# akshathmangudi/KAN-ViT

Hardware: AMD Instinct MI355X
Metric: images/sec (train step) KAN-ViT 224x224 (higher is better)
Workload: dtype f32

## Files before the change

include/kanvit.h:

```cpp
#ifndef KANVIT_H
#define KANVIT_H

#include <stddef.h>
#include <stdint.h>

#ifdef __cplusplus
extern "C" {
#endif

#if defined(__GNUC__) || defined(__clang__)
#pragma GCC visibility push(default)
#endif

#define KANVIT_ABI_VERSION 7

#define KANVIT_OK 0
#define KANVIT_EINVAL (-22)
#define KANVIT_ENOMEM (-12)
#define KANVIT_EDEVICE (-5)

#define KANVIT_FLAG_BF16_MFMA 1

#define KANVIT_FLAG_UNIFORM_KNOTS 2
#define KANVIT_FLAG_FUSED_LN 8
#define KANVIT_FLAG_SHARED_BPARAMS 4

#define KANVIT_FLAG_SINE_DFREQ 16

#define KANVIT_LINEAR 0
#define KANVIT_CHEBY 1
#define KANVIT_BSPLINE 2
#define KANVIT_RBF 3
#define KANVIT_SINE 4
#define KANVIT_FOURIER 5

typedef struct kanvit_layer_desc {
    int32_t family;
    int32_t groups;
    int32_t x_group_mod;
    int32_t I;
    int32_t O;
    int32_t G;
    int32_t spline_order;
    int32_t has_base;
    float rbf_inv_h;
    int32_t flags;
    int64_t M;
    int64_t ldx;
    int64_t ldu;
    int64_t ldy;
    int64_t bparam_stride;
    float ln_eps;
    int32_t base_act;
} kanvit_layer_desc;


#define KANVIT_BASE_SILU 0
#define KANVIT_BASE_GELU 1
#define KANVIT_BASE_GELU_TANH 2
#define KANVIT_BASE_RELU 3
#define KANVIT_BASE_TANH 4
#define KANVIT_BASE_IDENTITY 5

int kanvit_layer_ln_fusable(const kanvit_layer_desc* d);

size_t kanvit_layer_ln_bwd_workspace(const kanvit_layer_desc* d);
int kanvit_layer_ln_bwd(const kanvit_layer_desc* d, const float* x, const float* stats, const float* bparams, const float* du,
                        float* dx, float* dgamma, float* dbeta, void* workspace, size_t workspace_bytes, void* stream);

size_t kanvit_layer_fwd_workspace(const kanvit_layer_desc* d);
int kanvit_layer_fwd(const kanvit_layer_desc* d, const float* x, const float* u, const float* w,
                     const float* bparams, const float* bias, float* y, void* workspace, size_t workspace_bytes,
                     void* stream);

size_t kanvit_layer_bwd_input_workspace(const kanvit_layer_desc* d);
int kanvit_layer_bwd_input(const kanvit_layer_desc* d, const float* x, const float* u, const float* w,
                           const float* bparams, const float* dy, float* dx, float* du, float* dparam,
                           void* workspace, size_t workspace_bytes, void* stream);
int64_t kanvit_layer_dparam_tiles(const kanvit_layer_desc* d);
int kanvit_layer_sine_dfreq_ok(const kanvit_layer_desc* d);

size_t kanvit_layer_bwd_weight_workspace(const kanvit_layer_desc* d);
int kanvit_layer_bwd_weight(const kanvit_layer_desc* d, const float* x, const float* u, const float* bparams,
                            const float* dy, float* dw, void* workspace, size_t workspace_bytes, void* stream);

int kanvit_edge_l1_supported(const kanvit_layer_desc* d);
int64_t kanvit_edge_l1_row_bands(const kanvit_layer_desc* d);
size_t kanvit_edge_l1_fwd_workspace(const kanvit_layer_desc* d);
int kanvit_edge_l1_fwd(const kanvit_layer_desc* d, const float* x, const float* w, const float* bparams, float* A, void* workspace,
                       size_t workspace_bytes, void* stream);
size_t kanvit_edge_l1_bwd_workspace(const kanvit_layer_desc* d);
int kanvit_edge_l1_bwd(const kanvit_layer_desc* d, const float* x, const float* w, const float* bparams, const float* gA, float* dw,
                       float* dx, void* workspace, size_t workspace_bytes, void* stream);

#define KANVIT_BSPLINE_REFIT_TAU 1e-5
int kanvit_bspline_refit_supported(const kanvit_layer_desc* d);
size_t kanvit_bspline_refit_workspace(const kanvit_layer_desc* d);
int kanvit_bspline_refit_gram(const kanvit_layer_desc* d, const float* x, const float* old_knots, const float* new_knots, double* N,
                              double* C, void* workspace, size_t workspace_bytes, void* stream);
int kanvit_bspline_refit_solve(const kanvit_layer_desc* d, const double* N, const double* C, const float* w_old, float* w_new,
                               unsigned char* ok, void* stream);

int kanvit_bspline_regrid_supported(const kanvit_layer_desc* d, int old_G);
size_t kanvit_bspline_regrid_workspace(const kanvit_layer_desc* d, int old_G);
int kanvit_bspline_regrid_gram(const kanvit_layer_desc* d, int old_G, const float* x, const float* old_knots, const float* new_knots,
                               double* N, double* C, void* workspace, size_t workspace_bytes, void* stream);
int kanvit_bspline_regrid_solve(const kanvit_layer_desc* d, int old_G, const double* N, const double* C, const float* w_old,
                                float* w_new, unsigned char* ok, void* stream);

typedef struct kanvit_patch_desc {
    int32_t C, H, W;
    int32_t n_patches;
    int32_t prepend_rows;
    int32_t reserved;
} kanvit_patch_desc;
int kanvit_patch_embed_fwd(const kanvit_layer_desc* d, const kanvit_patch_desc* p, const float* images, const float* w,
                           const float* bparams, const float* bias, const float* cls, const float* pos, float* y,
                           void* stream);
int kanvit_patch_embed_fwd_ws(const kanvit_layer_desc* d, const kanvit_patch_desc* p, const float* images, const float* w,
                              const float* bparams, const float* bias, const float* cls, const float* pos, float* y,
                              void* workspace, size_t workspace_bytes, void* stream);
int kanvit_patch_embed_bwd_weight_ok(const kanvit_layer_desc* d, const kanvit_patch_desc* p);
size_t kanvit_patch_embed_bwd_weight_workspace(const kanvit_layer_desc* d, const kanvit_patch_desc* p);
int kanvit_patch_embed_bwd_weight(const kanvit_layer_desc* d, const kanvit_patch_desc* p, const float* images,
                                  const float* bparams, const float* dy, float* dw, void* workspace, size_t workspace_bytes,
                                  void* stream);

#define KANVIT_ATTN_MAX_N 256
#define KANVIT_ATTN_MAX_D 64
typedef struct kanvit_attn_desc {
    int32_t B, H, N, D;
    int32_t causal;
    float scale;
    int32_t flags;
    int32_t reserved;
    int64_t q_stride_b, q_stride_h, q_stride_n;
    int64_t k_stride_b, k_stride_h, k_stride_n;
    int64_t v_stride_b, v_stride_h, v_stride_n;
    int64_t o_stride_b, o_stride_h, o_stride_n;
} kanvit_attn_desc;

int kanvit_attn_fwd(const kanvit_attn_desc* d, const float* q, const float* k, const float* v,
                    float* o, float* lse, void* stream);
size_t kanvit_attn_bwd_workspace(const kanvit_attn_desc* d);
int kanvit_attn_bwd(const kanvit_attn_desc* d, const float* q, const float* k, const float* v,
                    const float* o, const float* lse, const float* d_o,
                    float* dq, float* dk, float* dv, void* workspace, size_t workspace_bytes, void* stream);

#define KANVIT_ATTN_X_MAX_D 128
typedef struct kanvit_attn_ext {
    int32_t Nk;
    int32_t reserved;
    const void* mask;
    int64_t mask_stride_b, mask_stride_h, mask_stride_q, mask_stride_k;
} kanvit_attn_ext;
int kanvit_attn_x_fwd(const kanvit_attn_desc* d, const kanvit_attn_ext* e, const float* q, const float* k, const float* v,
                      float* o, float* lse, void* stream);
size_t kanvit_attn_x_bwd_workspace(const kanvit_attn_desc* d, const kanvit_attn_ext* e);
int kanvit_attn_x_bwd(const kanvit_attn_desc* d, const kanvit_attn_ext* e, const float* q, const float* k, const float* v,
                      const float* o, const float* lse, const float* d_o, float* dq, float* dk, float* dv, void* workspace,
                      size_t workspace_bytes, void* stream);

int kanvit_attn_probs(const kanvit_attn_desc* d, const kanvit_attn_ext* e, const float* q, const float* k, float* p,
                      int64_t p_stride_b, int64_t p_stride_h, int64_t p_stride_q, int32_t rows, void* stream);

int kanvit_ff_small_supported(int D, int F);
int64_t kanvit_ff_small_max_rows(void);
int kanvit_ff_small_fwd(int64_t M, int D, int F, const float* x, const float* w1, const float* b1, const float* w2, const float* b2,
                        float* y, void* stream);
size_t kanvit_ff_small_bwd_workspace(int64_t M, int D, int F);
int kanvit_ff_small_bwd(int64_t M, int D, int F, const float* x, const float* w1, const float* b1, const float* w2, const float* dy,
                        float* dx, float* dw1, float* db1, float* dw2, float* db2, void* workspace, size_t workspace_bytes, void* stream);
int kanvit_lnff_small_fwd(int64_t M, int D, int F, float eps, const float* x, const float* delta, const float* gamma, const float* beta,
                          const float* w1, const float* b1, const float* w2, const float* b2, float* s, float* mean, float* rstd, float* y,
                          void* stream);
int kanvit_lnff_small_bwd(int64_t M, int D, int F, const float* s, const float* mean, const float* rstd, const float* gamma, const float* beta,
                          const float* w1, const float* b1, const float* w2, const float* dy, const float* ds_in, float* ds, float* dgamma,
                          float* dbeta, float* dw1, float* db1, float* dw2, float* db2, void* workspace, size_t workspace_bytes, void* stream);

int kanvit_addln_fwd(int64_t M, int D, float eps, const float* x, const float* delta, const float* gamma, const float* beta,
                     float* xsum, float* y, float* mean, float* rstd, void* stream);
size_t kanvit_addln_bwd_workspace(int64_t M, int D);
int kanvit_addln_bwd(int64_t M, int D, const float* xsum, const float* gamma, const float* mean, const float* rstd,
                     const float* dy, const float* dres, float* dx, float* dgamma, float* dbeta, void* workspace,
                     size_t workspace_bytes, void* stream);
int kanvit_addln_fwd_ex(int64_t M, int D, float eps, const float* x, const void* delta, int delta_bf16, const float* gamma, const float* beta,
                        float* xsum, void* y, int y_bf16, float* mean, float* rstd, void* stream);
int kanvit_addln_bwd_ex(int64_t M, int D, const float* xsum, const float* gamma, const float* mean, const float* rstd,
                        const void* dy, int dy_bf16, const float* dres, float* dx, void* dx_bf16, float* dgamma, float* dbeta, void* workspace,
                        size_t workspace_bytes, void* stream);

size_t kanvit_relu_bwd_bias_workspace(int64_t M, int N);
int kanvit_relu_bwd_bias(int64_t M, int N, const float* dy, const float* y, float* dh, float* dbias, void* workspace,
                         size_t workspace_bytes, void* stream);
int kanvit_relu_bwd_bias_bf16(int64_t M, int N, const void* dy_bf16, const void* y_bf16, void* dh_bf16, float* dbias, void* workspace,
                              size_t workspace_bytes, void* stream);

int kanvit_split3_bf16(int64_t M, int K, const float* x, const float* bias, int relu, const void* mask_hi, int64_t mask_ld,
                       void* out, int pattern, void* stream);

#define KANVIT_DECLARE_FAMILY(name)                                                                           \
    int kanvit_##name##_fwd(const kanvit_layer_desc*, const float*, const float*, const float*, const float*, \
                            const float*, float*, void*, size_t, void*);                                      \
    int kanvit_##name##_bwd_input(const kanvit_layer_desc*, const float*, const float*, const float*,         \
                                  const float*, const float*, float*, float*, float*, void*, size_t, void*);  \
    int kanvit_##name##_bwd_weight(const kanvit_layer_desc*, const float*, const float*, const float*,        \
                                   const float*, float*, void*, size_t, void*);                               \
    int kanvit_##name##_qkv_fwd(const kanvit_layer_desc*, const float*, const float*, const float*,           \
                                const float*, const float*, float*, void*, size_t, void*);                    \
    int kanvit_##name##_qkv_bwd_input(const kanvit_layer_desc*, const float*, const float*, const float*,     \
                                      const float*, const float*, float*, float*, float*, void*, size_t,      \
                                      void*);                                                                 \
    int kanvit_##name##_qkv_bwd_weight(const kanvit_layer_desc*, const float*, const float*, const float*,    \
                                       const float*, float*, void*, size_t, void*);
KANVIT_DECLARE_FAMILY(linear)
KANVIT_DECLARE_FAMILY(cheby)
KANVIT_DECLARE_FAMILY(bspline)
KANVIT_DECLARE_FAMILY(rbf)
KANVIT_DECLARE_FAMILY(sine)
KANVIT_DECLARE_FAMILY(fourier)

int kanvit_abi_version(void);
const char* kanvit_last_error(void);
const char* kanvit_config(void);
int kanvit_config_reload(void);
int kanvit_device_count(void);

#if defined(__GNUC__) || defined(__clang__)
#pragma GCC visibility pop
#endif

#ifdef __cplusplus
}
#endif
#endif
```

kan-vit_amd/attention.py:

```python
import torch
from torch import nn

from kanvit import grouped, ops
from models.cheby import ChebyKANLayer
from models.effkan import KANLinear
from models.fastkan import FastKANLayer
from models.sinekan import SineKANLayer
from utils import FlashAttentionFunction, default


class FlashAttention(nn.Module):

    def __init__(self, *, dim, heads=8, dim_head=64, causal=False, q_bucket_size=512, k_bucket_size=1024,
                 parallel=False, mixed_precision=False):
        super().__init__()
        if parallel or mixed_precision:
            raise NotImplementedError("parallel / mixed_precision are not part of the accelerated path; "
                                      "data parallelism is done per process (see train.py --dp)")
        self.heads = heads
        self.causal = causal
        self.parallel = parallel
        self.mixed_precision = mixed_precision
        inner = heads * dim_head
        self.to_q = nn.Linear(dim, inner, bias=False)
        self.to_kv = nn.Linear(dim, inner * 2, bias=False)
        self.to_out = nn.Linear(inner, dim, bias=False)
        self.q_bucket_size = q_bucket_size
        self.k_bucket_size = k_bucket_size

    def forward(self, x, context=None, mask=None, q_bucket_size=None, k_bucket_size=None):
        qb = default(q_bucket_size, self.q_bucket_size)
        kb = default(k_bucket_size, self.k_bucket_size)
        h = self.heads
        context = default(context, x)
        q = self.to_q(x)
        k, v = self.to_kv(context).chunk(2, dim=-1)
        b, n, _ = q.shape
        q, k, v = (t.view(b, t.shape[1], h, -1).permute(0, 2, 1, 3) for t in (q, k, v))
        out = FlashAttentionFunction.apply(q, k, v, mask, self.causal, qb, kb)
        return self.to_out(out.permute(0, 2, 1, 3).reshape(b, n, -1))

    @torch.no_grad()
    def attention_map(self, x, context=None, mask=None, rows=None):
        h = self.heads
        context = default(context, x)
        q = self.to_q(x)
        k = self.to_kv(context).chunk(2, dim=-1)[0]
        b = q.shape[0]
        q, k = (t.view(b, t.shape[1], h, -1).permute(0, 2, 1, 3) for t in (q, k))
        return ops.attention_probs(q, k, mask=mask, causal=self.causal, rows=rows)


class MSA(torch.nn.Module):

    def __init__(self, d, n_heads=4, type: str = "vanilla"):
        super().__init__()
        self.d = d
        self.n_heads = n_heads
        self.type = type
        assert d % n_heads == 0
        dh = d // n_heads
        makers = {
            "vanilla": lambda: nn.Linear(dh, dh),
            "flash-attn": lambda: nn.Linear(dh, dh),
            "fourier": lambda: nn.Linear(dh, dh),
            "efficientkan": lambda: KANLinear(dh, dh),
            "fast": lambda: FastKANLayer(dh, dh),
            "sine": lambda: SineKANLayer(dh, dh, grid_size=4),
            "cheby": lambda: ChebyKANLayer(dh, dh, 4),
        }
        if type not in makers:
            raise ValueError(f"{type} invalid. Please use a different argument.")
        make = makers[type]
        self.q_mappings = nn.ModuleList([make() for _ in range(n_heads)])
        self.k_mappings = nn.ModuleList([make() for _ in range(n_heads)])
        self.v_mappings = nn.ModuleList([make() for _ in range(n_heads)])
        self.d_head = dh
        self.softmax = nn.Softmax(dim=-1)

    REGULARIZED_TYPES = ("efficientkan", "cheby", "fast")

    def edge_activation_l1(self, x, include_base=False):
        from dataclasses import replace
        layers = list(self.q_mappings) + list(self.k_mappings) + list(self.v_mappings)
        l0 = layers[0]
        if not isinstance(l0, (KANLinear, ChebyKANLayer, FastKANLayer)):
            raise NotImplementedError(f"edge_activation_l1: per-head layers of type {type(l0).__name__} have no edge-activation "
                                      f"statistic; supported MSA types: {', '.join(self.REGULARIZED_TYPES)}")
        H, dh = self.n_heads, self.d_head
        x2d = x.reshape(-1, self.d)
        cfg = l0.kan_cfg() if isinstance(l0, ChebyKANLayer) else l0.kan_cfg(layers)
        w, bp, _ = type(l0).kan_pack_grouped(layers)
        base = bool(include_base) and cfg.has_base
        if base and len({ops.base_activation_code(m.base_activation) for m in layers}) > 1:
            raise NotImplementedError("edge_activation_l1(include_base=True): one grouped launch has one base activation")
        if cfg.has_base and not base:
            w = w.reshape(3 * H, dh, cfg.GP, dh)[:, :, :cfg.G].reshape(3 * H, dh * cfg.G, dh)
            cfg = replace(cfg, has_base=0, base_act=0)
        if isinstance(l0, FastKANLayer):
            xin = FastKANLayer.kan_u_grouped(layers, x2d, H)
            if base:
                xin = torch.cat([xin, x2d.to(xin.dtype).repeat(1, 3)], dim=1)
            cfg = replace(cfg, groups=3 * H, x_group_mod=3 * H)
        else:
            xin = x2d
            cfg = replace(cfg, groups=3 * H, x_group_mod=H)
        A = ops.edge_l1(xin, w, cfg, bp)
        return A.view(3, H, dh, dh).transpose(-1, -2)

    def regularization_loss(self, x, regularize_activation=1.0, regularize_entropy=1.0, include_base=False):
        return ops.l1_entropy_loss(self.edge_activation_l1(x, include_base), regularize_activation, regularize_entropy)

    @torch.no_grad()
    def update_grid(self, x, margin=0.01):
        from dataclasses import replace
        layers = list(self.q_mappings) + list(self.k_mappings) + list(self.v_mappings)
        l0 = layers[0]
        if not isinstance(l0, KANLinear):
            raise NotImplementedError(f"update_grid: MSA type '{self.type}' has no B-spline grid to update (only 'efficientkan' has)")
        for m in layers[1:]:
            assert (m.grid_size, m.spline_order, m.grid_eps, m.enable_standalone_scale_spline) == \
                (l0.grid_size, l0.spline_order, l0.grid_eps, l0.enable_standalone_scale_spline), \
                "update_grid: the per-head layers of one MSA must agree in grid_size, spline_order and grid_eps"
        H, dh = self.n_heads, self.d_head
        nb = l0.grid_size + l0.spline_order
        x2d = x.reshape(-1, self.d).float()
        new_grid = KANLinear.adapted_grid(x2d, l0.grid_size, l0.spline_order, l0.grid_eps, margin).view(H, dh, -1)
        cfg = replace(l0.kan_cfg(layers), has_base=0, base_act=0, groups=3 * H, x_group_mod=H)
        sw = torch.stack([m.scaled_spline_weight for m in layers])
        w_old = sw.permute(0, 2, 3, 1).reshape(3 * H, dh * nb, dh)
        old = torch.stack([m.grid.reshape(-1) for m in layers])
        w_new, ok = ops.bspline_refit(x2d, w_old, cfg, old, new_grid)
        for g, m in enumerate(layers):
            m.apply_refit(new_grid[g % H], w_new[g], ok[g % H])
        return (~ok).sum()

    @torch.no_grad()
    def extend_grid(self, x, grid_size, margin=0.01):
        from dataclasses import replace
        layers = list(self.q_mappings) + list(self.k_mappings) + list(self.v_mappings)
        l0 = layers[0]
        if not isinstance(l0, KANLinear):
            raise NotImplementedError(f"extend_grid: MSA type '{self.type}' has no B-spline grid to extend (only 'efficientkan' has)")
        for m in layers[1:]:
            assert (m.grid_size, m.spline_order, m.grid_eps, m.enable_standalone_scale_spline) == \
                (l0.grid_size, l0.spline_order, l0.grid_eps, l0.enable_standalone_scale_spline), \
                "extend_grid: the per-head layers of one MSA must agree in grid_size, spline_order and grid_eps"
        KANLinear.check_extension(grid_size, l0.spline_order)
        H, dh, order = self.n_heads, self.d_head, l0.spline_order
        nb_old = l0.grid_size + order
        x2d = x.reshape(-1, self.d).float()
        cfg = replace(l0.kan_cfg(layers), has_base=0, base_act=0, groups=3 * H, x_group_mod=H, G=grid_size + order)
        sw = torch.stack([m.scaled_spline_weight for m in layers])
        w_old = sw.permute(0, 2, 3, 1).reshape(3 * H, dh * nb_old, dh)
        grids = torch.stack([m.grid for m in layers])
        old = grids.reshape(3 * H, -1)
        new_grid = KANLinear.adapted_grid(x2d, grid_size, order, l0.grid_eps, margin).view(H, dh, -1)
        w_new, ok = ops.bspline_regrid(x2d, w_old, cfg, nb_old, old, new_grid)
        lo = grids[:, :, order].view(3, H * dh).min(dim=0).values
        hi = grids[:, :, -order - 1].view(3, H * dh).max(dim=0).values
        xf = KANLinear.span_samples(lo, hi, KANLinear.FALLBACK_SAMPLES)
        fb_grid = KANLinear.adapted_grid(xf, grid_size, order, l0.grid_eps, margin).view(H, dh, -1)
        w_fb, _ = ops.bspline_regrid(xf, w_old, cfg, nb_old, old, fb_grid)
        for g, m in enumerate(layers):
            m.apply_regrid(grid_size, new_grid[g % H], w_new[g], fb_grid[g % H], w_fb[g], ok[g % H])
        return (~ok).sum()

    @torch.no_grad()
    def attention_map(self, x, rows=None):
        b, n, d = x.shape
        qkv = grouped.run_qkv(self.q_mappings, self.k_mappings, self.v_mappings, x.reshape(b * n, d))
        return ops.attention_probs_packed(qkv.view(b, n, 3, self.n_heads, self.d_head), causal=False,
                                          scale=1.0 / (self.d_head ** 0.5), rows=rows)

    def forward(self, sequences):
        b, n, d = sequences.shape
        qkv = grouped.run_qkv(self.q_mappings, self.k_mappings, self.v_mappings, sequences.reshape(b * n, d))
        return ops.attention_packed(qkv.view(b, n, 3, self.n_heads, self.d_head), causal=False,
                                    scale=1.0 / (self.d_head ** 0.5))
```

kan-vit_amd/csrc/attention_x.hip:

```cpp
#include "kanvit_common.h"

#include <float.h>
#include <initializer_list>

namespace {

template <int DT>
struct XShape {
    static constexpr int THR = DT <= 2 ? 512 : 256;
    static constexpr int W = THR / 64;
    static constexpr bool ALIAS = DT > 2;
};
constexpr float LOG2E_X = 1.4426950408889634f;

struct AttnXArgs {
    const float* q;
    const float* k;
    const float* v;
    const float* o;
    const float* lse_in;
    const float* d_o;
    const float* delta_in;
    const unsigned char* mask;
    float* out;
    float* lse;
    float* dq;
    float* dk;
    float* dv;
    float* delta;
    long long msb, msh, msq, msk;
    long long qsb, qsh, qsn, ksb, ksh, ksn, vsb, vsh, vsn, osb, osh, osn;
    int B, H, Nq, Nk, D, causal, nqt, nkt;
    int vec;
    float scale;
};

__device__ __forceinline__ bool x_dead(const AttnXArgs& a, const unsigned char* mrow_base, int qrow, int key) {
    if (key >= a.Nk || (a.causal && key > qrow)) return true;
    if (mrow_base) {
        const int qi = qrow < a.Nq ? qrow : a.Nq - 1;
        return mrow_base[(long long)qi * a.msq + (long long)key * a.msk] == 0;
    }
    return false;
}

template <bool KEY_IN_REG>
__device__ __forceinline__ unsigned x_dead_bits(const AttnXArgs& a, const unsigned char* mrow_base, int lane_index, int tile0, int hf) {
    unsigned bits = 0;
#pragma unroll
    for (int r = 0; r < 16; ++r) {
        const int reg_index = tile0 + kv_acc_row(r, hf);
        const bool d = KEY_IN_REG ? x_dead(a, mrow_base, lane_index, reg_index) : x_dead(a, mrow_base, reg_index, lane_index);
        bits |= (d ? 1u : 0u) << r;
    }
    return bits;
}

template <int DT>
__device__ __forceinline__ void x_load_tile(float* __restrict__ dst, const float* __restrict__ src, long long stride_n, int row0,
                                            int rows, int n_valid, int D, int tid, int nthr, bool vec) {
    constexpr int W = 32 * DT, KS = W + 1;
    if (vec) {
        constexpr int W4 = W / 4;
        for (int idx = tid; idx < rows * W4; idx += nthr) {
            const int r = idx / W4, c = (idx - r * W4) * 4;
            const int n = row0 + r;
            f32x4 t = {0.0f, 0.0f, 0.0f, 0.0f};
            if (n < n_valid && c < D) t = *reinterpret_cast<const f32x4*>(src + (long long)n * stride_n + c);
#pragma unroll
            for (int e = 0; e < 4; ++e) dst[r * KS + c + e] = t[e];
        }
        return;
    }
    for (int idx = tid; idx < rows * W; idx += nthr) {
        const int r = idx / W, c = idx - r * W;
        const int n = row0 + r;
        dst[r * KS + c] = (n < n_valid && c < D) ? src[(long long)n * stride_n + c] : 0.0f;
    }
}

template <int DT>
__device__ __forceinline__ void x_store_tile(float* __restrict__ dstg, long long stride_n, int row0, int n_valid, int D,
                                             const float* __restrict__ T, int lane) {
    constexpr int KS = 32 * DT + 1;
    for (int idx = lane; idx < 32 * D; idx += 64) {
        const int r = idx / D, c = idx - r * D;
        const int n = row0 + r;
        if (n < n_valid) dstg[(long long)n * stride_n + c] = T[r * KS + c];
    }
}

constexpr int XCH = 4;

template <int DT>
__global__ __launch_bounds__(XShape<DT>::THR) void attn_x_fwd_kernel(const AttnXArgs a) {
    extern __shared__ __attribute__((aligned(16))) float smem[];
    constexpr int KS = 32 * DT + 1, CH = XCH * 32, XTHR = XShape<DT>::THR, XW = XShape<DT>::W;
    const int tid = threadIdx.x, lane = tid & 63, wave = tid >> 6, l31 = lane & 31, hf = lane >> 5;
    const int bh = blockIdx.x, bi = bh / a.H, hi = bh - bi * a.H;
    const int D = a.D, nkt = a.nkt;
    float* K_s = smem;
    float* V_s = K_s + CH * KS;
    float* Q_w = (XShape<DT>::ALIAS ? smem : V_s + CH * KS) + wave * 32 * KS;

    const float* qb = a.q + bi * a.qsb + hi * a.qsh;
    const float* kb = a.k + bi * a.ksb + hi * a.ksh;
    const float* vb = a.v + bi * a.vsb + hi * a.vsh;
    float* ob = a.out + bi * a.osb + hi * a.osh;
    const unsigned char* mb = a.mask ? a.mask + bi * a.msb + hi * a.msh : nullptr;

    const float sc2 = a.scale * LOG2E_X;
    const int qt = blockIdx.y * XW + wave;
    const int qrow = qt * 32 + l31;
    x_load_tile<DT>(Q_w, qb, a.qsn, qt * 32, 32, (qt < a.nqt) ? a.Nq : 0, D, lane, 64, a.vec);
    __syncthreads();
    float qf[16 * DT];
#pragma unroll
    for (int s = 0; s < 16 * DT; ++s) qf[s] = Q_w[l31 * KS + 2 * s + hf];

    f32x16 oacc[DT];
#pragma unroll
    for (int dt = 0; dt < DT; ++dt)
#pragma unroll
        for (int r = 0; r < 16; ++r) oacc[dt][r] = 0.0f;
    float mrun = -INFINITY, lrun = 0.0f;

    for (int kc = 0; kc < nkt; kc += XCH) {
        __syncthreads();
        x_load_tile<DT>(K_s, kb, a.ksn, kc * 32, CH, a.Nk, D, tid, XTHR, a.vec);
        x_load_tile<DT>(V_s, vb, a.vsn, kc * 32, CH, a.Nk, D, tid, XTHR, a.vec);
        __syncthreads();
        f32x16 sacc[XCH];
        unsigned dbits[XCH];
#pragma unroll
        for (int j = 0; j < XCH; ++j) {
#pragma unroll
            for (int r = 0; r < 16; ++r) sacc[j][r] = 0.0f;
            dbits[j] = (kc + j < nkt) ? x_dead_bits<true>(a, mb, qrow, (kc + j) * 32, hf) : 0xffffu;
            if (kc + j < nkt) {
                const float* kp = K_s + (j * 32 + l31) * KS + hf;
#pragma unroll
                for (int s = 0; s < 16 * DT; ++s) sacc[j] = __builtin_amdgcn_mfma_f32_32x32x2f32(kp[2 * s], qf[s], sacc[j], 0, 0, 0);
            }
        }
        float mx = mrun;
#pragma unroll
        for (int j = 0; j < XCH; ++j)
#pragma unroll
            for (int r = 0; r < 16; ++r) {
                const float sv = ((dbits[j] >> r) & 1u) ? -INFINITY : sacc[j][r];
                sacc[j][r] = sv;
                mx = fmaxf(mx, sv);
            }
        mx = fmaxf(mx, __shfl_xor(mx, 32));
        const float mxs = (mx == -INFINITY) ? 0.0f : mx * sc2;
        const float corr = exp2f(mrun * sc2 - mxs);
        float sum = 0.0f;
#pragma unroll
        for (int j = 0; j < XCH; ++j)
#pragma unroll
            for (int r = 0; r < 16; ++r) {
                const float p = exp2f(sacc[j][r] * sc2 - mxs);
                sacc[j][r] = p;
                sum += p;
            }
        sum += __shfl_xor(sum, 32);
        lrun = lrun * corr + sum;
        mrun = mx;
#pragma unroll
        for (int dt = 0; dt < DT; ++dt)
#pragma unroll
            for (int r = 0; r < 16; ++r) oacc[dt][r] *= corr;
#pragma unroll
        for (int j = 0; j < XCH; ++j) {
            if (kc + j < nkt) {
#pragma unroll
                for (int r = 0; r < 16; ++r) {
                    const float* vp = V_s + (j * 32 + kv_acc_row(r, hf)) * KS + l31;
#pragma unroll
                    for (int dt = 0; dt < DT; ++dt) oacc[dt] = __builtin_amdgcn_mfma_f32_32x32x2f32(vp[dt * 32], sacc[j][r], oacc[dt], 0, 0, 0);
                }
            }
        }
    }
    const float inv = lrun > 0.0f ? 1.0f / lrun : 0.0f;
    __syncthreads();
#pragma unroll
    for (int dt = 0; dt < DT; ++dt)
#pragma unroll
        for (int r = 0; r < 16; ++r) Q_w[l31 * KS + dt * 32 + kv_acc_row(r, hf)] = oacc[dt][r] * inv;
    __syncthreads();
    if (qt < a.nqt) {
        x_store_tile<DT>(ob, a.osn, qt * 32, a.Nq, D, Q_w, lane);
        if (hf == 0 && qrow < a.Nq && a.lse) a.lse[(long long)bh * a.Nq + qrow] = lrun > 0.0f ? mrun * a.scale + logf(lrun) : -FLT_MAX;
    }
}

__global__ __launch_bounds__(256) void attn_x_delta_kernel(const AttnXArgs a) {
    const int sub = threadIdx.x & 15;
    const long long row = (long long)blockIdx.x * 16 + (threadIdx.x >> 4);
    const long long rows = (long long)a.B * a.H * a.Nq;
    float s = 0.0f;
    if (row < rows) {
        const int n = (int)(row % a.Nq);
        const long long bh = row / a.Nq;
        const int hi = (int)(bh % a.H);
        const long long bi = bh / a.H;
        const float* op = a.o + bi * a.osb + hi * a.osh + (long long)n * a.osn;
        const float* dp = a.d_o + bi * a.osb + hi * a.osh + (long long)n * a.osn;
        for (int c = sub; c < a.D; c += 16) s += op[c] * dp[c];
    }
    s += __shfl_xor(s, 8);
    s += __shfl_xor(s, 4);
    s += __shfl_xor(s, 2);
    s += __shfl_xor(s, 1);
    if (row < rows && sub == 0) a.delta[row] = s;
}

template <int DT>
__global__ __launch_bounds__(XShape<DT>::THR) void attn_x_bwd_kv_kernel(const AttnXArgs a) {
    extern __shared__ __attribute__((aligned(16))) float smem[];
    constexpr int KS = 32 * DT + 1, CH = XCH * 32, XTHR = XShape<DT>::THR, XW = XShape<DT>::W;
    const int tid = threadIdx.x, lane = tid & 63, wave = tid >> 6, l31 = lane & 31, hf = lane >> 5;
    const int bh = blockIdx.x, bi = bh / a.H, hi = bh - bi * a.H;
    const int D = a.D;
    float* Q_s = smem;
    float* dO_s = Q_s + CH * KS;
    float* lse_s = dO_s + CH * KS;
    float* dl_s = lse_s + CH;
    float* T_w = (XShape<DT>::ALIAS ? smem : dl_s + CH) + wave * 32 * KS;

    const float* qb = a.q + bi * a.qsb + hi * a.qsh;
    const float* kb = a.k + bi * a.ksb + hi * a.ksh;
    const float* vb = a.v + bi * a.vsb + hi * a.vsh;
    const float* dob = a.d_o + bi * a.osb + hi * a.osh;
    float* dkb = a.dk + bi * a.ksb + hi * a.ksh;
    float* dvb = a.dv + bi * a.vsb + hi * a.vsh;
    const unsigned char* mb = a.mask ? a.mask + bi * a.msb + hi * a.msh : nullptr;
    const float sc2 = a.scale * LOG2E_X;

    const int jt = blockIdx.y * XW + wave;
    const int key = jt * 32 + l31;
    float kf[16 * DT], vf[16 * DT];
    x_load_tile<DT>(T_w, kb, a.ksn, jt * 32, 32, (jt < a.nkt) ? a.Nk : 0, D, lane, 64, a.vec);
    __syncthreads();
#pragma unroll
    for (int s = 0; s < 16 * DT; ++s) kf[s] = T_w[l31 * KS + 2 * s + hf];
    __syncthreads();
    x_load_tile<DT>(T_w, vb, a.vsn, jt * 32, 32, (jt < a.nkt) ? a.Nk : 0, D, lane, 64, a.vec);
    __syncthreads();
#pragma unroll
    for (int s = 0; s < 16 * DT; ++s) vf[s] = T_w[l31 * KS + 2 * s + hf];

    f32x16 dkacc[DT], dvacc[DT];
#pragma unroll
    for (int dt = 0; dt < DT; ++dt)
#pragma unroll
        for (int r = 0; r < 16; ++r) {
            dkacc[dt][r] = 0.0f;
            dvacc[dt][r] = 0.0f;
        }
    for (int qc = 0; qc < a.nqt; qc += XCH) {
        __syncthreads();
        x_load_tile<DT>(Q_s, qb, a.qsn, qc * 32, CH, a.Nq, D, tid, XTHR, a.vec);
        x_load_tile<DT>(dO_s, dob, a.osn, qc * 32, CH, a.Nq, D, tid, XTHR, a.vec);
        for (int n = tid; n < CH; n += XTHR) {
            const int qn = qc * 32 + n;
            lse_s[n] = (qn < a.Nq) ? a.lse_in[(long long)bh * a.Nq + qn] * LOG2E_X : INFINITY;
            dl_s[n] = (qn < a.Nq) ? a.delta_in[(long long)bh * a.Nq + qn] : 0.0f;
        }
        __syncthreads();
        for (int qq = 0; qq < XCH && qc + qq < a.nqt; ++qq) {
            f32x16 sacc, pacc;
#pragma unroll
            for (int r = 0; r < 16; ++r) {
                sacc[r] = 0.0f;
                pacc[r] = 0.0f;
            }
            const float* qp = Q_s + (qq * 32 + l31) * KS + hf;
            const float* dp = dO_s + (qq * 32 + l31) * KS + hf;
#pragma unroll
            for (int s = 0; s < 16 * DT; ++s) {
                sacc = __builtin_amdgcn_mfma_f32_32x32x2f32(qp[2 * s], kf[s], sacc, 0, 0, 0);
                pacc = __builtin_amdgcn_mfma_f32_32x32x2f32(dp[2 * s], vf[s], pacc, 0, 0, 0);
            }
            const unsigned db = x_dead_bits<false>(a, mb, key, (qc + qq) * 32, hf);
#pragma unroll
            for (int r = 0; r < 16; ++r) {
                const int ql = qq * 32 + kv_acc_row(r, hf), qrow = qc * 32 + ql;
                float p = exp2f(sacc[r] * sc2 - lse_s[ql]);
                if (jt >= a.nkt || qrow >= a.Nq || ((db >> r) & 1u)) p = 0.0f;
                sacc[r] = p;
                pacc[r] = p == 0.0f ? 0.0f : p * a.scale * (pacc[r] - dl_s[ql]);
            }
#pragma unroll
            for (int r = 0; r < 16; ++r) {
                const int row = (qq * 32 + kv_acc_row(r, hf)) * KS + l31;
#pragma unroll
                for (int dt = 0; dt < DT; ++dt) {
                    dvacc[dt] = __builtin_amdgcn_mfma_f32_32x32x2f32(dO_s[row + dt * 32], sacc[r], dvacc[dt], 0, 0, 0);
                    dkacc[dt] = __builtin_amdgcn_mfma_f32_32x32x2f32(Q_s[row + dt * 32], pacc[r], dkacc[dt], 0, 0, 0);
                }
            }
        }
    }
    __syncthreads();
#pragma unroll
    for (int dt = 0; dt < DT; ++dt)
#pragma unroll
        for (int r = 0; r < 16; ++r) T_w[l31 * KS + dt * 32 + kv_acc_row(r, hf)] = dkacc[dt][r];
    __syncthreads();
    if (jt < a.nkt) x_store_tile<DT>(dkb, a.ksn, jt * 32, a.Nk, D, T_w, lane);
    __syncthreads();
#pragma unroll
    for (int dt = 0; dt < DT; ++dt)
#pragma unroll
        for (int r = 0; r < 16; ++r) T_w[l31 * KS + dt * 32 + kv_acc_row(r, hf)] = dvacc[dt][r];
    __syncthreads();
    if (jt < a.nkt) x_store_tile<DT>(dvb, a.vsn, jt * 32, a.Nk, D, T_w, lane);
}

template <int DT>
__global__ __launch_bounds__(XShape<DT>::THR) void attn_x_bwd_q_kernel(const AttnXArgs a) {
    extern __shared__ __attribute__((aligned(16))) float smem[];
    constexpr int KS = 32 * DT + 1, CH = XCH * 32, XTHR = XShape<DT>::THR, XW = XShape<DT>::W;
    const int tid = threadIdx.x, lane = tid & 63, wave = tid >> 6, l31 = lane & 31, hf = lane >> 5;
    const int bh = blockIdx.x, bi = bh / a.H, hi = bh - bi * a.H;
    const int D = a.D, nkt = a.nkt;
    float* K_s = smem;
    float* V_s = K_s + CH * KS;
    float* T_w = (XShape<DT>::ALIAS ? smem : V_s + CH * KS) + wave * 32 * KS;

    const float* qb = a.q + bi * a.qsb + hi * a.qsh;
    const float* kb = a.k + bi * a.ksb + hi * a.ksh;
    const float* vb = a.v + bi * a.vsb + hi * a.vsh;
    const float* dob = a.d_o + bi * a.osb + hi * a.osh;
    float* dqb = a.dq + bi * a.qsb + hi * a.qsh;
    const unsigned char* mb = a.mask ? a.mask + bi * a.msb + hi * a.msh : nullptr;
    const float sc2 = a.scale * LOG2E_X;

    const int qt = blockIdx.y * XW + wave;
    const int qrow = qt * 32 + l31;
    const bool q_ok = (qt < a.nqt) && (qrow < a.Nq);
    float qf[16 * DT], dof[16 * DT];
    x_load_tile<DT>(T_w, qb, a.qsn, qt * 32, 32, (qt < a.nqt) ? a.Nq : 0, D, lane, 64, a.vec);
    __syncthreads();
#pragma unroll
    for (int s = 0; s < 16 * DT; ++s) qf[s] = T_w[l31 * KS + 2 * s + hf];
    __syncthreads();
    x_load_tile<DT>(T_w, dob, a.osn, qt * 32, 32, (qt < a.nqt) ? a.Nq : 0, D, lane, 64, a.vec);
    __syncthreads();
#pragma unroll
    for (int s = 0; s < 16 * DT; ++s) dof[s] = T_w[l31 * KS + 2 * s + hf];
    const float lse2 = q_ok ? a.lse_in[(long long)bh * a.Nq + qrow] * LOG2E_X : INFINITY;
    const float dl = q_ok ? a.delta_in[(long long)bh * a.Nq + qrow] : 0.0f;

    f32x16 dqacc[DT];
#pragma unroll
    for (int dt = 0; dt < DT; ++dt)
#pragma unroll
        for (int r = 0; r < 16; ++r) dqacc[dt][r] = 0.0f;
    for (int kc = 0; kc < nkt; kc += XCH) {
        __syncthreads();
        x_load_tile<DT>(K_s, kb, a.ksn, kc * 32, CH, a.Nk, D, tid, XTHR, a.vec);
        x_load_tile<DT>(V_s, vb, a.vsn, kc * 32, CH, a.Nk, D, tid, XTHR, a.vec);
        __syncthreads();
        for (int j = 0; j < XCH && kc + j < nkt; ++j) {
            f32x16 sacc, pacc;
#pragma unroll
            for (int r = 0; r < 16; ++r) {
                sacc[r] = 0.0f;
                pacc[r] = 0.0f;
            }
            const float* kp = K_s + (j * 32 + l31) * KS + hf;
            const float* vp = V_s + (j * 32 + l31) * KS + hf;
#pragma unroll
            for (int s = 0; s < 16 * DT; ++s) {
                sacc = __builtin_amdgcn_mfma_f32_32x32x2f32(kp[2 * s], qf[s], sacc, 0, 0, 0);
                pacc = __builtin_amdgcn_mfma_f32_32x32x2f32(vp[2 * s], dof[s], pacc, 0, 0, 0);
            }
            const unsigned db = x_dead_bits<true>(a, mb, qrow, (kc + j) * 32, hf);
#pragma unroll
            for (int r = 0; r < 16; ++r) {
                const float p = exp2f(sacc[r] * sc2 - lse2);
                const bool dead = !q_ok || ((db >> r) & 1u);
                pacc[r] = dead ? 0.0f : p * a.scale * (pacc[r] - dl);
            }
#pragma unroll
            for (int r = 0; r < 16; ++r) {
                const float* kr = K_s + (j * 32 + kv_acc_row(r, hf)) * KS + l31;
#pragma unroll
                for (int dt = 0; dt < DT; ++dt) dqacc[dt] = __builtin_amdgcn_mfma_f32_32x32x2f32(kr[dt * 32], pacc[r], dqacc[dt], 0, 0, 0);
            }
        }
    }
    __syncthreads();
#pragma unroll
    for (int dt = 0; dt < DT; ++dt)
#pragma unroll
        for (int r = 0; r < 16; ++r) T_w[l31 * KS + dt * 32 + kv_acc_row(r, hf)] = dqacc[dt][r];
    __syncthreads();
    if (qt < a.nqt) x_store_tile<DT>(dqb, a.qsn, qt * 32, a.Nq, D, T_w, lane);
}

typedef __bf16 bf16x8_t __attribute__((ext_vector_type(8)));
typedef __bf16 bf16x2_t __attribute__((ext_vector_type(2)));
typedef unsigned u32x4 __attribute__((ext_vector_type(4)));

__device__ __forceinline__ unsigned kv_pk(float lo, float hi) {
    bf16x2_t v = {(__bf16)lo, (__bf16)hi};
    return __builtin_bit_cast(unsigned, v);
}
__device__ __forceinline__ bf16x8_t kv_pack8(const float (&f)[8]) {
    const u32x4 u = {kv_pk(f[0], f[1]), kv_pk(f[2], f[3]), kv_pk(f[4], f[5]), kv_pk(f[6], f[7])};
    return __builtin_bit_cast(bf16x8_t, u);
}
__device__ __forceinline__ bf16x8_t kv_acc8(const f32x16& a, int s) {
    const u32x4 u = {kv_pk(a[8 * s], a[8 * s + 1]), kv_pk(a[8 * s + 2], a[8 * s + 3]), kv_pk(a[8 * s + 4], a[8 * s + 5]),
                     kv_pk(a[8 * s + 6], a[8 * s + 7])};
    return __builtin_bit_cast(bf16x8_t, u);
}
__device__ __forceinline__ int kv_key_slot(int ko) {
    const int w = ko & 15;
    return (ko & 16) + 8 * ((w >> 2) & 1) + 4 * (w >> 3) + (w & 3);
}

template <int DT>
struct XbShape {
    static constexpr int RB = 32 * DT + 8;
    static constexpr int TB = XCH * 32 + 8;
    static constexpr int ROWS = XCH * 32 * RB;
    static constexpr int TRANS = 32 * DT * TB;
};

__device__ __forceinline__ bf16x8_t xb_grow8(const float* __restrict__ p, int c, int D, bool ok, bool vec) {
    float f[8];
    if (vec) {
        f32x4 u0 = {0.0f, 0.0f, 0.0f, 0.0f}, u1 = u0;
        if (ok && c < D) u0 = *reinterpret_cast<const f32x4*>(p + c);
        if (ok && c + 4 < D) u1 = *reinterpret_cast<const f32x4*>(p + c + 4);
#pragma unroll
        for (int e = 0; e < 4; ++e) {
            f[e] = u0[e];
            f[4 + e] = u1[e];
        }
    } else {
#pragma unroll
        for (int e = 0; e < 8; ++e) f[e] = (ok && c + e < D) ? p[c + e] : 0.0f;
    }
    return kv_pack8(f);
}

template <int DT, int NTHR, bool ROWS, bool TRANS>
__device__ __forceinline__ void xb_fill(unsigned short* __restrict__ rimg, unsigned short* __restrict__ timg, const float* __restrict__ src,
                                        long long stride_n, int row0, int n_valid, int D, int tid, bool vec) {
    constexpr int W4 = 8 * DT, ITEMS = XCH * 16 * W4, RB = XbShape<DT>::RB, TB = XbShape<DT>::TB;
    static_assert(ITEMS % NTHR == 0, "whole passes");
#pragma unroll
    for (int it = 0; it < ITEMS / NTHR; ++it) {
        const int idx = it * NTHR + tid;
        const int m = idx / W4, c = (idx - m * W4) * 4;
        const int n0 = row0 + 2 * m;
        f32x4 t0 = {0.0f, 0.0f, 0.0f, 0.0f}, t1 = t0;
        if (vec) {
            if (c < D && n0 < n_valid) t0 = *reinterpret_cast<const f32x4*>(src + (long long)n0 * stride_n + c);
            if (c < D && n0 + 1 < n_valid) t1 = *reinterpret_cast<const f32x4*>(src + (long long)(n0 + 1) * stride_n + c);
        } else {
#pragma unroll
            for (int e = 0; e < 4; ++e) {
                if (c + e < D && n0 < n_valid) t0[e] = src[(long long)n0 * stride_n + c + e];
                if (c + e < D && n0 + 1 < n_valid) t1[e] = src[(long long)(n0 + 1) * stride_n + c + e];
            }
        }
        if constexpr (ROWS) {
            unsigned* r0p = reinterpret_cast<unsigned*>(rimg + (2 * m) * RB + c);
            unsigned* r1p = reinterpret_cast<unsigned*>(rimg + (2 * m + 1) * RB + c);
            r0p[0] = kv_pk(t0[0], t0[1]);
            r0p[1] = kv_pk(t0[2], t0[3]);
            r1p[0] = kv_pk(t1[0], t1[1]);
            r1p[1] = kv_pk(t1[2], t1[3]);
        }
        if constexpr (TRANS) {
            const int pos = ((2 * m) & ~31) + kv_key_slot((2 * m) & 31);
#pragma unroll
            for (int e = 0; e < 4; ++e) *reinterpret_cast<unsigned*>(timg + (c + e) * TB + pos) = kv_pk(t0[e], t1[e]);
        }
    }
}

template <int DT>
__device__ __forceinline__ void xb_store_row(float* __restrict__ p, const f32x16 (&acc)[DT], float mul, int D, int hf, bool vec) {
#pragma unroll
    for (int dt = 0; dt < DT; ++dt)
#pragma unroll
        for (int q = 0; q < 4; ++q) {
            const int c = dt * 32 + 8 * q + 4 * hf;
            if (vec) {
                if (c < D) {
                    const f32x4 v = {acc[dt][4 * q] * mul, acc[dt][4 * q + 1] * mul, acc[dt][4 * q + 2] * mul, acc[dt][4 * q + 3] * mul};
                    *reinterpret_cast<f32x4*>(p + c) = v;
                }
            } else {
#pragma unroll
                for (int e = 0; e < 4; ++e)
                    if (c + e < D) p[c + e] = acc[dt][4 * q + e] * mul;
            }
        }
}

constexpr int XB_THR = 512;

template <int DT>
__device__ __forceinline__ void xb_fwd_scores(f32x16 (&sacc)[XCH], const unsigned short* __restrict__ Kr, const bf16x8_t (&qf)[2 * DT],
                                              const AttnXArgs& a, const unsigned char* mb, int qrow, int kc, int l31, int hf) {
    constexpr int RB = XbShape<DT>::RB;
#pragma unroll
    for (int j = 0; j < XCH; ++j) {
#pragma unroll
        for (int r = 0; r < 16; ++r) sacc[j][r] = 0.0f;
        const unsigned dbits = (kc + j < a.nkt) ? x_dead_bits<true>(a, mb, qrow, (kc + j) * 32, hf) : 0xffffu;
        if (kc + j < a.nkt) {
            const unsigned short* kp = Kr + (j * 32 + l31) * RB + 8 * hf;
#pragma unroll
            for (int ks = 0; ks < 2 * DT; ++ks)
                sacc[j] = __builtin_amdgcn_mfma_f32_32x32x16_bf16(*reinterpret_cast<const bf16x8_t*>(kp + 16 * ks), qf[ks], sacc[j], 0, 0, 0);
        }
#pragma unroll
        for (int r = 0; r < 16; ++r) sacc[j][r] = ((dbits >> r) & 1u) ? -INFINITY : sacc[j][r];
    }
}

template <int DT>
__global__ __launch_bounds__(XB_THR) void attn_x_fwd_bf16_kernel(const AttnXArgs a) {
    extern __shared__ __attribute__((aligned(16))) float smem[];
    constexpr int TB = XbShape<DT>::TB, XW = XB_THR / 64;
    const int tid = threadIdx.x, lane = tid & 63, wave = tid >> 6, l31 = lane & 31, hf = lane >> 5;
    const int bh = blockIdx.x, bi = bh / a.H, hi = bh - bi * a.H;
    const int D = a.D, nkt = a.nkt;
    unsigned short* Kr = reinterpret_cast<unsigned short*>(smem);
    unsigned short* Vt = Kr + XbShape<DT>::ROWS;

    const float* qb = a.q + bi * a.qsb + hi * a.qsh;
    const float* kb = a.k + bi * a.ksb + hi * a.ksh;
    const float* vb = a.v + bi * a.vsb + hi * a.vsh;
    float* ob = a.out + bi * a.osb + hi * a.osh;
    const unsigned char* mb = a.mask ? a.mask + bi * a.msb + hi * a.msh : nullptr;

    const float sc2 = a.scale * LOG2E_X;
    const int qt = blockIdx.y * XW + wave;
    const int qrow = qt * 32 + l31;
    const bool q_ok = qt < a.nqt && qrow < a.Nq;
    bf16x8_t qf[2 * DT];
#pragma unroll
    for (int ks = 0; ks < 2 * DT; ++ks) qf[ks] = xb_grow8(qb + (long long)(q_ok ? qrow : 0) * a.qsn, 16 * ks + 8 * hf, D, q_ok, a.vec);

    f32x16 sacc[XCH];
    float mx = -INFINITY;
    for (int kc = 0; kc < nkt; kc += XCH) {
        __syncthreads();
        xb_fill<DT, XB_THR, true, false>(Kr, nullptr, kb, a.ksn, kc * 32, a.Nk, D, tid, a.vec);
        __syncthreads();
        xb_fwd_scores<DT>(sacc, Kr, qf, a, mb, qrow, kc, l31, hf);
#pragma unroll
        for (int j = 0; j < XCH; ++j)
#pragma unroll
            for (int r = 0; r < 16; ++r) mx = fmaxf(mx, sacc[j][r]);
    }
    mx = fmaxf(mx, __shfl_xor(mx, 32));
    const float mxs = (mx == -INFINITY) ? 0.0f : mx * sc2;

    f32x16 oacc[DT];
#pragma unroll
    for (int dt = 0; dt < DT; ++dt)
#pragma unroll
        for (int r = 0; r < 16; ++r) oacc[dt][r] = 0.0f;
    float lsum = 0.0f;
    for (int kc = 0; kc < nkt; kc += XCH) {
        __syncthreads();
        if (nkt > XCH) xb_fill<DT, XB_THR, true, false>(Kr, nullptr, kb, a.ksn, kc * 32, a.Nk, D, tid, a.vec);
        xb_fill<DT, XB_THR, false, true>(nullptr, Vt, vb, a.vsn, kc * 32, a.Nk, D, tid, a.vec);
        __syncthreads();
        xb_fwd_scores<DT>(sacc, Kr, qf, a, mb, qrow, kc, l31, hf);
        float sum = 0.0f;
#pragma unroll
        for (int j = 0; j < XCH; ++j)
#pragma unroll
            for (int r = 0; r < 16; ++r) {
                const float p = exp2f(sacc[j][r] * sc2 - mxs);
                sacc[j][r] = p;
                sum += p;
            }
        lsum += sum + __shfl_xor(sum, 32);
#pragma unroll
        for (int j = 0; j < XCH; ++j) {
            if (kc + j < nkt) {
#pragma unroll
                for (int s2 = 0; s2 < 2; ++s2) {
                    const bf16x8_t pb = kv_acc8(sacc[j], s2);
                    const unsigned short* vp = Vt + l31 * TB + j * 32 + 16 * s2 + 8 * hf;
#pragma unroll
                    for (int dt = 0; dt < DT; ++dt)
                        oacc[dt] = __builtin_amdgcn_mfma_f32_32x32x16_bf16(*reinterpret_cast<const bf16x8_t*>(vp + dt * 32 * TB), pb, oacc[dt], 0, 0, 0);
                }
            }
        }
    }
    if (q_ok) {
        const float inv = lsum > 0.0f ? 1.0f / lsum : 0.0f;
        xb_store_row<DT>(ob + (long long)qrow * a.osn, oacc, inv, D, hf, a.vec && ((uintptr_t)ob % 16 == 0));
        if (hf == 0 && a.lse) a.lse[(long long)bh * a.Nq + qrow] = lsum > 0.0f ? mx * a.scale + logf(lsum) : -FLT_MAX;
    }
}

template <int DT>
__global__ __launch_bounds__(XB_THR) void attn_x_bwd_kv_bf16_kernel(const AttnXArgs a) {
    extern __shared__ __attribute__((aligned(16))) float smem[];
    constexpr int RB = XbShape<DT>::RB, TB = XbShape<DT>::TB, CH = XCH * 32, XW = XB_THR / 64;
    const int tid = threadIdx.x, lane = tid & 63, wave = tid >> 6, l31 = lane & 31, hf = lane >> 5;
    const int bh = blockIdx.x, bi = bh / a.H, hi = bh - bi * a.H;
    const int D = a.D;
    unsigned short* Qr = reinterpret_cast<unsigned short*>(smem);
    unsigned short* dOr = Qr + XbShape<DT>::ROWS;
    unsigned short* Qt = dOr + XbShape<DT>::ROWS;
    unsigned short* dOt = Qt + XbShape<DT>::TRANS;
    float* lse_s = reinterpret_cast<float*>(dOt + XbShape<DT>::TRANS);
    float* dl_s = lse_s + CH;

    const float* qb = a.q + bi * a.qsb + hi * a.qsh;
    const float* kb = a.k + bi * a.ksb + hi * a.ksh;
    const float* vb = a.v + bi * a.vsb + hi * a.vsh;
    const float* dob = a.d_o + bi * a.osb + hi * a.osh;
    float* dkb = a.dk + bi * a.ksb + hi * a.ksh;
    float* dvb = a.dv + bi * a.vsb + hi * a.vsh;
    const unsigned char* mb = a.mask ? a.mask + bi * a.msb + hi * a.msh : nullptr;
    const float sc2 = a.scale * LOG2E_X;

    const int jt = blockIdx.y * XW + wave;
    const int key = jt * 32 + l31;
    const bool k_ok = jt < a.nkt && key < a.Nk;
    bf16x8_t kf[2 * DT], vf[2 * DT];
#pragma unroll
    for (int ks = 0; ks < 2 * DT; ++ks) {
        kf[ks] = xb_grow8(kb + (long long)(k_ok ? key : 0) * a.ksn, 16 * ks + 8 * hf, D, k_ok, a.vec);
        vf[ks] = xb_grow8(vb + (long long)(k_ok ? key : 0) * a.vsn, 16 * ks + 8 * hf, D, k_ok, a.vec);
    }

    f32x16 dkacc[DT], dvacc[DT];
#pragma unroll
    for (int dt = 0; dt < DT; ++dt)
#pragma unroll
        for (int r = 0; r < 16; ++r) {
            dkacc[dt][r] = 0.0f;
            dvacc[dt][r] = 0.0f;
        }
    for (int qc = 0; qc < a.nqt; qc += XCH) {
        __syncthreads();
        xb_fill<DT, XB_THR, true, true>(Qr, Qt, qb, a.qsn, qc * 32, a.Nq, D, tid, a.vec);
        xb_fill<DT, XB_THR, true, true>(dOr, dOt, dob, a.osn, qc * 32, a.Nq, D, tid, a.vec);
        for (int n = tid; n < CH; n += XB_THR) {
            const int qn = qc * 32 + n;
            lse_s[n] = (qn < a.Nq) ? a.lse_in[(long long)bh * a.Nq + qn] * LOG2E_X : INFINITY;
            dl_s[n] = (qn < a.Nq) ? a.delta_in[(long long)bh * a.Nq + qn] : 0.0f;
        }
        __syncthreads();
        for (int qq = 0; qq < XCH && qc + qq < a.nqt; ++qq) {
            f32x16 sacc, pacc;
#pragma unroll
            for (int r = 0; r < 16; ++r) {
                sacc[r] = 0.0f;
                pacc[r] = 0.0f;
            }
            const unsigned short* qp = Qr + (qq * 32 + l31) * RB + 8 * hf;
            const unsigned short* dp = dOr + (qq * 32 + l31) * RB + 8 * hf;
#pragma unroll
            for (int ks = 0; ks < 2 * DT; ++ks) {
                sacc = __builtin_amdgcn_mfma_f32_32x32x16_bf16(*reinterpret_cast<const bf16x8_t*>(qp + 16 * ks), kf[ks], sacc, 0, 0, 0);
                pacc = __builtin_amdgcn_mfma_f32_32x32x16_bf16(*reinterpret_cast<const bf16x8_t*>(dp + 16 * ks), vf[ks], pacc, 0, 0, 0);
            }
            const unsigned db = x_dead_bits<false>(a, mb, key, (qc + qq) * 32, hf);
#pragma unroll
            for (int r = 0; r < 16; ++r) {
                const int ql = qq * 32 + kv_acc_row(r, hf), qrow = qc * 32 + ql;
                float p = exp2f(sacc[r] * sc2 - lse_s[ql]);
                if (jt >= a.nkt || qrow >= a.Nq || ((db >> r) & 1u)) p = 0.0f;
                sacc[r] = p;
                pacc[r] = p == 0.0f ? 0.0f : p * a.scale * (pacc[r] - dl_s[ql]);
            }
#pragma unroll
            for (int s2 = 0; s2 < 2; ++s2) {
                const bf16x8_t pb = kv_acc8(sacc, s2), sb = kv_acc8(pacc, s2);
                const int off = l31 * TB + qq * 32 + 16 * s2 + 8 * hf;
#pragma unroll
                for (int dt = 0; dt < DT; ++dt) {
                    dvacc[dt] = __builtin_amdgcn_mfma_f32_32x32x16_bf16(*reinterpret_cast<const bf16x8_t*>(dOt + off + dt * 32 * TB), pb, dvacc[dt], 0, 0, 0);
                    dkacc[dt] = __builtin_amdgcn_mfma_f32_32x32x16_bf16(*reinterpret_cast<const bf16x8_t*>(Qt + off + dt * 32 * TB), sb, dkacc[dt], 0, 0, 0);
                }
            }
        }
    }
    if (k_ok) {
        xb_store_row<DT>(dkb + (long long)key * a.ksn, dkacc, 1.0f, D, hf, a.vec && ((uintptr_t)dkb % 16 == 0));
        xb_store_row<DT>(dvb + (long long)key * a.vsn, dvacc, 1.0f, D, hf, a.vec && ((uintptr_t)dvb % 16 == 0));
    }
}

template <int DT>
__global__ __launch_bounds__(XB_THR) void attn_x_bwd_q_bf16_kernel(const AttnXArgs a) {
    extern __shared__ __attribute__((aligned(16))) float smem[];
    constexpr int RB = XbShape<DT>::RB, TB = XbShape<DT>::TB, XW = XB_THR / 64;
    const int tid = threadIdx.x, lane = tid & 63, wave = tid >> 6, l31 = lane & 31, hf = lane >> 5;
    const int bh = blockIdx.x, bi = bh / a.H, hi = bh - bi * a.H;
    const int D = a.D, nkt = a.nkt;
    unsigned short* Kr = reinterpret_cast<unsigned short*>(smem);
    unsigned short* Vr = Kr + XbShape<DT>::ROWS;
    unsigned short* Kt = Vr + XbShape<DT>::ROWS;

    const float* qb = a.q + bi * a.qsb + hi * a.qsh;
    const float* kb = a.k + bi * a.ksb + hi * a.ksh;
    const float* vb = a.v + bi * a.vsb + hi * a.vsh;
    const float* dob = a.d_o + bi * a.osb + hi * a.osh;
    float* dqb = a.dq + bi * a.qsb + hi * a.qsh;
    const unsigned char* mb = a.mask ? a.mask + bi * a.msb + hi * a.msh : nullptr;
    const float sc2 = a.scale * LOG2E_X;

    const int qt = blockIdx.y * XW + wave;
    const int qrow = qt * 32 + l31;
    const bool q_ok = (qt < a.nqt) && (qrow < a.Nq);
    bf16x8_t qf[2 * DT], dof[2 * DT];
#pragma unroll
    for (int ks = 0; ks < 2 * DT; ++ks) {
        qf[ks] = xb_grow8(qb + (long long)(q_ok ? qrow : 0) * a.qsn, 16 * ks + 8 * hf, D, q_ok, a.vec);
        dof[ks] = xb_grow8(dob + (long long)(q_ok ? qrow : 0) * a.osn, 16 * ks + 8 * hf, D, q_ok, a.vec);
    }
    const float lse2 = q_ok ? a.lse_in[(long long)bh * a.Nq + qrow] * LOG2E_X : INFINITY;
    const float dl = q_ok ? a.delta_in[(long long)bh * a.Nq + qrow] : 0.0f;

    f32x16 dqacc[DT];
#pragma unroll
    for (int dt = 0; dt < DT; ++dt)
#pragma unroll
        for (int r = 0; r < 16; ++r) dqacc[dt][r] = 0.0f;
    for (int kc = 0; kc < nkt; kc += XCH) {
        __syncthreads();
        xb_fill<DT, XB_THR, true, true>(Kr, Kt, kb, a.ksn, kc * 32, a.Nk, D, tid, a.vec);
        xb_fill<DT, XB_THR, true, false>(Vr, nullptr, vb, a.vsn, kc * 32, a.Nk, D, tid, a.vec);
        __syncthreads();
        for (int j = 0; j < XCH && kc + j < nkt; ++j) {
            f32x16 sacc, pacc;
#pragma unroll
            for (int r = 0; r < 16; ++r) {
                sacc[r] = 0.0f;
                pacc[r] = 0.0f;
            }
            const unsigned short* kp = Kr + (j * 32 + l31) * RB + 8 * hf;
            const unsigned short* vp = Vr + (j * 32 + l31) * RB + 8 * hf;
#pragma unroll
            for (int ks = 0; ks < 2 * DT; ++ks) {
                sacc = __builtin_amdgcn_mfma_f32_32x32x16_bf16(*reinterpret_cast<const bf16x8_t*>(kp + 16 * ks), qf[ks], sacc, 0, 0, 0);
                pacc = __builtin_amdgcn_mfma_f32_32x32x16_bf16(*reinterpret_cast<const bf16x8_t*>(vp + 16 * ks), dof[ks], pacc, 0, 0, 0);
            }
            const unsigned db = x_dead_bits<true>(a, mb, qrow, (kc + j) * 32, hf);
#pragma unroll
            for (int r = 0; r < 16; ++r) {
                const float p = exp2f(sacc[r] * sc2 - lse2);
                const bool dead = !q_ok || ((db >> r) & 1u);
                pacc[r] = dead ? 0.0f : p * a.scale * (pacc[r] - dl);
            }
#pragma unroll
            for (int s2 = 0; s2 < 2; ++s2) {
                const bf16x8_t sb = kv_acc8(pacc, s2);
                const unsigned short* kt = Kt + l31 * TB + j * 32 + 16 * s2 + 8 * hf;
#pragma unroll
                for (int dt = 0; dt < DT; ++dt)
                    dqacc[dt] = __builtin_amdgcn_mfma_f32_32x32x16_bf16(*reinterpret_cast<const bf16x8_t*>(kt + dt * 32 * TB), sb, dqacc[dt], 0, 0, 0);
            }
        }
    }
    if (q_ok) xb_store_row<DT>(dqb + (long long)qrow * a.qsn, dqacc, 1.0f, D, hf, a.vec && ((uintptr_t)dqb % 16 == 0));
}

int x_check(const kanvit_attn_desc* d, const kanvit_attn_ext* e, const char* who) {
    if (!d || !e) return kv_fail(KANVIT_EINVAL, "%s: null descriptor", who);
    if (d->B < 0 || d->H < 1 || d->N < 1 || e->Nk < 1 || d->D < 1) return kv_fail(KANVIT_EINVAL, "%s: bad sizes", who);
    if (d->D > KANVIT_ATTN_X_MAX_D || (d->D & 1)) return kv_fail(KANVIT_EINVAL, "%s: D=%d must be even and <= %d", who, d->D, KANVIT_ATTN_X_MAX_D);
    if ((long long)d->B * d->H > 0x7fffffffLL) return kv_fail(KANVIT_EINVAL, "%s: B*H too large", who);
    if (!(d->scale > 0.0f)) return kv_fail(KANVIT_EINVAL, "%s: scale=%g must be positive (the running maximum is taken over the raw scores)", who, (double)d->scale);
    if (d->causal && e->Nk > d->N)
        return kv_fail(KANVIT_EINVAL, "%s: causal with k_len=%d > q_len=%d is ill-defined in the reference (utils.py:169,183: the first k_len - q_len queries see no key)", who, e->Nk, d->N);
    if ((d->flags & KANVIT_FLAG_BF16_MFMA) && d->D > KANVIT_ATTN_MAX_D)
        return kv_fail(KANVIT_EINVAL, "%s: KANVIT_FLAG_BF16_MFMA covers D <= %d in the general attention kernels; D=%d runs exact fp32 only (pass no flag)",
                       who, KANVIT_ATTN_MAX_D, d->D);
    if ((long long)(d->N + 127) / 128 > 65535 || (long long)(e->Nk + 127) / 128 > 65535) return kv_fail(KANVIT_EINVAL, "%s: sequence too long for one launch", who);
    return 0;
}

AttnXArgs x_args(const kanvit_attn_desc* d, const kanvit_attn_ext* e) {
    AttnXArgs a{};
    a.B = d->B; a.H = d->H; a.Nq = d->N; a.Nk = e->Nk; a.D = d->D; a.causal = d->causal; a.scale = d->scale;
    a.nqt = (d->N + 31) / 32;
    a.nkt = (e->Nk + 31) / 32;
    a.qsb = d->q_stride_b; a.qsh = d->q_stride_h; a.qsn = d->q_stride_n;
    a.ksb = d->k_stride_b; a.ksh = d->k_stride_h; a.ksn = d->k_stride_n;
    a.vsb = d->v_stride_b; a.vsh = d->v_stride_h; a.vsn = d->v_stride_n;
    a.osb = d->o_stride_b; a.osh = d->o_stride_h; a.osn = d->o_stride_n;
    a.vec = (d->D % 4 == 0);
    for (long long sd : {a.qsb, a.qsh, a.qsn, a.ksb, a.ksh, a.ksn, a.vsb, a.vsh, a.vsn, a.osb, a.osh, a.osn}) a.vec = a.vec && (sd % 4 == 0);
    a.mask = (const unsigned char*)e->mask;
    a.msb = e->mask_stride_b; a.msh = e->mask_stride_h; a.msq = e->mask_stride_q; a.msk = e->mask_stride_k;
    return a;
}

template <int DT>
constexpr size_t x_stage_floats() {
    static_assert(!XShape<DT>::ALIAS || XShape<DT>::W * 32 <= 2 * XCH * 32, "aliased staging tiles must lie inside the chunk buffers");
    return XShape<DT>::ALIAS ? 0 : (size_t)XShape<DT>::W * 32 * (32 * DT + 1);
}

template <int DT>
int x_launch_fwd(const AttnXArgs& a, hipStream_t st) {
    constexpr int KS = 32 * DT + 1, CH = XCH * 32, XTHR = XShape<DT>::THR, XW = XShape<DT>::W;
    const size_t lds = sizeof(float) * ((size_t)2 * CH * KS + x_stage_floats<DT>());
    static_assert(sizeof(float) * ((size_t)2 * CH * KS + x_stage_floats<DT>()) <= 160 * 1024, "forward LDS over 160 KiB");
    KV_ALLOW_LDS(160 * 1024, (attn_x_fwd_kernel<DT>));
    hipLaunchKernelGGL((attn_x_fwd_kernel<DT>), dim3((unsigned)(a.B * a.H), (unsigned)((a.nqt + XW - 1) / XW)), dim3(XTHR), lds, st, a);
    KV_LAUNCH_CHECK("attn_x_fwd_kernel");
    return 0;
}

template <int DT>
int x_launch_bwd(const AttnXArgs& a, hipStream_t st) {
    constexpr int KS = 32 * DT + 1, CH = XCH * 32, XTHR = XShape<DT>::THR, XW = XShape<DT>::W;
    const size_t lds_kv = sizeof(float) * ((size_t)2 * CH * KS + 2 * (size_t)CH + x_stage_floats<DT>());
    const size_t lds_q = sizeof(float) * ((size_t)2 * CH * KS + x_stage_floats<DT>());
    static_assert(sizeof(float) * ((size_t)2 * CH * KS + 2 * (size_t)CH + x_stage_floats<DT>()) <= 160 * 1024, "dK/dV LDS over 160 KiB");
    KV_ALLOW_LDS(160 * 1024, (attn_x_bwd_kv_kernel<DT>));
    KV_ALLOW_LDS(160 * 1024, (attn_x_bwd_q_kernel<DT>));
    hipLaunchKernelGGL((attn_x_bwd_kv_kernel<DT>), dim3((unsigned)(a.B * a.H), (unsigned)((a.nkt + XW - 1) / XW)), dim3(XTHR), lds_kv, st, a);
    KV_LAUNCH_CHECK("attn_x_bwd_kv_kernel");
    hipLaunchKernelGGL((attn_x_bwd_q_kernel<DT>), dim3((unsigned)(a.B * a.H), (unsigned)((a.nqt + XW - 1) / XW)), dim3(XTHR), lds_q, st, a);
    KV_LAUNCH_CHECK("attn_x_bwd_q_kernel");
    return 0;
}

template <int DT>
int xb_launch_fwd(const AttnXArgs& a, hipStream_t st) {
    constexpr int XW = XB_THR / 64;
    constexpr size_t lds = 2 * ((size_t)XbShape<DT>::ROWS + XbShape<DT>::TRANS);
    KV_ALLOW_LDS(lds, (attn_x_fwd_bf16_kernel<DT>));
    hipLaunchKernelGGL((attn_x_fwd_bf16_kernel<DT>), dim3((unsigned)(a.B * a.H), (unsigned)((a.nqt + XW - 1) / XW)), dim3(XB_THR), lds, st, a);
    KV_LAUNCH_CHECK("attn_x_fwd_bf16_kernel");
    return 0;
}

template <int DT>
int xb_launch_bwd(const AttnXArgs& a, hipStream_t st) {
    constexpr int XW = XB_THR / 64;
    constexpr size_t lds_kv = 2 * (2 * (size_t)XbShape<DT>::ROWS + 2 * (size_t)XbShape<DT>::TRANS) + sizeof(float) * 2 * XCH * 32;
    constexpr size_t lds_q = 2 * (2 * (size_t)XbShape<DT>::ROWS + XbShape<DT>::TRANS);
    static_assert(lds_kv <= 160 * 1024 && (2 * (2 * (size_t)XbShape<DT>::ROWS + 2 * (size_t)XbShape<DT>::TRANS)) % 16 == 0, "dK/dV LDS");
    KV_ALLOW_LDS(lds_kv, (attn_x_bwd_kv_bf16_kernel<DT>));
    KV_ALLOW_LDS(lds_q, (attn_x_bwd_q_bf16_kernel<DT>));
    hipLaunchKernelGGL((attn_x_bwd_kv_bf16_kernel<DT>), dim3((unsigned)(a.B * a.H), (unsigned)((a.nkt + XW - 1) / XW)), dim3(XB_THR), lds_kv, st, a);
    KV_LAUNCH_CHECK("attn_x_bwd_kv_bf16_kernel");
    hipLaunchKernelGGL((attn_x_bwd_q_bf16_kernel<DT>), dim3((unsigned)(a.B * a.H), (unsigned)((a.nqt + XW - 1) / XW)), dim3(XB_THR), lds_q, st, a);
    KV_LAUNCH_CHECK("attn_x_bwd_q_bf16_kernel");
    return 0;
}

}

extern "C" {

int kanvit_attn_x_fwd(const kanvit_attn_desc* d, const kanvit_attn_ext* e, const float* q, const float* k, const float* v, float* o,
                      float* lse, void* stream) {
    if (int rc = x_check(d, e, "kanvit_attn_x_fwd")) return rc;
    if (!q || !k || !v || !o) return kv_fail(KANVIT_EINVAL, "kanvit_attn_x_fwd: null q/k/v/o");
    if (d->B == 0) return 0;
    AttnXArgs a = x_args(d, e);
    a.q = q; a.k = k; a.v = v; a.out = o; a.lse = lse;
    a.vec = a.vec && (((uintptr_t)q | (uintptr_t)k | (uintptr_t)v) % 16 == 0);
    hipStream_t st = (hipStream_t)stream;
    if (d->flags & KANVIT_FLAG_BF16_MFMA) return d->D <= 32 ? xb_launch_fwd<1>(a, st) : xb_launch_fwd<2>(a, st);
    return d->D <= 32 ? x_launch_fwd<1>(a, st) : d->D <= 64 ? x_launch_fwd<2>(a, st) : d->D <= 96 ? x_launch_fwd<3>(a, st) : x_launch_fwd<4>(a, st);
}

size_t kanvit_attn_x_bwd_workspace(const kanvit_attn_desc* d, const kanvit_attn_ext* e) {
    if (!d || !e || d->B < 0 || d->H < 1 || d->N < 1) return 0;
    return (sizeof(float) * (size_t)d->B * d->H * d->N + 15) / 16 * 16;
}

int kanvit_attn_x_bwd(const kanvit_attn_desc* d, const kanvit_attn_ext* e, const float* q, const float* k, const float* v, const float* o,
                      const float* lse, const float* d_o, float* dq, float* dk, float* dv, void* workspace, size_t workspace_bytes,
                      void* stream) {
    if (int rc = x_check(d, e, "kanvit_attn_x_bwd")) return rc;
    if (!q || !k || !v || !o || !lse || !d_o || !dq || !dk || !dv) return kv_fail(KANVIT_EINVAL, "kanvit_attn_x_bwd: null argument");
    if (d->B == 0) return 0;
    const size_t need = kanvit_attn_x_bwd_workspace(d, e);
    if (!workspace || workspace_bytes < need) return kv_fail(KANVIT_ENOMEM, "kanvit_attn_x_bwd: workspace %zu bytes < required %zu", workspace_bytes, need);
    AttnXArgs a = x_args(d, e);
    a.q = q; a.k = k; a.v = v; a.o = o; a.lse_in = lse; a.d_o = d_o;
    a.dq = dq; a.dk = dk; a.dv = dv; a.delta = (float*)workspace; a.delta_in = (const float*)workspace;
    a.vec = a.vec && (((uintptr_t)q | (uintptr_t)k | (uintptr_t)v | (uintptr_t)d_o) % 16 == 0);
    hipStream_t st = (hipStream_t)stream;
    const long long rows = (long long)d->B * d->H * d->N;
    hipLaunchKernelGGL(attn_x_delta_kernel, dim3((unsigned)((rows + 15) / 16)), dim3(256), 0, st, a);
    KV_LAUNCH_CHECK("attn_x_delta_kernel");
    if (d->flags & KANVIT_FLAG_BF16_MFMA) return d->D <= 32 ? xb_launch_bwd<1>(a, st) : xb_launch_bwd<2>(a, st);
    return d->D <= 32 ? x_launch_bwd<1>(a, st) : d->D <= 64 ? x_launch_bwd<2>(a, st) : d->D <= 96 ? x_launch_bwd<3>(a, st) : x_launch_bwd<4>(a, st);
}

}
```

kan-vit_amd/kanvit/_lib.py:

```python
import ctypes as C
import os

import torch

HERE = os.path.dirname(os.path.abspath(__file__))
LIB_PATH = os.environ.get("KANVIT_LIB") or os.path.join(HERE, "libkanvit.so")

LINEAR, CHEBY, BSPLINE, RBF, SINE, FOURIER = range(6)
FLAG_BF16_MFMA = 1
FLAG_UNIFORM_KNOTS = 2
FLAG_SHARED_BPARAMS = 4
FLAG_FUSED_LN = 8
FLAG_SINE_DFREQ = 16
FAMILY_NAMES = ["linear", "cheby", "bspline", "rbf", "sine", "fourier"]
BASE_SILU, BASE_GELU, BASE_GELU_TANH, BASE_RELU, BASE_TANH, BASE_IDENTITY = range(6)
BASE_NAMES = ["silu", "gelu", "gelu-tanh", "relu", "tanh", "identity"]


class KanvitError(RuntimeError):
    pass


class LayerDesc(C.Structure):
    _fields_ = [("family", C.c_int32), ("groups", C.c_int32), ("x_group_mod", C.c_int32), ("I", C.c_int32),
                ("O", C.c_int32), ("G", C.c_int32), ("spline_order", C.c_int32), ("has_base", C.c_int32),
                ("rbf_inv_h", C.c_float), ("flags", C.c_int32), ("M", C.c_int64), ("ldx", C.c_int64),
                ("ldu", C.c_int64), ("ldy", C.c_int64), ("bparam_stride", C.c_int64), ("ln_eps", C.c_float), ("base_act", C.c_int32)]


class AttnDesc(C.Structure):
    _fields_ = [("B", C.c_int32), ("H", C.c_int32), ("N", C.c_int32), ("D", C.c_int32), ("causal", C.c_int32),
                ("scale", C.c_float), ("flags", C.c_int32), ("reserved", C.c_int32),
                ("q_stride_b", C.c_int64), ("q_stride_h", C.c_int64), ("q_stride_n", C.c_int64),
                ("k_stride_b", C.c_int64), ("k_stride_h", C.c_int64), ("k_stride_n", C.c_int64),
                ("v_stride_b", C.c_int64), ("v_stride_h", C.c_int64), ("v_stride_n", C.c_int64),
                ("o_stride_b", C.c_int64), ("o_stride_h", C.c_int64), ("o_stride_n", C.c_int64)]


class AttnExt(C.Structure):
    _fields_ = [("Nk", C.c_int32), ("reserved", C.c_int32), ("mask", C.c_void_p),
                ("mask_stride_b", C.c_int64), ("mask_stride_h", C.c_int64), ("mask_stride_q", C.c_int64), ("mask_stride_k", C.c_int64)]


class PatchDesc(C.Structure):
    _fields_ = [("C", C.c_int32), ("H", C.c_int32), ("W", C.c_int32), ("n_patches", C.c_int32), ("prepend_rows", C.c_int32),
                ("reserved", C.c_int32)]


_P = C.c_void_p
_LAYER_FWD = [C.POINTER(LayerDesc), _P, _P, _P, _P, _P, _P, _P, C.c_size_t, _P]
_LAYER_BWD_IN = [C.POINTER(LayerDesc), _P, _P, _P, _P, _P, _P, _P, _P, _P, C.c_size_t, _P]
_LAYER_BWD_W = [C.POINTER(LayerDesc), _P, _P, _P, _P, _P, _P, C.c_size_t, _P]

SYMBOLS = {
    "kanvit_abi_version": (C.c_int, []),
    "kanvit_last_error": (C.c_char_p, []),
    "kanvit_device_count": (C.c_int, []),
    "kanvit_config": (C.c_char_p, []),
    "kanvit_config_reload": (C.c_int, []),
    "kanvit_ff_small_supported": (C.c_int, [C.c_int, C.c_int]),
    "kanvit_ff_small_max_rows": (C.c_int64, []),
    "kanvit_ff_small_fwd": (C.c_int, [C.c_int64, C.c_int, C.c_int] + [C.c_void_p] * 7),
    "kanvit_ff_small_bwd_workspace": (C.c_size_t, [C.c_int64, C.c_int, C.c_int]),
    "kanvit_ff_small_bwd": (C.c_int, [C.c_int64, C.c_int, C.c_int] + [C.c_void_p] * 11 + [C.c_size_t, C.c_void_p]),
    "kanvit_lnff_small_fwd": (C.c_int, [C.c_int64, C.c_int, C.c_int, C.c_float] + [C.c_void_p] * 13),
    "kanvit_lnff_small_bwd": (C.c_int, [C.c_int64, C.c_int, C.c_int] + [C.c_void_p] * 18 + [C.c_size_t, C.c_void_p]),
    "kanvit_layer_ln_fusable": (C.c_int, [C.POINTER(LayerDesc)]),
    "kanvit_layer_ln_bwd_workspace": (C.c_size_t, [C.POINTER(LayerDesc)]),
    "kanvit_layer_ln_bwd": (C.c_int, [C.POINTER(LayerDesc)] + [C.c_void_p] * 8 + [C.c_size_t, C.c_void_p]),
    "kanvit_layer_fwd_workspace": (C.c_size_t, [C.POINTER(LayerDesc)]),
    "kanvit_layer_bwd_input_workspace": (C.c_size_t, [C.POINTER(LayerDesc)]),
    "kanvit_layer_fwd": (C.c_int, _LAYER_FWD),
    "kanvit_layer_bwd_input": (C.c_int, _LAYER_BWD_IN),
    "kanvit_layer_dparam_tiles": (C.c_int64, [C.POINTER(LayerDesc)]),
    "kanvit_layer_sine_dfreq_ok": (C.c_int, [C.POINTER(LayerDesc)]),
    "kanvit_layer_bwd_weight_workspace": (C.c_size_t, [C.POINTER(LayerDesc)]),
    "kanvit_layer_bwd_weight": (C.c_int, _LAYER_BWD_W),
    "kanvit_edge_l1_supported": (C.c_int, [C.POINTER(LayerDesc)]),
    "kanvit_edge_l1_row_bands": (C.c_int64, [C.POINTER(LayerDesc)]),
    "kanvit_edge_l1_fwd_workspace": (C.c_size_t, [C.POINTER(LayerDesc)]),
    "kanvit_edge_l1_fwd": (C.c_int, [C.POINTER(LayerDesc), _P, _P, _P, _P, _P, C.c_size_t, _P]),
    "kanvit_edge_l1_bwd_workspace": (C.c_size_t, [C.POINTER(LayerDesc)]),
    "kanvit_edge_l1_bwd": (C.c_int, [C.POINTER(LayerDesc), _P, _P, _P, _P, _P, _P, _P, C.c_size_t, _P]),
    "kanvit_bspline_refit_supported": (C.c_int, [C.POINTER(LayerDesc)]),
    "kanvit_bspline_refit_workspace": (C.c_size_t, [C.POINTER(LayerDesc)]),
    "kanvit_bspline_refit_gram": (C.c_int, [C.POINTER(LayerDesc), _P, _P, _P, _P, _P, _P, C.c_size_t, _P]),
    "kanvit_bspline_refit_solve": (C.c_int, [C.POINTER(LayerDesc), _P, _P, _P, _P, _P, _P]),
    "kanvit_bspline_regrid_supported": (C.c_int, [C.POINTER(LayerDesc), C.c_int]),
    "kanvit_bspline_regrid_workspace": (C.c_size_t, [C.POINTER(LayerDesc), C.c_int]),
    "kanvit_bspline_regrid_gram": (C.c_int, [C.POINTER(LayerDesc), C.c_int, _P, _P, _P, _P, _P, _P, C.c_size_t, _P]),
    "kanvit_bspline_regrid_solve": (C.c_int, [C.POINTER(LayerDesc), C.c_int, _P, _P, _P, _P, _P, _P]),
    "kanvit_patch_embed_fwd": (C.c_int, [C.POINTER(LayerDesc), C.POINTER(PatchDesc), _P, _P, _P, _P, _P, _P, _P, _P]),
    "kanvit_patch_embed_fwd_ws": (C.c_int, [C.POINTER(LayerDesc), C.POINTER(PatchDesc), _P, _P, _P, _P, _P, _P, _P, _P, C.c_size_t, _P]),
    "kanvit_patch_embed_bwd_weight_ok": (C.c_int, [C.POINTER(LayerDesc), C.POINTER(PatchDesc)]),
    "kanvit_patch_embed_bwd_weight_workspace": (C.c_size_t, [C.POINTER(LayerDesc), C.POINTER(PatchDesc)]),
    "kanvit_patch_embed_bwd_weight": (C.c_int, [C.POINTER(LayerDesc), C.POINTER(PatchDesc), _P, _P, _P, _P, _P, C.c_size_t, _P]),
    "kanvit_attn_fwd": (C.c_int, [C.POINTER(AttnDesc), _P, _P, _P, _P, _P, _P]),
    "kanvit_attn_bwd_workspace": (C.c_size_t, [C.POINTER(AttnDesc)]),
    "kanvit_attn_bwd": (C.c_int, [C.POINTER(AttnDesc), _P, _P, _P, _P, _P, _P, _P, _P, _P, _P, C.c_size_t, _P]),
    "kanvit_attn_x_fwd": (C.c_int, [C.POINTER(AttnDesc), C.POINTER(AttnExt), _P, _P, _P, _P, _P, _P]),
    "kanvit_attn_x_bwd_workspace": (C.c_size_t, [C.POINTER(AttnDesc), C.POINTER(AttnExt)]),
    "kanvit_attn_x_bwd": (C.c_int, [C.POINTER(AttnDesc), C.POINTER(AttnExt), _P, _P, _P, _P, _P, _P, _P, _P, _P, _P, C.c_size_t, _P]),
    "kanvit_attn_probs": (C.c_int, [C.POINTER(AttnDesc), C.POINTER(AttnExt), _P, _P, _P, C.c_int64, C.c_int64, C.c_int64, C.c_int32, _P]),
    "kanvit_addln_fwd": (C.c_int, [C.c_int64, C.c_int, C.c_float, _P, _P, _P, _P, _P, _P, _P, _P, _P]),
    "kanvit_addln_fwd_ex": (C.c_int, [C.c_int64, C.c_int, C.c_float, _P, _P, C.c_int, _P, _P, _P, _P, C.c_int, _P, _P, _P]),
    "kanvit_addln_bwd_ex": (C.c_int, [C.c_int64, C.c_int, _P, _P, _P, _P, _P, C.c_int, _P, _P, _P, _P, _P, _P, C.c_size_t, _P]),
    "kanvit_addln_bwd_workspace": (C.c_size_t, [C.c_int64, C.c_int]),
    "kanvit_addln_bwd": (C.c_int, [C.c_int64, C.c_int, _P, _P, _P, _P, _P, _P, _P, _P, _P, _P, C.c_size_t, _P]),
    "kanvit_relu_bwd_bias_workspace": (C.c_size_t, [C.c_int64, C.c_int]),
    "kanvit_relu_bwd_bias": (C.c_int, [C.c_int64, C.c_int, _P, _P, _P, _P, _P, C.c_size_t, _P]),
    "kanvit_relu_bwd_bias_bf16": (C.c_int, [C.c_int64, C.c_int, _P, _P, _P, _P, _P, C.c_size_t, _P]),
    "kanvit_split3_bf16": (C.c_int, [C.c_int64, C.c_int, _P, _P, C.c_int, _P, C.c_int64, _P, C.c_int, _P]),
}
for _f in FAMILY_NAMES:
    SYMBOLS[f"kanvit_{_f}_fwd"] = (C.c_int, _LAYER_FWD)
    SYMBOLS[f"kanvit_{_f}_bwd_input"] = (C.c_int, _LAYER_BWD_IN)
    SYMBOLS[f"kanvit_{_f}_bwd_weight"] = (C.c_int, _LAYER_BWD_W)
    SYMBOLS[f"kanvit_{_f}_qkv_fwd"] = (C.c_int, _LAYER_FWD)
    SYMBOLS[f"kanvit_{_f}_qkv_bwd_input"] = (C.c_int, _LAYER_BWD_IN)
    SYMBOLS[f"kanvit_{_f}_qkv_bwd_weight"] = (C.c_int, _LAYER_BWD_W)

_lib = None


def lib():
    global _lib
    if _lib is None:
        if not os.path.exists(LIB_PATH):
            raise KanvitError(
                f"{LIB_PATH} not found: build it with `python kan-vit_amd/kanvit/build.py` "
                "(or __graft_entry__.build()). The kanvit ops have no CPU / eager fallback.")
        handle = C.CDLL(LIB_PATH)
        for name, (res, args) in SYMBOLS.items():
            fn = getattr(handle, name)
            fn.restype = res
            fn.argtypes = args
        if handle.kanvit_abi_version() != 7:
            raise KanvitError("libkanvit.so ABI version mismatch")
        _lib = handle
    return _lib


_py_switches = None


def py_switches() -> dict:
    global _py_switches
    if _py_switches is None:
        _py_switches = {"ff": os.environ.get("KANVIT_FF", ""), "no_ff_small": int(bool(os.environ.get("KANVIT_NO_FF_SMALL"))),
                        "no_lnff": int(bool(os.environ.get("KANVIT_NO_LNFF"))),
                        "no_ff_epi": int(bool(os.environ.get("KANVIT_NO_FF_EPILOGUE"))),
                        "no_dfreq_w": int(bool(os.environ.get("KANVIT_NO_DFREQ_W"))),
                        "no_patch_bw": int(bool(os.environ.get("KANVIT_NO_PATCH_BW")))}
    return _py_switches


def active_config() -> str:
    ps = py_switches()
    alt = f" lib={LIB_PATH}" if os.environ.get("KANVIT_LIB") else ""
    return lib().kanvit_config().decode() + f" py_ff={ps['ff'] or 'default'} py_no_ff_small={ps['no_ff_small']} py_no_lnff={ps['no_lnff']} py_no_ff_epi={ps['no_ff_epi']} py_no_dfreq_w={ps['no_dfreq_w']} py_no_patch_bw={ps['no_patch_bw']}" + alt


def reload_config() -> str:
    global _py_switches
    _py_switches = None
    lib().kanvit_config_reload()
    return active_config()


def check(rc, what):
    if rc != 0:
        msg = lib().kanvit_last_error()
        raise KanvitError(f"{what} failed (code {rc}): {msg.decode() if msg else '?'}")
```

kan-vit_amd/kanvit/grouped.py:

```python
from __future__ import annotations

from dataclasses import replace
from typing import Sequence

import torch
import torch.nn.functional as F

from . import ops


class _StackParams(torch.autograd.Function):

    @staticmethod
    def forward(ctx, *tensors):
        return torch.stack(tensors)

    @staticmethod
    def backward(ctx, grad):
        return grad.contiguous().unbind(0)


class _StackPermuted(torch.autograd.Function):

    @staticmethod
    def forward(ctx, perm, *tensors):
        ctx.inv = tuple(sorted(range(len(perm)), key=lambda a: perm[a]))
        return torch.stack([t.permute(*perm) for t in tensors])

    @staticmethod
    def backward(ctx, grad):
        inv = (0,) + tuple(1 + a for a in ctx.inv)
        return (None,) + grad.permute(*inv).contiguous().unbind(0)


def stack_params(tensors: Sequence[torch.Tensor], perm: Sequence[int] = None) -> torch.Tensor:
    tensors = list(tensors)
    if perm is not None:
        if any(t.requires_grad for t in tensors) and torch.is_grad_enabled():
            return _StackPermuted.apply(tuple(perm), *tensors)
        return torch.stack([t.permute(*perm) for t in tensors])
    if any(t.requires_grad for t in tensors) and torch.is_grad_enabled():
        return _StackParams.apply(*tensors)
    return torch.stack(tensors)


def linear_cfg(lin: torch.nn.Linear) -> ops.LayerCfg:
    return ops.LayerCfg(family=ops.LINEAR, I=lin.in_features, O=lin.out_features, G=1)


def linear_pack(lin: torch.nn.Linear):
    return lin.weight.t(), None, lin.bias


def _cfg_pack(m):
    if isinstance(m, torch.nn.Linear):
        return linear_cfg(m), linear_pack(m)
    return m.kan_cfg(), m.kan_pack()


def run_single(layer, x2d: torch.Tensor) -> torch.Tensor:
    cfg, (w, bp, bias) = _cfg_pack(layer)
    if hasattr(layer, "kan_ln") and layer.kan_ln() is not None and ops.ln_fusable(cfg, x2d.shape[0]):
        ln = layer.kan_ln()
        return ops.kan_layer_ln(x2d, w.unsqueeze(0), cfg, torch.cat([bp, ln.weight, ln.bias]).unsqueeze(0),
                                None if bias is None else bias.reshape(1, -1), ln.eps)
    u = layer.kan_u(x2d) if hasattr(layer, "kan_u") else None
    return ops.kan_layer(x2d, w.unsqueeze(0), cfg, u=u,
                         bparams=None if bp is None else bp.unsqueeze(0),
                         bias=None if bias is None else bias.reshape(1, -1))


def run_qkv(q_layers: Sequence, k_layers: Sequence, v_layers: Sequence, x2d: torch.Tensor) -> torch.Tensor:
    H = len(q_layers)
    layers = list(q_layers) + list(k_layers) + list(v_layers)
    acts = {ops.base_activation_code(m.base_activation) for m in layers
            if hasattr(m, "base_activation") and getattr(m, "use_base_update", True)}
    if len(acts) > 1:
        dh = x2d.shape[1] // H
        return torch.cat([run_single(m, x2d[:, (g % H) * dh:(g % H + 1) * dh]) for g, m in enumerate(layers)], dim=1)
    if isinstance(layers[0], torch.nn.Linear):
        cfg0 = linear_cfg(layers[0])
    elif hasattr(type(layers[0]), "kan_pack_grouped") and "layers" in layers[0].kan_cfg.__code__.co_varnames:
        cfg0 = layers[0].kan_cfg(layers)
    else:
        cfg0 = layers[0].kan_cfg()
    cfg = replace(cfg0, groups=3 * H, x_group_mod=H)
    if isinstance(layers[0], torch.nn.Linear):
        w = stack_params([m.weight for m in layers], perm=(1, 0))
        bp = None
        bias = None if layers[0].bias is None else stack_params([m.bias for m in layers])
    else:
        w, bp, bias = type(layers[0]).kan_pack_grouped(layers)
    if hasattr(layers[0], "kan_ln") and layers[0].kan_ln() is not None and ops.ln_fusable(cfg, x2d.shape[0]):
        gamma = stack_params([l.kan_ln().weight for l in layers])
        beta = stack_params([l.kan_ln().bias for l in layers])
        return ops.kan_layer_ln(x2d, w, cfg, torch.cat([bp, gamma, beta], dim=1), bias, layers[0].kan_ln().eps)
    u = None
    if hasattr(layers[0], "kan_u_grouped"):
        u = type(layers[0]).kan_u_grouped(layers, x2d, H)
    return ops.kan_layer(x2d, w, cfg, u=u, bparams=bp, bias=bias)
```

kan-vit_amd/kanvit/ops.py:

```python
from __future__ import annotations

import ctypes as C
from dataclasses import dataclass
from typing import Optional, Tuple

import torch

from . import _lib
from ._lib import BSPLINE, CHEBY, FOURIER, LINEAR, RBF, SINE, AttnDesc, KanvitError, LayerDesc, check


@dataclass(frozen=True)
class LayerCfg:
    family: int
    I: int
    O: int
    G: int
    groups: int = 1
    x_group_mod: int = 1
    spline_order: int = 0
    has_base: int = 0
    rbf_inv_h: float = 0.0
    flags: int = 0
    ln_eps: float = 0.0
    base_act: int = 0

    @property
    def GP(self) -> int:
        return {LINEAR: 1, CHEBY: self.G, BSPLINE: self.G + self.has_base, RBF: self.G + self.has_base,
                SINE: self.G, FOURIER: 2 * self.G}[self.family]

    @property
    def K(self) -> int:
        return self.I * self.GP


class KernelTimer:

    def __init__(self):
        self.records = {}

    def add(self, tag, start, end, flops, nbytes):
        self.records.setdefault(tag, []).append((start, end, flops, nbytes))

    def summary(self):
        torch.cuda.synchronize()
        out = {}
        for tag, recs in self.records.items():
            ms = [s.elapsed_time(e) for s, e, _, _ in recs]
            out[tag] = {"launches": len(recs), "total_ms": sum(ms), "avg_ms": sum(ms) / len(ms),
                        "flops": recs[0][2], "bytes": recs[0][3]}
        return out


timer: Optional[KernelTimer] = None


class _timed:
    def __init__(self, tag, flops=0, nbytes=0):
        self.tag, self.flops, self.nbytes = tag, flops, nbytes

    def __enter__(self):
        if timer is not None:
            self.s = torch.cuda.Event(enable_timing=True)
            self.e = torch.cuda.Event(enable_timing=True)
            self.s.record()
        return self

    def __exit__(self, *exc):
        if timer is not None:
            self.e.record()
            timer.add(self.tag, self.s, self.e, self.flops, self.nbytes)
        return False


def _layer_cost(cfg: "LayerCfg", M: int, kind: str):
    flops = 2 * M * cfg.K * cfg.O * cfg.groups
    xb, yb, wb = M * cfg.x_group_mod * cfg.I, M * cfg.groups * cfg.O, cfg.groups * cfg.K * cfg.O
    nbytes = 4 * {"fwd": xb + yb + wb, "bwd_input": 2 * xb + yb + wb, "bwd_weight": xb + yb + wb}[kind]
    return flops, nbytes


def _ptr(t: Optional[torch.Tensor]):
    return None if t is None else C.c_void_p(t.data_ptr())


def _stream():
    return C.c_void_p(torch.cuda.current_stream().cuda_stream)


def _require_gpu_f32(name: str, t: Optional[torch.Tensor]):
    if t is None:
        return
    if not t.is_cuda:
        raise KanvitError(f"{name} is on {t.device}: the kanvit ops run only on an AMD GPU (no CPU fallback)")
    if t.dtype != torch.float32:
        raise KanvitError(f"{name} has dtype {t.dtype}; the kanvit kernels compute in float32")


SUPPORTED_BASE_ACTIVATIONS = ("nn.SiLU(), F.silu; nn.GELU(), F.gelu; nn.GELU(approximate='tanh'), "
                              "functools.partial(F.gelu, approximate='tanh'); nn.ReLU(), F.relu, torch.relu; "
                              "nn.Tanh(), torch.tanh, F.tanh; nn.Identity()")


def base_activation_code(fn) -> Optional[int]:
    import functools
    import torch.nn.functional as F
    nn = torch.nn
    if isinstance(fn, functools.partial):
        if fn.args or not (fn.func is F.gelu or fn.func is torch._C._nn.gelu):
            return None
        if set(fn.keywords) - {"approximate"}:
            return None
        a = fn.keywords.get("approximate", "none")
        return {"none": _lib.BASE_GELU, "tanh": _lib.BASE_GELU_TANH}.get(a)
    if isinstance(fn, nn.Module):
        t = type(fn)
        if t is nn.SiLU:
            return None if fn.inplace else _lib.BASE_SILU
        if t is nn.GELU:
            return {"none": _lib.BASE_GELU, "tanh": _lib.BASE_GELU_TANH}.get(fn.approximate)
        if t is nn.ReLU:
            return None if fn.inplace else _lib.BASE_RELU
        if t is nn.Tanh:
            return _lib.BASE_TANH
        if t is nn.Identity:
            return _lib.BASE_IDENTITY
        return None
    if fn is F.silu:
        return _lib.BASE_SILU
    if fn is F.gelu or fn is torch._C._nn.gelu:
        return _lib.BASE_GELU
    if fn is F.relu or fn is torch.relu:
        return _lib.BASE_RELU
    if fn is torch.tanh or fn is F.tanh:
        return _lib.BASE_TANH
    return None


def base_act_of(fn) -> int:
    code = base_activation_code(fn)
    if code is None:
        raise NotImplementedError(f"base_activation {fn!r} is not implemented by the fused kernels; supported: "
                                  f"{SUPPORTED_BASE_ACTIVATIONS}")
    return code


def _desc(cfg: LayerCfg, M: int, ldx: int, ldu: int, ldy: int, bp_stride: int) -> LayerDesc:
    return LayerDesc(cfg.family, cfg.groups, cfg.x_group_mod, cfg.I, cfg.O, cfg.G, cfg.spline_order, cfg.has_base,
                     cfg.rbf_inv_h, cfg.flags, M, ldx, ldu, ldy, bp_stride, cfg.ln_eps, cfg.base_act)


def _workspace(nbytes: int, device):
    return torch.empty(max((nbytes + 3) // 4, 4), device=device, dtype=torch.float32)


_fwd_f32 = torch.amp.custom_fwd(device_type="cuda", cast_inputs=torch.float32)
_bwd = torch.amp.custom_bwd(device_type="cuda")


class _KanLayerFn(torch.autograd.Function):

    @staticmethod
    @_fwd_f32
    def forward(ctx, x, u, w, bparams, bias, cfg: LayerCfg):
        for n, t in (("x", x), ("u", u), ("w", w), ("bparams", bparams), ("bias", bias)):
            _require_gpu_f32(n, t)
        x = x.contiguous()
        w = w.contiguous()
        u = None if u is None else u.contiguous()
        bparams = None if bparams is None else bparams.contiguous()
        bias = None if bias is None else bias.contiguous()
        M, ldx = x.shape
        if ldx != cfg.x_group_mod * cfg.I:
            raise KanvitError(f"x has {ldx} columns, expected x_group_mod*I = {cfg.x_group_mod * cfg.I}")
        if tuple(w.shape) != (cfg.groups, cfg.K, cfg.O):
            raise KanvitError(f"packed weight shape {tuple(w.shape)} != {(cfg.groups, cfg.K, cfg.O)}")
        if u is not None and tuple(u.shape) != (M, cfg.groups * cfg.I):
            raise KanvitError(f"u shape {tuple(u.shape)} != {(M, cfg.groups * cfg.I)}")
        y = torch.empty(M, cfg.groups * cfg.O, device=x.device, dtype=torch.float32)
        d = _desc(cfg, M, ldx, cfg.groups * cfg.I, cfg.groups * cfg.O, 0 if bparams is None else bparams.shape[1])
        tag = ("qkv" if cfg.groups > 1 else "layer") + "_fwd" + ("_bf16" if cfg.flags & _lib.FLAG_BF16_MFMA else "")
        with torch.cuda.device(x.device):
            nbytes = int(_lib.lib().kanvit_layer_fwd_workspace(C.byref(d)))
            ws = _workspace(nbytes, x.device) if nbytes else None
            with _timed(tag, *_layer_cost(cfg, M, "fwd")):
                check(_lib.lib().kanvit_layer_fwd(C.byref(d), _ptr(x), _ptr(u), _ptr(w), _ptr(bparams), _ptr(bias),
                                                  _ptr(y), _ptr(ws), C.c_size_t(nbytes), _stream()), "kanvit_layer_fwd")
        ctx.cfg = cfg
        ctx.has_u = u is not None
        ctx.has_bp = bparams is not None
        ctx.has_bias = bias is not None
        ctx.save_for_backward(x, u, w, bparams)
        return y

    @staticmethod
    @_bwd
    def backward(ctx, dy):
        x, u, w, bparams = ctx.saved_tensors
        return _kan_backward(ctx.cfg, x, u if ctx.has_u else None, w, bparams, dy.float().contiguous(), ctx.needs_input_grad[:5],
                             ctx.has_u, ctx.has_bias) + (None,)


def _kan_backward(cfg: "LayerCfg", x, u, w, bparams, dy, needs, has_u, has_bias, patch=None):
    if patch is not None:
        pd, M = patch
        ldx = cfg.I
        assert not (needs[0] or needs[1]), "the patch form has no input gradient"
    else:
        pd = None
        M, ldx = x.shape
    need_x, need_u, need_w, need_bp, need_b = needs
    d = _desc(cfg, M, ldx, cfg.groups * cfg.I, cfg.groups * cfg.O, 0 if bparams is None else bparams.shape[1])
    L = _lib.lib()

    def weight_pass(desc, out, tag):
        if pd is not None:
            nbytes = int(L.kanvit_patch_embed_bwd_weight_workspace(C.byref(desc), C.byref(pd)))
            ws = torch.empty(max(nbytes // 4, 1), device=x.device, dtype=torch.float32)
            with _timed(tag, *_layer_cost(cfg, M, "bwd_weight")):
                check(L.kanvit_patch_embed_bwd_weight(C.byref(desc), C.byref(pd), _ptr(x), _ptr(bparams), _ptr(dy), _ptr(out),
                                                      _ptr(ws), C.c_size_t(nbytes), _stream()), "kanvit_patch_embed_bwd_weight")
            return
        nbytes = int(L.kanvit_layer_bwd_weight_workspace(C.byref(desc)))
        ws = torch.empty(max(nbytes // 4, 1), device=x.device, dtype=torch.float32)
        with _timed(tag, *_layer_cost(cfg, M, "bwd_weight")):
            check(L.kanvit_layer_bwd_weight(C.byref(desc), _ptr(x), _ptr(u), _ptr(bparams), _ptr(dy), _ptr(out),
                                            _ptr(ws), C.c_size_t(nbytes), _stream()), "kanvit_layer_bwd_weight")

    dx = du = dw = dbp = db = None
    sine_freq = cfg.family == SINE and need_bp
    freq_via_w = False
    if sine_freq and not need_x and (pd is not None or not _lib.py_switches()["no_dfreq_w"]):
        with torch.cuda.device(x.device):
            freq_via_w = bool(L.kanvit_layer_sine_dfreq_ok(C.byref(d)))
    if pd is not None and sine_freq and not freq_via_w:
        raise KanvitError("patch form: SineKAN's frequency gradient needs the register weight-gradient kernel")
    with torch.cuda.device(x.device):
        if need_x or (need_u and has_u) or (sine_freq and not freq_via_w):
            dx = torch.empty_like(x)
            du_buf = torch.empty(M, cfg.groups * cfg.I, device=x.device, dtype=torch.float32) if cfg.family == RBF else None
            dpart = None
            if cfg.family == SINE:
                tiles = int(L.kanvit_layer_dparam_tiles(C.byref(d)))
                dpart = torch.empty(tiles, cfg.groups, cfg.G, device=x.device, dtype=torch.float32)
            nb_in = int(L.kanvit_layer_bwd_input_workspace(C.byref(d)))
            ws_in = _workspace(nb_in, x.device) if nb_in else None
            with _timed(("qkv" if cfg.groups > 1 else "layer") + "_bwd_input" + ("_bf16" if nb_in else ""),
                        *_layer_cost(cfg, M, "bwd_input")):
                check(L.kanvit_layer_bwd_input(C.byref(d), _ptr(x), _ptr(u), _ptr(w), _ptr(bparams), _ptr(dy),
                                               _ptr(dx), _ptr(du_buf), _ptr(dpart), _ptr(ws_in), C.c_size_t(nb_in),
                                               _stream()), "kanvit_layer_bwd_input")
            if cfg.family == RBF:
                if has_u:
                    du = du_buf
                else:
                    nshare = cfg.groups // cfg.x_group_mod
                    dx = dx + du_buf.view(M, nshare, cfg.x_group_mod * cfg.I).sum(1)
            if sine_freq:
                dbp = torch.zeros_like(bparams)
                dbp[:, :cfg.G] = dpart.sum(0)
        if need_w:
            dw = torch.empty_like(w)
            weight_pass(d, dw, ("qkv" if cfg.groups > 1 else "layer") + "_bwd_weight" + ("_bf16" if cfg.flags & 1 else ""))
        if freq_via_w:
            dq = LayerDesc(*[getattr(d, f) for f, _ in LayerDesc._fields_])
            dq.flags = cfg.flags | _lib.FLAG_SINE_DFREQ
            q = torch.empty_like(w)
            weight_pass(dq, q, ("qkv" if cfg.groups > 1 else "layer") + "_bwd_freq" + ("_bf16" if cfg.flags & 1 else ""))
            dbp = torch.zeros_like(bparams)
            dbp[:, :cfg.G] = q.mul_(w).view(cfg.groups, cfg.I, cfg.G, cfg.O).sum((1, 3))
        if need_b and has_bias:
            if pd is not None:
                db = dy[:, pd.prepend_rows:, :].sum((0, 1)).view(1, cfg.O)
            else:
                db = dy.view(M, cfg.groups, cfg.O).sum(0)
    return (dx if need_x else None), (du if need_u else None), dw, dbp, db


def ln_fusable(cfg: "LayerCfg", M: int) -> bool:
    if cfg.family != RBF:
        return False
    f = cfg.flags | (_lib.FLAG_BF16_MFMA if _autocast_flags() else 0)
    d = _desc(LayerCfg(**{**cfg.__dict__, "flags": f}), M, cfg.x_group_mod * cfg.I, cfg.groups * cfg.I, cfg.groups * cfg.O,
              cfg.G + 2 * cfg.I)
    return bool(_lib.lib().kanvit_layer_ln_fusable(C.byref(d)))


class _KanLayerLnFn(torch.autograd.Function):

    @staticmethod
    @_fwd_f32
    def forward(ctx, x, w, bparams, bias, cfg: LayerCfg):
        for n, t in (("x", x), ("w", w), ("bparams", bparams), ("bias", bias)):
            _require_gpu_f32(n, t)
        x, w, bparams = x.contiguous(), w.contiguous(), bparams.contiguous()
        bias = None if bias is None else bias.contiguous()
        M, ldx = x.shape
        if ldx != cfg.x_group_mod * cfg.I:
            raise KanvitError(f"x has {ldx} columns, expected x_group_mod*I = {cfg.x_group_mod * cfg.I}")
        if tuple(w.shape) != (cfg.groups, cfg.K, cfg.O):
            raise KanvitError(f"packed weight shape {tuple(w.shape)} != {(cfg.groups, cfg.K, cfg.O)}")
        if tuple(bparams.shape) != (cfg.groups, cfg.G + 2 * cfg.I):
            raise KanvitError(f"bparams shape {tuple(bparams.shape)} != {(cfg.groups, cfg.G + 2 * cfg.I)} (centres | gamma | beta)")
        y = torch.empty(M, cfg.groups * cfg.O, device=x.device, dtype=torch.float32)
        stats = torch.empty(M, cfg.x_group_mod, 2, device=x.device, dtype=torch.float32)
        d = _desc(cfg, M, ldx, cfg.groups * cfg.I, cfg.groups * cfg.O, bparams.shape[1])
        tag = ("qkv" if cfg.groups > 1 else "layer") + "_fwd" + ("_bf16" if cfg.flags & _lib.FLAG_BF16_MFMA else "")
        with torch.cuda.device(x.device):
            nbytes = int(_lib.lib().kanvit_layer_fwd_workspace(C.byref(d)))
            ws = _workspace(nbytes, x.device) if nbytes else None
            with _timed(tag, *_layer_cost(cfg, M, "fwd")):
                check(_lib.lib().kanvit_layer_fwd(C.byref(d), _ptr(x), _ptr(stats), _ptr(w), _ptr(bparams), _ptr(bias),
                                                  _ptr(y), _ptr(ws), C.c_size_t(nbytes), _stream()), "kanvit_layer_fwd")
        ctx.cfg = cfg
        ctx.has_bias = bias is not None
        ctx.save_for_backward(x, stats, w, bparams)
        return y

    @staticmethod
    @_bwd
    def backward(ctx, dy):
        x, stats, w, bparams = ctx.saved_tensors
        cfg = ctx.cfg
        need_x, need_w, need_bp, need_b = ctx.needs_input_grad[:4]
        need_ln = need_x or need_bp
        dx, du, dw, _, db = _kan_backward(cfg, x, stats, w, bparams, dy.float().contiguous(),
                                          (need_ln, need_ln, need_w, False, need_b), True, ctx.has_bias)
        dbp = None
        if need_ln:
            M, I, G = x.shape[0], cfg.I, cfg.G
            d = _desc(cfg, M, x.shape[1], cfg.groups * I, cfg.groups * cfg.O, bparams.shape[1])
            L = _lib.lib()
            dgb = torch.empty(2, cfg.groups, I, device=x.device, dtype=torch.float32)
            with torch.cuda.device(x.device):
                nbytes = int(L.kanvit_layer_ln_bwd_workspace(C.byref(d)))
                ws = _workspace(nbytes, x.device)
                with _timed("ln_bwd", 0, 4 * M * (cfg.groups * I + (3 if need_x else 1) * cfg.x_group_mod * I)):
                    check(L.kanvit_layer_ln_bwd(C.byref(d), _ptr(x), _ptr(stats), _ptr(bparams), _ptr(du), _ptr(dx if need_x else None),
                                                _ptr(dgb[0]), _ptr(dgb[1]), _ptr(ws), C.c_size_t(nbytes), _stream()), "kanvit_layer_ln_bwd")
            if need_bp:
                dbp = torch.cat([torch.zeros(cfg.groups, G, device=x.device, dtype=torch.float32), dgb[0], dgb[1]], dim=1)
        return (dx if need_x else None), dw, dbp, db, None


def kan_layer_ln(x: torch.Tensor, w: torch.Tensor, cfg: LayerCfg, bparams: torch.Tensor, bias: Optional[torch.Tensor],
                 eps: float) -> torch.Tensor:
    from dataclasses import replace
    f = cfg.flags | _lib.FLAG_FUSED_LN | (_lib.FLAG_BF16_MFMA if _autocast_flags() else 0)
    return _KanLayerLnFn.apply(x, w, bparams, bias, replace(cfg, flags=f, ln_eps=float(eps)))


def patchify(images: torch.Tensor, n_patches: int) -> torch.Tensor:
    b, c, h, w = images.shape
    ph, pw = h // n_patches, w // n_patches
    return images.reshape(b, c, n_patches, ph, n_patches, pw).permute(0, 2, 4, 1, 3, 5).reshape(b, n_patches * n_patches, c * ph * pw)


class _PatchEmbedFn(torch.autograd.Function):

    @staticmethod
    @_fwd_f32
    def forward(ctx, images, w, bparams, bias, cls, pos, cfg: LayerCfg, n_patches: int):
        for n, t in (("images", images), ("w", w), ("bparams", bparams), ("bias", bias), ("cls", cls), ("pos", pos)):
            _require_gpu_f32(n, t)
        images = images.contiguous()
        w = w.contiguous()
        B, Cc, H, W = images.shape
        P = n_patches * n_patches
        y = torch.empty(B, P + 1, cfg.O, device=images.device, dtype=torch.float32)
        d = _desc(cfg, B * P, cfg.I, cfg.I, cfg.O, 0 if bparams is None else bparams.shape[1])
        pd = _lib.PatchDesc(Cc, H, W, n_patches, 1, 0)
        bp = None if bparams is None else bparams.contiguous()
        bs = None if bias is None else bias.contiguous()
        cl, po = cls.contiguous(), pos.contiguous()
        bf = bool(cfg.flags & _lib.FLAG_BF16_MFMA)
        with torch.cuda.device(images.device):
            nbytes = int(_lib.lib().kanvit_layer_fwd_workspace(C.byref(d))) if bf else 0
            ws = _workspace(nbytes, images.device) if nbytes else None
            with _timed("layer_fwd" + ("_bf16" if bf else ""), *_layer_cost(cfg, B * P, "fwd")):
                check(_lib.lib().kanvit_patch_embed_fwd_ws(C.byref(d), C.byref(pd), _ptr(images), _ptr(w), _ptr(bp), _ptr(bs), _ptr(cl),
                                                            _ptr(po), _ptr(y), _ptr(ws), C.c_size_t(nbytes), _stream()),
                      "kanvit_patch_embed_fwd")
        ctx.cfg, ctx.n_patches = cfg, n_patches
        ctx.has_bp, ctx.has_bias = bparams is not None, bias is not None
        ctx.save_for_backward(images, w, bp)
        return y

    @staticmethod
    @_bwd
    def backward(ctx, dy):
        images, w, bparams = ctx.saved_tensors
        cfg, P = ctx.cfg, ctx.n_patches ** 2
        dy = dy.float().contiguous()
        B, Cc, H, W = images.shape
        dcls = dy[:, 0, :].sum(0) if ctx.needs_input_grad[4] else None
        needs = (False, False, ctx.needs_input_grad[1], ctx.needs_input_grad[2] and ctx.has_bp, ctx.needs_input_grad[3] and ctx.has_bias)
        pd = _lib.PatchDesc(Cc, H, W, ctx.n_patches, 1, 0)
        d = _desc(cfg, B * P, cfg.I, cfg.I, cfg.O, 0 if bparams is None else bparams.shape[1])
        with torch.cuda.device(images.device):
            gather = bool(_lib.lib().kanvit_patch_embed_bwd_weight_ok(C.byref(d), C.byref(pd))) and not _lib.py_switches()["no_patch_bw"]
        if cfg.family == SINE and _lib.py_switches()["no_dfreq_w"]:
            gather = False
        if gather:
            _, _, dw, dbp, db = _kan_backward(cfg, images, None, w, bparams, dy, needs, False, ctx.has_bias, patch=(pd, B * P))
        else:
            x = patchify(images, ctx.n_patches).reshape(-1, cfg.I)
            dyt = dy[:, 1:, :].reshape(-1, cfg.O)
            _, _, dw, dbp, db = _kan_backward(cfg, x, None, w, bparams, dyt, needs, False, ctx.has_bias)
        return None, dw, dbp, db, dcls, None, None, None


def patch_embed(images, w, cfg: LayerCfg, bparams, bias, cls, pos, n_patches: int) -> torch.Tensor:
    if _autocast_flags() and not (cfg.flags & _lib.FLAG_BF16_MFMA):
        from dataclasses import replace
        cfg = replace(cfg, flags=cfg.flags | _lib.FLAG_BF16_MFMA)
    return _PatchEmbedFn.apply(images, w, bparams, bias, cls, pos, cfg, n_patches)


def kan_layer(x: torch.Tensor, w: torch.Tensor, cfg: LayerCfg, u: Optional[torch.Tensor] = None,
              bparams: Optional[torch.Tensor] = None, bias: Optional[torch.Tensor] = None) -> torch.Tensor:
    if torch.is_autocast_enabled("cuda") and torch.get_autocast_dtype("cuda") == torch.bfloat16 and not (cfg.flags & 1):
        from dataclasses import replace
        cfg = replace(cfg, flags=cfg.flags | _lib.FLAG_BF16_MFMA)
    return _KanLayerFn.apply(x, u, w, bparams, bias, cfg)


EDGE_L1_FAMILIES = (BSPLINE, CHEBY, RBF)


def _edge_l1_desc(cfg: LayerCfg, x: torch.Tensor, bparams) -> LayerDesc:
    M, cols = x.shape
    two = cfg.family == RBF and cfg.has_base
    want = cfg.x_group_mod * cfg.I * (2 if two else 1)
    if cols != want:
        raise KanvitError(f"edge_l1: x has {cols} columns, expected {want}" + (" ([u | x] for RBF with the base column)" if two else ""))
    ldx = max(x.stride(0), cols) if M > 1 else cols
    return _desc(cfg, M, ldx, cfg.x_group_mod * cfg.I if two else 0, cfg.groups * cfg.O, 0 if bparams is None else bparams.shape[1])


class _EdgeL1Fn(torch.autograd.Function):

    @staticmethod
    @_fwd_f32
    def forward(ctx, x, w, bparams, cfg: LayerCfg):
        for n, t in (("x", x), ("w", w), ("bparams", bparams)):
            _require_gpu_f32(n, t)
        if x.dim() != 2:
            raise KanvitError(f"edge_l1: x must be 2-D, got {tuple(x.shape)}")
        if x.stride(1) != 1 or (x.shape[0] > 1 and x.stride(0) < x.shape[1]):
            x = x.contiguous()
        w = w.contiguous()
        bparams = None if bparams is None else bparams.contiguous()
        if tuple(w.shape) != (cfg.groups, cfg.K, cfg.O):
            raise KanvitError(f"packed weight shape {tuple(w.shape)} != {(cfg.groups, cfg.K, cfg.O)}")
        d = _edge_l1_desc(cfg, x, bparams)
        L = _lib.lib()
        A = torch.empty(cfg.groups, cfg.I, cfg.O, device=x.device, dtype=torch.float32)
        with torch.cuda.device(x.device):
            nbytes = int(L.kanvit_edge_l1_fwd_workspace(C.byref(d)))
            ws = _workspace(nbytes, x.device)
            with _timed("edge_l1_fwd", 2 * x.shape[0] * cfg.K * cfg.O * cfg.groups, 4 * (x.numel() + w.numel() + A.numel())):
                check(L.kanvit_edge_l1_fwd(C.byref(d), _ptr(x), _ptr(w), _ptr(bparams), _ptr(A), _ptr(ws), C.c_size_t(nbytes), _stream()),
                      "kanvit_edge_l1_fwd")
        ctx.cfg = cfg
        ctx.save_for_backward(x, w, bparams)
        return A

    @staticmethod
    @_bwd
    def backward(ctx, gA):
        x, w, bparams = ctx.saved_tensors
        cfg = ctx.cfg
        gA = gA.float().contiguous()
        d = _edge_l1_desc(cfg, x, bparams)
        L = _lib.lib()
        dw = torch.empty_like(w)
        dx = torch.empty_strided(x.shape, (d.ldx, 1), device=x.device, dtype=torch.float32) if ctx.needs_input_grad[0] else None
        with torch.cuda.device(x.device):
            nbytes = int(L.kanvit_edge_l1_bwd_workspace(C.byref(d)))
            ws = _workspace(nbytes, x.device)
            with _timed("edge_l1_bwd", (6 if dx is not None else 4) * x.shape[0] * cfg.K * cfg.O * cfg.groups,
                        4 * ((1 if dx is None else 2) * x.numel() + 2 * w.numel() + gA.numel())):
                check(L.kanvit_edge_l1_bwd(C.byref(d), _ptr(x), _ptr(w), _ptr(bparams), _ptr(gA), _ptr(dw), _ptr(dx), _ptr(ws),
                                           C.c_size_t(nbytes), _stream()), "kanvit_edge_l1_bwd")
        return dx, dw, None, None


def edge_l1(x2d: torch.Tensor, w_packed: torch.Tensor, cfg: LayerCfg, bparams: Optional[torch.Tensor] = None) -> torch.Tensor:
    if cfg.family not in EDGE_L1_FAMILIES:
        raise NotImplementedError(f"edge_l1: family {_lib.FAMILY_NAMES[cfg.family]} is not supported (supported: bspline, cheby, rbf)")
    keep = _lib.FLAG_UNIFORM_KNOTS | _lib.FLAG_SHARED_BPARAMS
    if cfg.flags & ~keep:
        from dataclasses import replace
        cfg = replace(cfg, flags=cfg.flags & keep)
    return _EdgeL1Fn.apply(x2d, w_packed, bparams, cfg)


def l1_entropy_loss(l1: torch.Tensor, regularize_activation: float = 1.0, regularize_entropy: float = 1.0) -> torch.Tensor:
    total = l1.sum((-2, -1), keepdim=True)
    p = l1 / total
    per_layer = regularize_activation * total.squeeze(-1).squeeze(-1) - regularize_entropy * torch.special.xlogy(p, p).sum((-2, -1))
    return per_layer.sum()


@torch.no_grad()
def bspline_refit(x2d: torch.Tensor, w_old_packed: torch.Tensor, cfg: LayerCfg, old_knots: torch.Tensor,
                  new_knots: torch.Tensor) -> Tuple[torch.Tensor, torch.Tensor]:
    if cfg.family != BSPLINE:
        raise NotImplementedError(f"bspline_refit: family {_lib.FAMILY_NAMES[cfg.family]} has no knot table to refit (bspline only)")
    from dataclasses import replace
    cfg = replace(cfg, flags=cfg.flags & (_lib.FLAG_UNIFORM_KNOTS | _lib.FLAG_SHARED_BPARAMS))
    for n, t in (("x", x2d), ("w_old", w_old_packed), ("old_knots", old_knots), ("new_knots", new_knots)):
        _require_gpu_f32(n, t)
    x = x2d
    if x.dim() != 2:
        raise KanvitError(f"bspline_refit: x must be 2-D, got {tuple(x.shape)}")
    if x.shape[1] != cfg.x_group_mod * cfg.I:
        raise KanvitError(f"bspline_refit: x has {x.shape[1]} columns, expected {cfg.x_group_mod * cfg.I}")
    if x.stride(1) != 1 or (x.shape[0] > 1 and x.stride(0) < x.shape[1]):
        x = x.contiguous()
    M = x.shape[0]
    ldx = max(x.stride(0), x.shape[1]) if M > 1 else x.shape[1]
    nb, nk = cfg.G, cfg.G + cfg.spline_order + 1
    w_old = w_old_packed.contiguous()
    if tuple(w_old.shape) != (cfg.groups, cfg.I * nb, cfg.O):
        raise KanvitError(f"bspline_refit: packed weight shape {tuple(w_old.shape)} != {(cfg.groups, cfg.I * nb, cfg.O)}")
    old_knots = old_knots.reshape(cfg.groups, -1).contiguous()
    new_knots = new_knots.contiguous()
    if old_knots.shape[1] < cfg.I * nk or tuple(new_knots.shape) != (cfg.x_group_mod, cfg.I, nk):
        raise KanvitError(f"bspline_refit: knot tables {tuple(old_knots.shape)} / {tuple(new_knots.shape)} do not hold "
                          f"[{cfg.groups}][{cfg.I}*{nk}] / [{cfg.x_group_mod}][{cfg.I}][{nk}]")
    d = _desc(cfg, M, ldx, 0, cfg.groups * cfg.O, old_knots.shape[1])
    L = _lib.lib()
    dev = x.device
    gram_n = torch.empty(cfg.x_group_mod, cfg.I, nb, nb, device=dev, dtype=torch.float64)
    gram_c = torch.empty(cfg.groups, cfg.I, nb, nb, device=dev, dtype=torch.float64)
    w_new = w_old.clone()
    ok = torch.empty(cfg.x_group_mod, cfg.I, device=dev, dtype=torch.uint8)
    with torch.cuda.device(dev):
        nbytes = int(L.kanvit_bspline_refit_workspace(C.byref(d)))
        ws = _workspace(nbytes, dev)
        with _timed("bspline_refit", 2 * M * (cfg.groups + cfg.x_group_mod) * cfg.I * nb * nb, 4 * (x.numel() + 2 * w_old.numel())):
            check(L.kanvit_bspline_refit_gram(C.byref(d), _ptr(x), _ptr(old_knots), _ptr(new_knots), _ptr(gram_n), _ptr(gram_c), _ptr(ws),
                                              C.c_size_t(nbytes), _stream()), "kanvit_bspline_refit_gram")
            check(L.kanvit_bspline_refit_solve(C.byref(d), _ptr(gram_n), _ptr(gram_c), _ptr(w_old), _ptr(w_new), _ptr(ok), _stream()),
                  "kanvit_bspline_refit_solve")
    return w_new, ok.bool()


@torch.no_grad()
def bspline_regrid(x2d: torch.Tensor, w_old_packed: torch.Tensor, cfg_new: LayerCfg, old_G: int, old_knots: torch.Tensor,
                   new_knots: torch.Tensor) -> Tuple[torch.Tensor, torch.Tensor]:
    if cfg_new.family != BSPLINE:
        raise NotImplementedError(f"bspline_regrid: family {_lib.FAMILY_NAMES[cfg_new.family]} has no knot table to refit (bspline only)")
    from dataclasses import replace
    cfg = replace(cfg_new, flags=cfg_new.flags & (_lib.FLAG_UNIFORM_KNOTS | _lib.FLAG_SHARED_BPARAMS))
    old_G = int(old_G)
    for n, t in (("x", x2d), ("w_old", w_old_packed), ("old_knots", old_knots), ("new_knots", new_knots)):
        _require_gpu_f32(n, t)
    x = x2d
    if x.dim() != 2:
        raise KanvitError(f"bspline_regrid: x must be 2-D, got {tuple(x.shape)}")
    if x.shape[1] != cfg.x_group_mod * cfg.I:
        raise KanvitError(f"bspline_regrid: x has {x.shape[1]} columns, expected {cfg.x_group_mod * cfg.I}")
    if x.stride(1) != 1 or (x.shape[0] > 1 and x.stride(0) < x.shape[1]):
        x = x.contiguous()
    M = x.shape[0]
    ldx = max(x.stride(0), x.shape[1]) if M > 1 else x.shape[1]
    nb, nk = cfg.G, cfg.G + cfg.spline_order + 1
    nbo, nko = old_G, old_G + cfg.spline_order + 1
    w_old = w_old_packed.contiguous()
    if tuple(w_old.shape) != (cfg.groups, cfg.I * nbo, cfg.O):
        raise KanvitError(f"bspline_regrid: old packed weight shape {tuple(w_old.shape)} != {(cfg.groups, cfg.I * nbo, cfg.O)} "
                          f"(old nb={nbo})")
    if old_knots.dim() < 1 or old_knots.shape[0] != cfg.groups:
        raise KanvitError(f"bspline_regrid: old knot table {tuple(old_knots.shape)} does not hold [{cfg.groups}][{cfg.I}*{nko}]")
    old_knots = old_knots.reshape(cfg.groups, -1).contiguous()
    new_knots = new_knots.contiguous()
    if old_knots.shape[1] < cfg.I * nko:
        raise KanvitError(f"bspline_regrid: old knot table {tuple(old_knots.shape)} does not hold [{cfg.groups}][{cfg.I}*{nko}]")
    if tuple(new_knots.shape) != (cfg.x_group_mod, cfg.I, nk):
        raise KanvitError(f"bspline_regrid: new knot table {tuple(new_knots.shape)} != [{cfg.x_group_mod}][{cfg.I}][{nk}]")
    d = _desc(cfg, M, ldx, 0, cfg.groups * cfg.O, old_knots.shape[1])
    L = _lib.lib()
    dev = x.device
    og = C.c_int(old_G)
    gram_n = torch.empty(cfg.x_group_mod, cfg.I, nb, nb, device=dev, dtype=torch.float64)
    gram_c = torch.empty(cfg.groups, cfg.I, nb, nbo, device=dev, dtype=torch.float64)
    w_new = torch.zeros(cfg.groups, cfg.I * nb, cfg.O, device=dev, dtype=torch.float32)
    ok = torch.empty(cfg.x_group_mod, cfg.I, device=dev, dtype=torch.uint8)
    with torch.cuda.device(dev):
        nbytes = int(L.kanvit_bspline_regrid_workspace(C.byref(d), og))
        ws = _workspace(nbytes, dev)
        with _timed("bspline_regrid", 2 * M * cfg.I * nb * (cfg.groups * nbo + cfg.x_group_mod * nb), 4 * (x.numel() + w_old.numel() + w_new.numel())):
            check(L.kanvit_bspline_regrid_gram(C.byref(d), og, _ptr(x), _ptr(old_knots), _ptr(new_knots), _ptr(gram_n), _ptr(gram_c), _ptr(ws),
                                               C.c_size_t(nbytes), _stream()), "kanvit_bspline_regrid_gram")
            check(L.kanvit_bspline_regrid_solve(C.byref(d), og, _ptr(gram_n), _ptr(gram_c), _ptr(w_old), _ptr(w_new), _ptr(ok), _stream()),
                  "kanvit_bspline_regrid_solve")
    return w_new, ok.bool()


_attn_flags = 0


def _attn_build_desc(q, k, v, o, causal: bool, scale: float, flags: int, self_attention: bool) -> AttnDesc:
    B, H, Nq, D = q.shape
    Nk = Nq if self_attention else k.shape[2]
    for n, t, L in (("q", q, Nq), ("k", k, Nk), ("v", v, Nk), ("o", o, Nq)):
        if t.dim() != 4 or tuple(t.shape) != (B, H, L, D):
            if not self_attention:
                raise KanvitError(f"attention: q {tuple(q.shape)}, k {tuple(k.shape)}, v {tuple(v.shape)}, o {tuple(o.shape)} do not agree")
            raise KanvitError(f"attention: {n} has shape {tuple(t.shape)}, expected {(B, H, L, D)} "
                              "(self-attention only: q, k, v and o must agree in batch, heads, length and head size)")
        if t.stride(3) != 1:
            raise KanvitError(f"{n}: innermost dimension must be contiguous")
    return AttnDesc(B, H, Nq, D, int(bool(causal)), float(scale), int(flags), 0,
                    q.stride(0), q.stride(1), q.stride(2), k.stride(0), k.stride(1), k.stride(2),
                    v.stride(0), v.stride(1), v.stride(2), o.stride(0), o.stride(1), o.stride(2))


def _attn_desc(q, k, v, o, causal: bool, scale: float, flags: int = 0) -> AttnDesc:
    return _attn_build_desc(q, k, v, o, causal, scale, flags, True)


def _attn_fits_one_workgroup(N: int, D: int) -> bool:
    if D > 64:
        return False
    ks, npad = (32 if D <= 32 else 64) + 1, (N + 31) // 32 * 32
    return N <= 256 and 4 * (2 * npad * ks + 2 * npad + 4 * 32 * ks) <= 160 * 1024


def _attn_x_flags(flags: int, D: int) -> int:
    return flags & _lib.FLAG_BF16_MFMA if D <= 64 else 0


def _attn_takes_general_kernels(q, k) -> bool:
    return q.dim() == 4 and tuple(k.shape) == tuple(q.shape) and not _attn_fits_one_workgroup(q.shape[2], q.shape[3])


def _attn_fwd(q, k, v, o, causal, scale, flags=0):
    if _attn_takes_general_kernels(q, k):
        return _attn_x_fwd(q, k, v, o, None, causal, scale, flags=_attn_x_flags(flags, q.shape[3]))
    B, H, N, _ = q.shape
    lse = torch.empty(B, H, N, device=q.device, dtype=torch.float32)
    d = _attn_desc(q, k, v, o, causal, scale, flags)
    flops, nbytes = 4 * B * H * N * N * q.shape[3], 4 * 4 * B * H * N * q.shape[3]
    with torch.cuda.device(q.device), _timed("attn_fwd" + ("_bf16" if flags & 1 else ""), flops, nbytes):
        check(_lib.lib().kanvit_attn_fwd(C.byref(d), _ptr(q), _ptr(k), _ptr(v), _ptr(o), _ptr(lse), _stream()),
              "kanvit_attn_fwd")
    return lse


def _attn_bwd(q, k, v, o, lse, do, dq, dk, dv, causal, scale, flags=0):
    if _attn_takes_general_kernels(q, k):
        return _attn_x_bwd(q, k, v, o, lse, do, dq, dk, dv, None, causal, scale, flags=_attn_x_flags(flags, q.shape[3]))
    d = _attn_desc(q, k, v, o, causal, scale, flags)
    if (do.stride() != o.stride()) or dq.stride() != q.stride() or dk.stride() != k.stride() or dv.stride() != v.stride():
        raise KanvitError("attention backward: gradient layouts must match their forward tensors")
    L = _lib.lib()
    nbytes = int(L.kanvit_attn_bwd_workspace(C.byref(d)))
    ws = torch.empty(max(nbytes // 4, 1), device=q.device, dtype=torch.float32)
    B, H, N, D = q.shape
    with torch.cuda.device(q.device), _timed("attn_bwd" + ("_bf16" if flags & 1 else ""), 10 * B * H * N * N * D, 4 * 9 * B * H * N * D):
        check(L.kanvit_attn_bwd(C.byref(d), _ptr(q), _ptr(k), _ptr(v), _ptr(o), _ptr(lse), _ptr(do), _ptr(dq), _ptr(dk),
                                _ptr(dv), _ptr(ws), C.c_size_t(nbytes), _stream()), "kanvit_attn_bwd")


def _attn_x_desc(q, k, v, o, mask, causal: bool, scale: float, flags: int = 0):
    for n, t in (("q", q), ("k", k), ("v", v), ("o", o)):
        _require_gpu_f32(n, t)
    d = _attn_build_desc(q, k, v, o, causal, scale, flags, False)
    B, H, Nq, Nk = d.B, d.H, d.N, k.shape[2]
    if mask is None:
        e = _lib.AttnExt(Nk, 0, None, 0, 0, 0, 0)
    else:
        if mask.dtype != torch.bool or not mask.is_cuda or tuple(mask.shape) != (B, H, Nq, Nk):
            raise KanvitError(f"attention mask: need a torch.bool GPU tensor expanded to {(B, H, Nq, Nk)}, got {mask.dtype} {tuple(mask.shape)}")
        e = _lib.AttnExt(Nk, 0, mask.data_ptr(), mask.stride(0), mask.stride(1), mask.stride(2), mask.stride(3))
    return d, e


def _attn_x_fwd(q, k, v, o, mask, causal, scale, flags=0):
    B, H, Nq, D = q.shape
    lse = torch.empty(B, H, Nq, device=q.device, dtype=torch.float32)
    d, e = _attn_x_desc(q, k, v, o, mask, causal, scale, flags)
    Nk = k.shape[2]
    tag = "attn_x_fwd" + ("_bf16" if flags & _lib.FLAG_BF16_MFMA else "")
    with torch.cuda.device(q.device), _timed(tag, 4 * B * H * Nq * Nk * D, 4 * 2 * B * H * (Nq + Nk) * D):
        check(_lib.lib().kanvit_attn_x_fwd(C.byref(d), C.byref(e), _ptr(q), _ptr(k), _ptr(v), _ptr(o), _ptr(lse), _stream()), "kanvit_attn_x_fwd")
    return lse


def _attn_x_bwd(q, k, v, o, lse, do, dq, dk, dv, mask, causal, scale, flags=0):
    d, e = _attn_x_desc(q, k, v, o, mask, causal, scale, flags)
    if (do.stride() != o.stride()) or dq.stride() != q.stride() or dk.stride() != k.stride() or dv.stride() != v.stride():
        raise KanvitError("attention backward: gradient layouts must match their forward tensors")
    L = _lib.lib()
    nbytes = int(L.kanvit_attn_x_bwd_workspace(C.byref(d), C.byref(e)))
    ws = torch.empty(max(nbytes // 4, 1), device=q.device, dtype=torch.float32)
    B, H, Nq, D = q.shape
    Nk = k.shape[2]
    tag = "attn_x_bwd" + ("_bf16" if flags & _lib.FLAG_BF16_MFMA else "")
    with torch.cuda.device(q.device), _timed(tag, 14 * B * H * Nq * Nk * D, 4 * 4 * B * H * (Nq + Nk) * D):
        check(L.kanvit_attn_x_bwd(C.byref(d), C.byref(e), _ptr(q), _ptr(k), _ptr(v), _ptr(o), _ptr(lse), _ptr(do), _ptr(dq), _ptr(dk),
                                  _ptr(dv), _ptr(ws), C.c_size_t(nbytes), _stream()), "kanvit_attn_x_bwd")


class _AttnPackedFn(torch.autograd.Function):

    @staticmethod
    @_fwd_f32
    def forward(ctx, qkv, causal: bool, scale: float, flags: int = 0):
        _require_gpu_f32("qkv", qkv)
        qkv = qkv.contiguous()
        B, N, three, H, D = qkv.shape
        q, k, v = (qkv[:, :, i].permute(0, 2, 1, 3) for i in range(3))
        o = torch.empty(B, N, H, D, device=qkv.device, dtype=torch.float32)
        lse = _attn_fwd(q, k, v, o.permute(0, 2, 1, 3), causal, scale, flags)
        ctx.save_for_backward(qkv, o, lse)
        ctx.causal, ctx.scale, ctx.flags = causal, scale, flags
        return o.view(B, N, H * D)

    @staticmethod
    @_bwd
    def backward(ctx, do):
        do = do.float()
        qkv, o, lse = ctx.saved_tensors
        B, N, _, H, D = qkv.shape
        do = do.contiguous().view(B, N, H, D)
        dqkv = torch.empty_like(qkv)
        q, k, v = (qkv[:, :, i].permute(0, 2, 1, 3) for i in range(3))
        dq, dk, dv = (dqkv[:, :, i].permute(0, 2, 1, 3) for i in range(3))
        _attn_bwd(q, k, v, o.permute(0, 2, 1, 3), lse, do.permute(0, 2, 1, 3), dq, dk, dv, ctx.causal, ctx.scale, ctx.flags)
        return dqkv, None, None, None


class _AttnFn(torch.autograd.Function):

    @staticmethod
    @_fwd_f32
    def forward(ctx, q, k, v, causal: bool, scale: float, flags: int = 0):
        for n, t in (("q", q), ("k", k), ("v", v)):
            _require_gpu_f32(n, t)
        q, k, v = (t if t.stride(3) == 1 else t.contiguous() for t in (q, k, v))
        o = torch.empty(q.shape, device=q.device, dtype=torch.float32)
        lse = _attn_fwd(q, k, v, o, causal, scale, flags)
        ctx.save_for_backward(q, k, v, o, lse)
        ctx.causal, ctx.scale, ctx.flags = causal, scale, flags
        return o

    @staticmethod
    @_bwd
    def backward(ctx, do):
        q, k, v, o, lse = ctx.saved_tensors
        do = do.float().contiguous()
        dq, dk, dv = (torch.empty_strided(t.shape, t.stride(), device=t.device, dtype=t.dtype) for t in (q, k, v))
        _attn_bwd(q, k, v, o, lse, do, dq, dk, dv, ctx.causal, ctx.scale, ctx.flags)
        return dq, dk, dv, None, None, None


def _autocast_flags() -> int:
    on = torch.is_autocast_enabled("cuda") and torch.get_autocast_dtype("cuda") == torch.bfloat16
    return _lib.FLAG_BF16_MFMA if on else 0


def attention_packed(qkv: torch.Tensor, causal: bool = False, scale: Optional[float] = None) -> torch.Tensor:
    return _AttnPackedFn.apply(qkv, causal, qkv.shape[-1] ** -0.5 if scale is None else scale, _autocast_flags())


def attention(q: torch.Tensor, k: torch.Tensor, v: torch.Tensor, causal: bool = False,
              scale: Optional[float] = None) -> torch.Tensor:
    return _AttnFn.apply(q, k, v, causal, q.shape[-1] ** -0.5 if scale is None else scale, _autocast_flags())


def expand_attention_mask(mask: Optional[torch.Tensor], q: torch.Tensor, k: torch.Tensor) -> Optional[torch.Tensor]:
    if mask is None:
        return None
    if mask.dim() == 2:
        mask = mask[:, None, None, :]
    return mask.to(device=q.device, dtype=torch.bool).expand(q.shape[0], q.shape[1], q.shape[2], k.shape[2])


def _attn_probs(q, k, mask, causal, scale, rows):
    for n, t in (("q", q), ("k", k)):
        _require_gpu_f32(n, t)
        if t.dim() != 4:
            raise KanvitError(f"attention_probs: {n} has shape {tuple(t.shape)}, expected [B, H, length, D]")
    B, H, Nq, D = q.shape
    if tuple(k.shape[:2]) != (B, H) or k.shape[3] != D:
        raise KanvitError(f"attention_probs: q {tuple(q.shape)} and k {tuple(k.shape)} do not agree in batch, heads and head size")
    Nk = k.shape[2]
    q, k = (t if t.stride(3) == 1 else t.contiguous() for t in (q, k))
    mask = expand_attention_mask(mask, q, k)
    scale = D ** -0.5 if scale is None else scale
    rows = Nq if rows is None else int(rows)
    if not 1 <= rows <= Nq:
        raise KanvitError(f"attention_probs: rows={rows} must be in [1, {Nq}]")
    if B == 0:
        return torch.empty(B, H, rows, Nk, device=q.device, dtype=torch.float32)
    d = AttnDesc(B, H, Nq, D, int(bool(causal)), float(scale), 0, 0, q.stride(0), q.stride(1), q.stride(2),
                 k.stride(0), k.stride(1), k.stride(2), 0, 0, 0, 0, 0, 0)
    if mask is None:
        e = _lib.AttnExt(Nk, 0, None, 0, 0, 0, 0)
    else:
        e = _lib.AttnExt(Nk, 0, mask.data_ptr(), mask.stride(0), mask.stride(1), mask.stride(2), mask.stride(3))
    p = torch.empty(B, H, rows, Nk, device=q.device, dtype=torch.float32)
    with torch.cuda.device(q.device), _timed("attn_probs", 6 * B * H * rows * Nk * D, 4 * B * H * (rows * Nk + rows * D + Nk * D)):
        check(_lib.lib().kanvit_attn_probs(C.byref(d), C.byref(e), _ptr(q), _ptr(k), _ptr(p), p.stride(0), p.stride(1), p.stride(2),
                                           rows, _stream()), "kanvit_attn_probs")
    return p


@torch.no_grad()
def attention_probs(q: torch.Tensor, k: torch.Tensor, mask: Optional[torch.Tensor] = None, causal: bool = False,
                    scale: Optional[float] = None, rows: Optional[int] = None) -> torch.Tensor:
    with torch.autocast("cuda", enabled=False):
        q, k = (t.float() if t.is_cuda and t.is_floating_point() else t for t in (q, k))
        return _attn_probs(q, k, mask, causal, scale, rows)


@torch.no_grad()
def attention_probs_packed(qkv: torch.Tensor, causal: bool = False, scale: Optional[float] = None,
                           rows: Optional[int] = None) -> torch.Tensor:
    with torch.autocast("cuda", enabled=False):
        if qkv.is_cuda and qkv.is_floating_point():
            qkv = qkv.float()
        _require_gpu_f32("qkv", qkv)
        if qkv.dim() != 5 or qkv.shape[2] != 3:
            raise KanvitError(f"attention_probs_packed: qkv has shape {tuple(qkv.shape)}, expected [B, N, 3, H, D]")
        qkv = qkv.contiguous()
        q, k = (qkv[:, :, i].permute(0, 2, 1, 3) for i in range(2))
        return _attn_probs(q, k, None, causal, scale, rows)


class _AddLayerNormFn(torch.autograd.Function):

    @staticmethod
    @torch.amp.custom_fwd(device_type="cuda")
    def forward(ctx, x, delta, gamma, beta, eps, y_bf16):
        if not x.is_cuda:
            raise KanvitError(f"x is on {x.device}: the kanvit ops run only on an AMD GPU (no CPU fallback)")
        L = _lib.lib()
        D = x.shape[-1]
        x2 = x.float().contiguous().view(-1, D)
        d2 = None
        if delta is not None:
            d2 = (delta if delta.dtype in (torch.float32, torch.bfloat16) else delta.float()).contiguous().view(-1, D)
        M = x2.shape[0]
        y = torch.empty(M, D, device=x.device, dtype=torch.bfloat16 if y_bf16 else torch.float32)
        s = torch.empty_like(x2) if d2 is not None else x2
        mean = torch.empty(M, device=x.device, dtype=torch.float32)
        rstd = torch.empty(M, device=x.device, dtype=torch.float32)
        g, b = gamma.float().contiguous(), beta.float().contiguous()
        with torch.cuda.device(x.device):
            check(L.kanvit_addln_fwd_ex(M, D, float(eps), _ptr(x2), _ptr(d2), int(d2 is not None and d2.dtype == torch.bfloat16), _ptr(g), _ptr(b),
                                        _ptr(s) if d2 is not None else None, _ptr(y), int(bool(y_bf16)), _ptr(mean), _ptr(rstd), _stream()),
                  "kanvit_addln_fwd")
        ctx.save_for_backward(s, g, mean, rstd)
        ctx.delta_dtype = None if d2 is None else d2.dtype
        ctx.shape = x.shape
        return s.view(x.shape), y.view(x.shape)

    @staticmethod
    @torch.amp.custom_bwd(device_type="cuda")
    def backward(ctx, gs, gy):
        s, g, mean, rstd = ctx.saved_tensors
        L = _lib.lib()
        M, D = s.shape
        if gy is None:
            gy2 = torch.zeros_like(s)
        else:
            gy2 = gy.contiguous().view(M, D)
            if gy2.dtype != torch.bfloat16:
                gy2 = gy2.float()
        gs2 = None if gs is None else gs.contiguous().view(M, D).float()
        dx = torch.empty_like(s)
        dxb = torch.empty(M, D, device=s.device, dtype=torch.bfloat16) if ctx.delta_dtype == torch.bfloat16 else None
        dg = torch.empty(D, device=s.device, dtype=torch.float32)
        db = torch.empty(D, device=s.device, dtype=torch.float32)
        nbytes = int(L.kanvit_addln_bwd_workspace(M, D))
        ws = _workspace(nbytes, s.device)
        with torch.cuda.device(s.device):
            check(L.kanvit_addln_bwd_ex(M, D, _ptr(s), _ptr(g), _ptr(mean), _ptr(rstd), _ptr(gy2), int(gy2.dtype == torch.bfloat16), _ptr(gs2),
                                        _ptr(dx), _ptr(dxb), _ptr(dg), _ptr(db), _ptr(ws), C.c_size_t(nbytes), _stream()), "kanvit_addln_bwd")
        dx = dx.view(ctx.shape)
        dd = None if ctx.delta_dtype is None else (dxb.view(ctx.shape) if dxb is not None else dx)
        return dx, dd, dg, db, None, None


def add_layernorm(x: torch.Tensor, delta: Optional[torch.Tensor], norm: torch.nn.LayerNorm, y_bf16: bool = False):
    D = x.shape[-1]
    if norm.weight is None or norm.bias is None or len(norm.normalized_shape) != 1 or D % 4 or D > 1024 or D < 4:
        s = x if delta is None else x + delta
        return s, norm(s)
    return _AddLayerNormFn.apply(x, delta, norm.weight, norm.bias, norm.eps, bool(y_bf16))
```

kan-vit_amd/model.py:

```python
import torch
import torch.nn as nn

from attention import MSA, FlashAttention
from kanvit import ops
from kanvit.dense import feed_forward, ff_mode, ff_small_supported, ln_feed_forward
from kanvit.ops import add_layernorm
from models.cheby import ChebyKANLayer
from models.effkan import KANLinear
from models.fastkan import FastKANLayer
from models.nfkan import NaiveFourierKANLayer
from models.sinekan import SineKANLayer


class TransformerBlock(nn.Module):

    def __init__(self, d_model, n_heads, feedforward_dim=128, attn_type="vanilla"):
        super().__init__()
        self.norm1 = nn.LayerNorm(d_model)
        self.attn = MSA(d_model, n_heads, type=attn_type)
        self.norm2 = nn.LayerNorm(d_model)
        self.ff = nn.Sequential(nn.Linear(d_model, feedforward_dim), nn.ReLU(inplace=True),
                                nn.Linear(feedforward_dim, d_model))

    def forward(self, x):
        x, f = self.run(x, None)
        return x + f

    @torch.no_grad()
    def attention_map(self, x, rows=None):
        return self.attn.attention_map(self.norm1(x), rows)

    def run(self, x, pending, reg=None):
        x, h1 = add_layernorm(x, pending, self.norm1)
        if reg is not None:
            return self._rest(x, h1) + (self.attn.regularization_loss(h1, **reg),)
        return self._rest(x, h1)

    def _rest(self, x, h1):
        if x.dim() == 3 and ff_small_supported(self.ff[0].in_features, self.ff[0].out_features):
            return ln_feed_forward(x, self.attn(h1), self.norm2, self.ff[0], self.ff[2])
        ybf = (x.is_cuda and torch.is_autocast_enabled("cuda") and torch.get_autocast_dtype("cuda") == torch.bfloat16 and ff_mode() != "bf16x3")
        x, h2 = add_layernorm(x, self.attn(h1), self.norm2, y_bf16=ybf)
        b, n, d = x.shape
        return x, feed_forward(h2.reshape(b * n, d), self.ff[0], self.ff[2]).view(b, n, d)


class _ClsToken(torch.autograd.Function):

    @staticmethod
    def forward(ctx, out, pending):
        ctx.shape = out.shape
        ctx.pdtype = pending.dtype
        return out[:, 0] + pending[:, 0]

    @staticmethod
    def backward(ctx, g):
        full = torch.nn.functional.pad(g.unsqueeze(1), (0, 0, 0, ctx.shape[1] - 1))
        return full, (full if ctx.pdtype == full.dtype else full.to(ctx.pdtype))


def _patch_embedding(kind, in_dim, d):
    if kind in ("vanilla", "flash-attn"):
        return nn.Linear(in_dim, d)
    if kind == "efficientkan":
        return KANLinear(in_dim, d)
    if kind == "sine":
        return SineKANLayer(in_dim, d, grid_size=28)
    if kind == "fourier":
        return NaiveFourierKANLayer(in_dim, d, grid_size=28)
    if kind == "cheby":
        return ChebyKANLayer(in_dim, d, 4)
    if kind == "fast":
        return FastKANLayer(in_dim, d)
    raise ValueError(f"Unknown transformer type: {kind}")


def split_types(kind: str):
    kinds = [k.strip() for k in kind.replace("+", ",").split(",") if k.strip()]
    if not kinds:
        raise ValueError(f"Unknown transformer type: {kind}")
    if len(kinds) > 1 and any(k in ("flash-attn",) for k in kinds):
        raise ValueError("'flash-attn' stacks bare FlashAttention modules (model.py:113-117) and cannot be mixed per block")
    return kinds


def patch_embedding_type(model) -> str:
    lm = model.linear_mapper
    return {KANLinear: "efficientkan", ChebyKANLayer: "cheby", FastKANLayer: "fast", SineKANLayer: "sine",
            NaiveFourierKANLayer: "fourier"}.get(type(lm), "vanilla")


class VisionTransformer(nn.Module):
    def __init__(self, chw, n_patches=7, n_blocks=4, d_hidden=64, n_heads=2, out_d=10, type: str = "vanilla"):
        super().__init__()
        kinds = split_types(type)
        self.block_types = [kinds[l % len(kinds)] for l in range(n_blocks)]
        type = kinds[0]
        self.chw = chw
        self.n_patches = n_patches
        self.n_blocks = n_blocks
        self.n_heads = n_heads
        self.d_hidden = d_hidden
        assert chw[1] % n_patches == 0
        assert chw[2] % n_patches == 0
        self.patch_size = (chw[1] // n_patches, chw[2] // n_patches)
        self.input_d = int(chw[0] * self.patch_size[0] * self.patch_size[1])

        self.linear_mapper = _patch_embedding(type, self.input_d, d_hidden)
        self.v_class = nn.Parameter(torch.randn(1, d_hidden))
        self.register_buffer('pos_embeddings', self.positional_embeddings(n_patches ** 2 + 1, d_hidden),
                             persistent=False)
        if type == "flash-attn":
            self.blocks = nn.ModuleList([FlashAttention(dim=d_hidden, heads=n_heads) for _ in range(n_blocks)])
        else:
            self.blocks = nn.ModuleList([TransformerBlock(d_hidden, n_heads, feedforward_dim=4 * d_hidden,
                                                          attn_type=self.block_types[l]) for l in range(n_blocks)])
        self.mlp_head = nn.Sequential(nn.LayerNorm(d_hidden), nn.Linear(d_hidden, out_d))
        self._fused_embed = None

    def patchify(self, images, n_patches):
        b, c, h, w = images.shape
        ph, pw = h // n_patches, w // n_patches
        t = images.reshape(b, c, n_patches, ph, n_patches, pw).permute(0, 2, 4, 1, 3, 5)
        return t.reshape(b, n_patches * n_patches, c * ph * pw)

    def positional_embeddings(self, seq_length, d):
        i = torch.arange(seq_length, dtype=torch.float64).unsqueeze(1)
        j = torch.arange(d, dtype=torch.float64).unsqueeze(0)
        ang = i / torch.pow(torch.tensor(10000.0, dtype=torch.float64), j / d)
        even = (torch.arange(d) % 2 == 0).unsqueeze(0)
        return torch.where(even, torch.sin(ang), torch.cos(ang)).to(torch.float32)

    def _embed_fused(self, images):
        lm = self.linear_mapper
        if isinstance(lm, nn.Linear) or not hasattr(lm, "kan_pack") or hasattr(lm, "kan_u"):
            return None
        mode = bool(torch.is_autocast_enabled("cuda") and torch.get_autocast_dtype("cuda") == torch.bfloat16)
        if self._fused_embed is None:
            self._fused_embed = {}
        if self._fused_embed.get(mode) is False:
            return None
        if (not images.is_cuda or images.dim() != 4 or images.dtype != torch.float32 or images.requires_grad
                or (images.is_contiguous() and images.data_ptr() % 16)):
            return None
        cfg = lm.kan_cfg()
        w, bp, bias = lm.kan_pack()
        try:
            out = ops.patch_embed(images, w.unsqueeze(0), cfg, None if bp is None else bp.unsqueeze(0),
                                  None if bias is None else bias.reshape(1, -1), self.v_class.reshape(-1),
                                  self.pos_embeddings[: self.n_patches ** 2 + 1], self.n_patches)
        except ops.KanvitError:
            if mode not in self._fused_embed:
                self._fused_embed[mode] = False
                return None
            raise
        self._fused_embed[mode] = True
        return out

    def _embed(self, images, patches=None):
        out = self._embed_fused(images)
        if out is None:
            if patches is None:
                patches = self.patchify(images, self.n_patches)
            b, p, _ = patches.shape
            if isinstance(self.linear_mapper, nn.Linear):
                tokens = self.linear_mapper(patches)
            else:
                tokens = self.linear_mapper(patches).reshape(b, p, self.d_hidden)
            cls = self.v_class.unsqueeze(0).expand(b, -1, -1)
            out = torch.cat((cls, tokens), dim=1) + self.pos_embeddings[: p + 1]
        return out

    @torch.no_grad()
    def update_grid(self, images, margin=0.01):
        kan_blocks = [isinstance(blk, TransformerBlock) and isinstance(blk.attn.q_mappings[0], KANLinear) for blk in self.blocks]
        if not isinstance(self.linear_mapper, KANLinear) and not any(kan_blocks):
            raise NotImplementedError(f"update_grid: model type(s) {sorted(self.layer_types())} have no KANLinear, the only layer "
                                      "with a B-spline grid to update ('efficientkan')")
        kept = torch.zeros((), dtype=torch.int64, device=images.device)
        if isinstance(self.linear_mapper, KANLinear):
            kept = kept + self.linear_mapper.update_grid(self.patchify(images, self.n_patches).reshape(-1, self.input_d), margin)
        self._fused_embed = None
        out = self._embed(images)
        for blk, is_kan in zip(self.blocks, kan_blocks):
            if is_kan:
                kept = kept + blk.attn.update_grid(blk.norm1(out), margin)
            if blk is not self.blocks[-1]:
                out = blk(out)
        self._fused_embed = None
        return kept

    @torch.no_grad()
    def extend_grid(self, images, grid_size, margin=0.01):
        kan_blocks = [isinstance(blk, TransformerBlock) and isinstance(blk.attn.q_mappings[0], KANLinear) for blk in self.blocks]
        if not isinstance(self.linear_mapper, KANLinear) and not any(kan_blocks):
            raise NotImplementedError(f"extend_grid: model type(s) {sorted(self.layer_types())} have no KANLinear, the only layer "
                                      "with a B-spline grid to extend ('efficientkan')")
        for m in self.modules():
            if isinstance(m, KANLinear):
                KANLinear.check_extension(grid_size, m.spline_order)
        fell_back = torch.zeros((), dtype=torch.int64, device=images.device)
        if isinstance(self.linear_mapper, KANLinear):
            fell_back = fell_back + self.linear_mapper.extend_grid(self.patchify(images, self.n_patches).reshape(-1, self.input_d),
                                                                   grid_size, margin)
        self._fused_embed = None
        out = self._embed(images)
        for blk, is_kan in zip(self.blocks, kan_blocks):
            if is_kan:
                fell_back = fell_back + blk.attn.extend_grid(blk.norm1(out), grid_size, margin)
            if blk is not self.blocks[-1]:
                out = blk(out)
        self._fused_embed = None
        return fell_back

    def _walk_attention_maps(self, images, rows):
        out = self._embed(images)
        for blk in self.blocks:
            yield blk.attention_map(out, rows=rows)
            if blk is not self.blocks[-1]:
                out = blk(out)

    @torch.no_grad()
    def attention_maps(self, images, rows=None):
        return torch.stack(list(self._walk_attention_maps(images, rows)))

    @staticmethod
    def _rollout_factor(block_map, head_fusion):
        if block_map.dim() != 4 or block_map.shape[-1] != block_map.shape[-2]:
            raise ValueError(f"rollout needs full attention maps [.., B, H, N, N] (rows=None), got a block of shape {tuple(block_map.shape)}")
        a = block_map.float()
        if head_fusion == "mean":
            a = a.mean(dim=1)
        elif head_fusion == "max":
            a = a.amax(dim=1)
        elif head_fusion == "min":
            a = a.amin(dim=1)
        else:
            raise ValueError(f"head_fusion must be 'mean', 'max' or 'min', got {head_fusion!r}")
        a = a + torch.eye(a.shape[-1], dtype=a.dtype, device=a.device)
        return a / a.sum(dim=-1, keepdim=True)

    @staticmethod
    def rollout(maps, head_fusion="mean"):
        if maps.dim() != 5:
            raise ValueError(f"rollout needs maps [n_blocks, B, H, N, N], got shape {tuple(maps.shape)}")
        with torch.autocast(maps.device.type, enabled=False):
            out = None
            for block_map in maps:
                f = VisionTransformer._rollout_factor(block_map, head_fusion)
                out = f if out is None else f @ out
        return out

    @torch.no_grad()
    def attention_rollout(self, images, head_fusion="mean"):
        out = None
        for block_map in self._walk_attention_maps(images, None):
            with torch.autocast(block_map.device.type, enabled=False):
                f = self._rollout_factor(block_map, head_fusion)
                out = f if out is None else f @ out
        return out

    def cls_saliency(self, rollout):
        return rollout[:, 0, 1:].reshape(-1, self.n_patches, self.n_patches)

    REGULARIZED_TYPES = MSA.REGULARIZED_TYPES

    def layer_types(self):
        return set(self.block_types) | {patch_embedding_type(self)}

    def forward(self, images, return_regularization=False, regularize_activation=1.0, regularize_entropy=1.0):
        reg, reg_kw, patches = None, None, None
        if return_regularization:
            kinds = self.layer_types()
            if not kinds <= set(self.REGULARIZED_TYPES):
                raise NotImplementedError(f"return_regularization: model type(s) {sorted(kinds - set(self.REGULARIZED_TYPES))} have no "
                                          f"edge-activation regulariser; supported: {', '.join(self.REGULARIZED_TYPES)}")
            reg_kw = dict(regularize_activation=regularize_activation, regularize_entropy=regularize_entropy)
            patches = self.patchify(images, self.n_patches)
            rows = patches.reshape(-1, self.input_d)
            if isinstance(self.linear_mapper, KANLinear):
                reg = self.linear_mapper.regularization_loss(x=rows, **reg_kw)
            else:
                reg = self.linear_mapper.regularization_loss(rows, **reg_kw)
        out = self._embed(images, patches)
        pending = None
        for blk in self.blocks:
            if isinstance(blk, TransformerBlock) and reg_kw is not None:
                out, pending, r = blk.run(out, pending, reg_kw)
                reg = reg + r
            elif isinstance(blk, TransformerBlock):
                out, pending = blk.run(out, pending)
            else:
                out = blk(out)
        if pending is not None:
            out = _ClsToken.apply(out, pending)
        else:
            out = out[:, 0]
        if return_regularization:
            return self.mlp_head(out), reg
        return self.mlp_head(out)
```

kan-vit_amd/models/fastkan.py:

```python
import torch
import torch.nn as nn
import torch.nn.functional as F

from kanvit import grouped, ops


_RBF_FACTS = {}


def _rbf_grid_is_default(layers) -> bool:
    key = tuple((id(m), m.rbf.grid._version, m.rbf.grid.data_ptr(), float(m.rbf.denominator)) for m in layers)
    hit = _RBF_FACTS.get(key)
    if hit is None:
        l0 = layers[0]
        g = l0.rbf.grid.detach().double()
        h = float(l0.rbf.denominator)
        ok = g.numel() == 8 and h > 0
        if ok:
            ideal = g[0] + h * torch.arange(8, device=g.device, dtype=torch.float64)
            ok = float((g - ideal).abs().max()) <= 2e-6 * (float(g.abs().max()) + 1.0)
        ok = ok and all(float(m.rbf.denominator) == h and m.rbf.grid.shape == l0.rbf.grid.shape and bool((m.rbf.grid == l0.rbf.grid).all())
                        for m in layers[1:])
        if len(_RBF_FACTS) > 256:
            _RBF_FACTS.clear()
        hit = _RBF_FACTS[key] = bool(ok)
    return hit


class SplineLinear(nn.Linear):

    def __init__(self, in_features: int, out_features: int, init_scale: float = 0.1, **kw) -> None:
        self.init_scale = init_scale
        super().__init__(in_features, out_features, bias=False, **kw)

    def reset_parameters(self) -> None:
        nn.init.trunc_normal_(self.weight, mean=0, std=self.init_scale)


class RadialBasisFunction(nn.Module):

    def __init__(self, grid_min: float = -2., grid_max: float = 2., num_grids: int = 8, denominator: float = None):
        super().__init__()
        self.grid = torch.nn.Parameter(torch.linspace(grid_min, grid_max, num_grids), requires_grad=False)
        self.denominator = denominator or (grid_max - grid_min) / (num_grids - 1)

    def forward(self, x):
        eye = torch.eye(self.grid.numel(), device=x.device, dtype=x.dtype)
        n = self.grid.numel()
        cfg = ops.LayerCfg(family=ops.RBF, I=1, O=n, G=n, has_base=0, rbf_inv_h=1.0 / self.denominator)
        y = ops.kan_layer(x.reshape(-1, 1), eye.unsqueeze(0), cfg, bparams=self.grid.reshape(1, -1))
        return y.reshape(*x.shape, n)


class FastKANLayer(nn.Module):

    def __init__(self, input_dim: int, output_dim: int, grid_min: float = -2., grid_max: float = 2.,
                 num_grids: int = 8, use_base_update: bool = True, base_activation=F.silu,
                 spline_weight_init_scale: float = 0.1) -> None:
        super().__init__()
        self.input_dim, self.output_dim, self.num_grids = input_dim, output_dim, num_grids
        self.layernorm = nn.LayerNorm(input_dim)
        self.rbf = RadialBasisFunction(grid_min, grid_max, num_grids)
        self.spline_linear = SplineLinear(input_dim * num_grids, output_dim, spline_weight_init_scale)
        self.use_base_update = use_base_update
        if use_base_update:
            ops.base_act_of(base_activation)
            self.base_activation = base_activation
            self.base_linear = nn.Linear(input_dim, output_dim)

    def kan_cfg(self, layers=None):
        from kanvit import _lib
        uni = _rbf_grid_is_default(layers if layers is not None else [self])
        return ops.LayerCfg(family=ops.RBF, I=self.input_dim, O=self.output_dim, G=self.num_grids,
                            has_base=int(self.use_base_update), rbf_inv_h=1.0 / float(self.rbf.denominator),
                            flags=_lib.FLAG_UNIFORM_KNOTS if uni else 0,
                            base_act=ops.base_act_of(self.base_activation) if self.use_base_update else 0)

    def kan_pack(self):
        i, g, o = self.input_dim, self.num_grids, self.output_dim
        w = self.spline_linear.weight.view(o, i, g).permute(1, 2, 0)
        bias = None
        if self.use_base_update:
            w = torch.cat([w, self.base_linear.weight.t().unsqueeze(1)], dim=1)
            bias = self.base_linear.bias
        return w.reshape(-1, o), self.rbf.grid.detach(), bias

    @staticmethod
    def kan_pack_grouped(layers):
        l0 = layers[0]
        i, gr, o = l0.input_dim, l0.num_grids, l0.output_dim
        g = len(layers)
        w = grouped.stack_params([m.spline_linear.weight for m in layers]).view(g, o, i, gr).permute(0, 2, 3, 1)
        bias = None
        if l0.use_base_update:
            bw = grouped.stack_params([m.base_linear.weight for m in layers]).permute(0, 2, 1).unsqueeze(2)
            w = torch.cat([w, bw], dim=2)
            bias = grouped.stack_params([m.base_linear.bias for m in layers])
        return w.reshape(g, -1, o), torch.stack([m.rbf.grid.detach() for m in layers]), bias

    def kan_u(self, x2d):
        return self.layernorm(x2d) if getattr(self, "_use_ln", True) else None

    def kan_ln(self):
        return self.layernorm if getattr(self, "_use_ln", True) else None

    @staticmethod
    def kan_u_grouped(layers, x2d, n_heads):
        M = x2d.shape[0]
        dh = layers[0].input_dim
        xhat = F.layer_norm(x2d.view(M, n_heads, dh), (dh,), None, None, layers[0].layernorm.eps)
        gamma = grouped.stack_params([l.layernorm.weight for l in layers]).view(1, 3, n_heads, dh)
        beta = grouped.stack_params([l.layernorm.bias for l in layers]).view(1, 3, n_heads, dh)
        return torch.addcmul(beta, xhat.unsqueeze(1), gamma).reshape(M, 3 * n_heads * dh)

    def edge_activation_l1(self, x, include_base=False):
        from dataclasses import replace
        i, g, o = self.input_dim, self.num_grids, self.output_dim
        x2d = x if x.dim() == 2 else x.reshape(-1, i)
        u = self.layernorm(x2d)
        cfg = self.kan_cfg()
        if self.use_base_update and include_base:
            w, bp, _ = self.kan_pack()
            xin = torch.cat([u, x2d.to(u.dtype)], dim=1)
        else:
            cfg = replace(cfg, has_base=0, base_act=0)
            w, bp, xin = self.spline_linear.weight.view(o, i, g).permute(1, 2, 0).reshape(-1, o), self.rbf.grid.detach(), u
        return ops.edge_l1(xin, w.unsqueeze(0), cfg, bp.unsqueeze(0))[0].t()

    def regularization_loss(self, x, regularize_activation=1.0, regularize_entropy=1.0, include_base=False):
        return ops.l1_entropy_loss(self.edge_activation_l1(x, include_base), regularize_activation, regularize_entropy)

    def forward(self, x, time_benchmark=False):
        self._use_ln = not time_benchmark
        try:
            y = grouped.run_single(self, x.reshape(-1, self.input_dim))
        finally:
            self._use_ln = True
        return y.reshape(*x.shape[:-1], self.output_dim)
```

Measured before the change: 1514.

## Compute only the CLS row in the final transformer block

In the last transformer block only the CLS token reaches the classifier head, so Q projection, attention, the residual/LN and the feed-forward run for that single row. K and V are still projected for every token. New single-query attention forward and backward kernels are added, and the backward pass scatters gradients back by zero-padding. The path is skipped when regularization is on, when the small-FF path applies, or when KANVIT_NO_CLS_TAIL is set.

```diff
diff --git a/include/kanvit.h b/include/kanvit.h
--- a/include/kanvit.h
+++ b/include/kanvit.h
@@ -163,6 +163,11 @@
 
 int kanvit_attn_probs(const kanvit_attn_desc* d, const kanvit_attn_ext* e, const float* q, const float* k, float* p,
                       int64_t p_stride_b, int64_t p_stride_h, int64_t p_stride_q, int32_t rows, void* stream);
+
+int kanvit_attn_q1_fwd(const kanvit_attn_desc* d, const kanvit_attn_ext* e, const float* q, const float* k, const float* v,
+                       float* o, float* p, void* stream);
+int kanvit_attn_q1_bwd(const kanvit_attn_desc* d, const kanvit_attn_ext* e, const float* q, const float* k, const float* v,
+                       const float* o, const float* p, const float* d_o, float* dq, float* dk, float* dv, void* stream);
 
 int kanvit_ff_small_supported(int D, int F);
 int64_t kanvit_ff_small_max_rows(void);
diff --git a/kan-vit_amd/attention.py b/kan-vit_amd/attention.py
--- a/kan-vit_amd/attention.py
+++ b/kan-vit_amd/attention.py
@@ -178,3 +178,11 @@
         qkv = grouped.run_qkv(self.q_mappings, self.k_mappings, self.v_mappings, sequences.reshape(b * n, d))
         return ops.attention_packed(qkv.view(b, n, 3, self.n_heads, self.d_head), causal=False,
                                     scale=1.0 / (self.d_head ** 0.5))
+
+    def forward_cls(self, sequences):
+        b, n, d = sequences.shape
+        q0 = grouped.run_projections([self.q_mappings], sequences[:, 0], tag="qcls")
+        kv = grouped.run_projections([self.k_mappings, self.v_mappings], sequences.reshape(b * n, d), tag="kv")
+        o = ops.attention_q1(q0.view(b, self.n_heads, self.d_head), kv.view(b, n, 2, self.n_heads, self.d_head),
+                             scale=1.0 / (self.d_head ** 0.5))
+        return o.view(b, d)
diff --git a/kan-vit_amd/csrc/attention_x.hip b/kan-vit_amd/csrc/attention_x.hip
--- a/kan-vit_amd/csrc/attention_x.hip
+++ b/kan-vit_amd/csrc/attention_x.hip
@@ -867,9 +867,287 @@
     return 0;
 }
 
+struct AttnQ1Args {
+    const float* q;
+    const float* k;
+    const float* v;
+    const float* o_in;
+    const float* d_o;
+    float* o;
+    float* p;
+    float* dq;
+    float* dk;
+    float* dv;
+    long long qsb, qsh, ksb, ksh, ksn, vsb, vsh, vsn, osb, osh;
+    int H, Nk, D;
+    float scale;
+};
+
+constexpr int Q1_THR = 256, Q1_GROUPS = Q1_THR / 16;
+
+template <int V>
+struct Q1Frag {
+    static constexpr int T = KANVIT_ATTN_X_MAX_D / (16 * V);
+    float f[T][V];
+};
+
+template <int V>
+__device__ __forceinline__ void q1_zero(Q1Frag<V>& r) {
+#pragma unroll
+    for (int t = 0; t < Q1Frag<V>::T; ++t)
+#pragma unroll
+        for (int e = 0; e < V; ++e) r.f[t][e] = 0.0f;
+}
+
+template <int V>
+__device__ __forceinline__ void q1_load(Q1Frag<V>& r, const float* __restrict__ row, int sub, int D) {
+#pragma unroll
+    for (int t = 0; t < Q1Frag<V>::T; ++t) {
+        const int c = (t * 16 + sub) * V;
+        if (c < D) {
+            if constexpr (V == 4) {
+                const f32x4 u = *reinterpret_cast<const f32x4*>(row + c);
+#pragma unroll
+                for (int e = 0; e < 4; ++e) r.f[t][e] = u[e];
+            } else if constexpr (V == 2) {
+                const float2 u = *reinterpret_cast<const float2*>(row + c);
+                r.f[t][0] = u.x;
+                r.f[t][1] = u.y;
+            } else {
+                r.f[t][0] = row[c];
+            }
+        } else {
+#pragma unroll
+            for (int e = 0; e < V; ++e) r.f[t][e] = 0.0f;
+        }
+    }
+}
+
+template <int V>
+__device__ __forceinline__ void q1_store(float* __restrict__ row, const Q1Frag<V>& r, float mul, int sub, int D) {
+#pragma unroll
+    for (int t = 0; t < Q1Frag<V>::T; ++t) {
+        const int c = (t * 16 + sub) * V;
+        if (c < D) {
+            if constexpr (V == 4) {
+                const f32x4 u = {mul * r.f[t][0], mul * r.f[t][1], mul * r.f[t][2], mul * r.f[t][3]};
+                *reinterpret_cast<f32x4*>(row + c) = u;
+            } else if constexpr (V == 2) {
+                *reinterpret_cast<float2*>(row + c) = make_float2(mul * r.f[t][0], mul * r.f[t][1]);
+            } else {
+                row[c] = mul * r.f[t][0];
+            }
+        }
+    }
+}
+
+template <int V>
+__device__ __forceinline__ float q1_dot(const Q1Frag<V>& a, const Q1Frag<V>& b) {
+    float s = 0.0f;
+#pragma unroll
+    for (int t = 0; t < Q1Frag<V>::T; ++t)
+#pragma unroll
+        for (int e = 0; e < V; ++e) s = fmaf(a.f[t][e], b.f[t][e], s);
+    s += __shfl_xor(s, 8);
+    s += __shfl_xor(s, 4);
+    s += __shfl_xor(s, 2);
+    s += __shfl_xor(s, 1);
+    return s;
+}
+
+template <int V>
+__device__ __forceinline__ void q1_axpy(Q1Frag<V>& acc, float a, const Q1Frag<V>& x) {
+#pragma unroll
+    for (int t = 0; t < Q1Frag<V>::T; ++t)
+#pragma unroll
+        for (int e = 0; e < V; ++e) acc.f[t][e] = fmaf(a, x.f[t][e], acc.f[t][e]);
+}
+
+template <int V>
+__device__ __forceinline__ void q1_reduce_groups(float* __restrict__ red, const Q1Frag<V>& acc, float* __restrict__ out, float mul,
+                                                 int tid, int D) {
+    const int sub = tid & 15, grp = tid >> 4;
+#pragma unroll
+    for (int t = 0; t < Q1Frag<V>::T; ++t) {
+        const int c = (t * 16 + sub) * V;
+        if (c < D) {
+#pragma unroll
+            for (int e = 0; e < V; ++e) red[grp * KANVIT_ATTN_X_MAX_D + c + e] = acc.f[t][e];
+        }
+    }
+    __syncthreads();
+    if (tid < D) {
+        float s = 0.0f;
+#pragma unroll
+        for (int g = 0; g < Q1_GROUPS; ++g) s += red[g * KANVIT_ATTN_X_MAX_D + tid];
+        out[tid] = mul * s;
+    }
+}
+
+template <bool IS_MAX>
+__device__ __forceinline__ float q1_block_reduce(float x, float* __restrict__ wred, int tid) {
+#pragma unroll
+    for (int m = 32; m >= 1; m >>= 1) {
+        const float y = __shfl_xor(x, m);
+        x = IS_MAX ? fmaxf(x, y) : x + y;
+    }
+    __syncthreads();
+    if ((tid & 63) == 0) wred[tid >> 6] = x;
+    __syncthreads();
+    float r = wred[0];
+#pragma unroll
+    for (int w = 1; w < Q1_THR / 64; ++w) r = IS_MAX ? fmaxf(r, wred[w]) : r + wred[w];
+    return r;
+}
+
+template <int V>
+__global__ __launch_bounds__(Q1_THR) void attn_q1_fwd_kernel(const AttnQ1Args a) {
+    __shared__ float red[Q1_GROUPS * KANVIT_ATTN_X_MAX_D];
+    __shared__ float wred[Q1_THR / 64];
+    const int tid = threadIdx.x, sub = tid & 15, grp = tid >> 4;
+    const long long bh = blockIdx.x, bi = bh / a.H, hi = bh - bi * a.H;
+    const int D = a.D, Nk = a.Nk;
+    const float* kb = a.k + bi * a.ksb + hi * a.ksh;
+    const float* vb = a.v + bi * a.vsb + hi * a.vsh;
+    float* pb = a.p + bh * Nk;
+
+    Q1Frag<V> qf;
+    q1_load<V>(qf, a.q + bi * a.qsb + hi * a.qsh, sub, D);
+
+    float mx = -INFINITY;
+    for (int j = grp; j < Nk; j += Q1_GROUPS) {
+        Q1Frag<V> kf;
+        q1_load<V>(kf, kb + (long long)j * a.ksn, sub, D);
+        const float s = a.scale * q1_dot<V>(qf, kf);
+        if (sub == 0) pb[j] = s;
+        mx = fmaxf(mx, s);
+    }
+    mx = q1_block_reduce<true>(mx, wred, tid);
+
+    float sum = 0.0f;
+    for (int j = tid; j < Nk; j += Q1_THR) {
+        const float e = expf(pb[j] - mx);
+        pb[j] = e;
+        sum += e;
+    }
+    sum = q1_block_reduce<false>(sum, wred, tid);
+    const float inv = 1.0f / sum;
+
+    Q1Frag<V> oacc;
+    q1_zero<V>(oacc);
+    for (int j = grp; j < Nk; j += Q1_GROUPS) {
+        Q1Frag<V> vf;
+        q1_load<V>(vf, vb + (long long)j * a.vsn, sub, D);
+        q1_axpy<V>(oacc, pb[j] * inv, vf);
+    }
+    q1_reduce_groups<V>(red, oacc, a.o + bi * a.osb + hi * a.osh, 1.0f, tid, D);
+    for (int j = tid; j < Nk; j += Q1_THR) pb[j] *= inv;
+}
+
+template <int V>
+__global__ __launch_bounds__(Q1_THR) void attn_q1_bwd_kernel(const AttnQ1Args a) {
+    __shared__ float red[Q1_GROUPS * KANVIT_ATTN_X_MAX_D];
+    const int tid = threadIdx.x, sub = tid & 15, grp = tid >> 4;
+    const long long bh = blockIdx.x, bi = bh / a.H, hi = bh - bi * a.H;
+    const int D = a.D, Nk = a.Nk;
+    const float* kb = a.k + bi * a.ksb + hi * a.ksh;
+    const float* vb = a.v + bi * a.vsb + hi * a.vsh;
+    float* dkb = a.dk + bi * a.ksb + hi * a.ksh;
+    float* dvb = a.dv + bi * a.vsb + hi * a.vsh;
+    const float* pb = a.p + bh * Nk;
+
+    Q1Frag<V> qf, dof, of;
+    q1_load<V>(qf, a.q + bi * a.qsb + hi * a.qsh, sub, D);
+    q1_load<V>(dof, a.d_o + bi * a.osb + hi * a.osh, sub, D);
+    q1_load<V>(of, a.o_in + bi * a.osb + hi * a.osh, sub, D);
+    const float delta = q1_dot<V>(dof, of);
+
+    Q1Frag<V> dqacc;
+    q1_zero<V>(dqacc);
+    for (int j = grp; j < Nk; j += Q1_GROUPS) {
+        Q1Frag<V> kf, vf;
+        q1_load<V>(vf, vb + (long long)j * a.vsn, sub, D);
+        q1_load<V>(kf, kb + (long long)j * a.ksn, sub, D);
+        const float pj = pb[j];
+        const float ds = pj * (q1_dot<V>(dof, vf) - delta);
+        q1_store<V>(dvb + (long long)j * a.vsn, dof, pj, sub, D);
+        q1_store<V>(dkb + (long long)j * a.ksn, qf, a.scale * ds, sub, D);
+        q1_axpy<V>(dqacc, ds, kf);
+    }
+    q1_reduce_groups<V>(red, dqacc, a.dq + bi * a.qsb + hi * a.qsh, a.scale, tid, D);
+}
+
+int q1_check(const kanvit_attn_desc* d, const kanvit_attn_ext* e, const char* who) {
+    if (!d || !e) return kv_fail(KANVIT_EINVAL, "%s: null descriptor", who);
+    if (d->B < 0 || d->H < 1 || e->Nk < 1 || d->D < 1) return kv_fail(KANVIT_EINVAL, "%s: bad sizes", who);
+    if (d->N != 1) return kv_fail(KANVIT_EINVAL, "%s: q_len=%d, this entry takes ONE query per head (kanvit_attn_x_* take any)", who, d->N);
+    if (d->D > KANVIT_ATTN_X_MAX_D || (d->D & 1)) return kv_fail(KANVIT_EINVAL, "%s: D=%d must be even and <= %d", who, d->D, KANVIT_ATTN_X_MAX_D);
+    if ((long long)d->B * d->H > 0x7fffffffLL) return kv_fail(KANVIT_EINVAL, "%s: B*H too large", who);
+    if (!(d->scale == d->scale) || d->scale - d->scale != 0.0f) return kv_fail(KANVIT_EINVAL, "%s: scale must be finite", who);
+    if (d->causal || e->mask) return kv_fail(KANVIT_EINVAL, "%s: no causal / mask form (kanvit_attn_x_* have them)", who);
+    if (d->flags) return kv_fail(KANVIT_EINVAL, "%s: flags=%d: one mode, exact fp32 (KANVIT_FLAG_BF16_MFMA is not taken; pass no flag)", who, d->flags);
+    return 0;
+}
+
+AttnQ1Args q1_args(const kanvit_attn_desc* d, const kanvit_attn_ext* e) {
+    AttnQ1Args a{};
+    a.H = d->H; a.Nk = e->Nk; a.D = d->D; a.scale = d->scale;
+    a.qsb = d->q_stride_b; a.qsh = d->q_stride_h;
+    a.ksb = d->k_stride_b; a.ksh = d->k_stride_h; a.ksn = d->k_stride_n;
+    a.vsb = d->v_stride_b; a.vsh = d->v_stride_h; a.vsn = d->v_stride_n;
+    a.osb = d->o_stride_b; a.osh = d->o_stride_h;
+    return a;
+}
+
+int q1_width(const AttnQ1Args& a, std::initializer_list<const void*> ptrs) {
+    long long m = a.D;
+    for (long long sd : {a.qsb, a.qsh, a.ksb, a.ksh, a.ksn, a.vsb, a.vsh, a.vsn, a.osb, a.osh}) m |= sd;
+    uintptr_t pm = 0;
+    for (const void* p : ptrs) pm |= (uintptr_t)p;
+    if (m % 4 == 0 && pm % 16 == 0) return 4;
+    if (m % 2 == 0 && pm % 8 == 0) return 2;
+    return 1;
+}
+
 }
 
 extern "C" {
+
+int kanvit_attn_q1_fwd(const kanvit_attn_desc* d, const kanvit_attn_ext* e, const float* q, const float* k, const float* v, float* o,
+                       float* p, void* stream) {
+    if (int rc = q1_check(d, e, "kanvit_attn_q1_fwd")) return rc;
+    if (d->B == 0) return 0;
+    if (!q || !k || !v || !o || !p) return kv_fail(KANVIT_EINVAL, "kanvit_attn_q1_fwd: null q/k/v/o/p");
+    AttnQ1Args a = q1_args(d, e);
+    a.q = q; a.k = k; a.v = v; a.o = o; a.p = p;
+    hipStream_t st = (hipStream_t)stream;
+    const dim3 grid((unsigned)(d->B * d->H));
+    switch (q1_width(a, {q, k, v})) {
+        case 4: hipLaunchKernelGGL(attn_q1_fwd_kernel<4>, grid, dim3(Q1_THR), 0, st, a); break;
+        case 2: hipLaunchKernelGGL(attn_q1_fwd_kernel<2>, grid, dim3(Q1_THR), 0, st, a); break;
+        default: hipLaunchKernelGGL(attn_q1_fwd_kernel<1>, grid, dim3(Q1_THR), 0, st, a); break;
+    }
+    KV_LAUNCH_CHECK("attn_q1_fwd_kernel");
+    return 0;
+}
+
+int kanvit_attn_q1_bwd(const kanvit_attn_desc* d, const kanvit_attn_ext* e, const float* q, const float* k, const float* v, const float* o,
+                       const float* p, const float* d_o, float* dq, float* dk, float* dv, void* stream) {
+    if (int rc = q1_check(d, e, "kanvit_attn_q1_bwd")) return rc;
+    if (d->B == 0) return 0;
+    if (!q || !k || !v || !o || !p || !d_o || !dq || !dk || !dv) return kv_fail(KANVIT_EINVAL, "kanvit_attn_q1_bwd: null argument");
+    AttnQ1Args a = q1_args(d, e);
+    a.q = q; a.k = k; a.v = v; a.o_in = o; a.p = const_cast<float*>(p); a.d_o = d_o; a.dq = dq; a.dk = dk; a.dv = dv;
+    hipStream_t st = (hipStream_t)stream;
+    const dim3 grid((unsigned)(d->B * d->H));
+    switch (q1_width(a, {q, k, v, o, d_o, dq, dk, dv})) {
+        case 4: hipLaunchKernelGGL(attn_q1_bwd_kernel<4>, grid, dim3(Q1_THR), 0, st, a); break;
+        case 2: hipLaunchKernelGGL(attn_q1_bwd_kernel<2>, grid, dim3(Q1_THR), 0, st, a); break;
+        default: hipLaunchKernelGGL(attn_q1_bwd_kernel<1>, grid, dim3(Q1_THR), 0, st, a); break;
+    }
+    KV_LAUNCH_CHECK("attn_q1_bwd_kernel");
+    return 0;
+}
 
 int kanvit_attn_x_fwd(const kanvit_attn_desc* d, const kanvit_attn_ext* e, const float* q, const float* k, const float* v, float* o,
                       float* lse, void* stream) {
diff --git a/kan-vit_amd/kanvit/_lib.py b/kan-vit_amd/kanvit/_lib.py
--- a/kan-vit_amd/kanvit/_lib.py
+++ b/kan-vit_amd/kanvit/_lib.py
@@ -102,6 +102,8 @@
     "kanvit_attn_x_bwd_workspace": (C.c_size_t, [C.POINTER(AttnDesc), C.POINTER(AttnExt)]),
     "kanvit_attn_x_bwd": (C.c_int, [C.POINTER(AttnDesc), C.POINTER(AttnExt), _P, _P, _P, _P, _P, _P, _P, _P, _P, _P, C.c_size_t, _P]),
     "kanvit_attn_probs": (C.c_int, [C.POINTER(AttnDesc), C.POINTER(AttnExt), _P, _P, _P, C.c_int64, C.c_int64, C.c_int64, C.c_int32, _P]),
+    "kanvit_attn_q1_fwd": (C.c_int, [C.POINTER(AttnDesc), C.POINTER(AttnExt), _P, _P, _P, _P, _P, _P]),
+    "kanvit_attn_q1_bwd": (C.c_int, [C.POINTER(AttnDesc), C.POINTER(AttnExt), _P, _P, _P, _P, _P, _P, _P, _P, _P, _P]),
     "kanvit_addln_fwd": (C.c_int, [C.c_int64, C.c_int, C.c_float, _P, _P, _P, _P, _P, _P, _P, _P, _P]),
     "kanvit_addln_fwd_ex": (C.c_int, [C.c_int64, C.c_int, C.c_float, _P, _P, C.c_int, _P, _P, _P, _P, C.c_int, _P, _P, _P]),
     "kanvit_addln_bwd_ex": (C.c_int, [C.c_int64, C.c_int, _P, _P, _P, _P, _P, C.c_int, _P, _P, _P, _P, _P, _P, C.c_size_t, _P]),
@@ -151,14 +153,15 @@
                         "no_lnff": int(bool(os.environ.get("KANVIT_NO_LNFF"))),
                         "no_ff_epi": int(bool(os.environ.get("KANVIT_NO_FF_EPILOGUE"))),
                         "no_dfreq_w": int(bool(os.environ.get("KANVIT_NO_DFREQ_W"))),
-                        "no_patch_bw": int(bool(os.environ.get("KANVIT_NO_PATCH_BW")))}
+                        "no_patch_bw": int(bool(os.environ.get("KANVIT_NO_PATCH_BW"))),
+                        "no_cls_tail": int(bool(os.environ.get("KANVIT_NO_CLS_TAIL")))}
     return _py_switches
 
 
 def active_config() -> str:
     ps = py_switches()
     alt = f" lib={LIB_PATH}" if os.environ.get("KANVIT_LIB") else ""
-    return lib().kanvit_config().decode() + f" py_ff={ps['ff'] or 'default'} py_no_ff_small={ps['no_ff_small']} py_no_lnff={ps['no_lnff']} py_no_ff_epi={ps['no_ff_epi']} py_no_dfreq_w={ps['no_dfreq_w']} py_no_patch_bw={ps['no_patch_bw']}" + alt
+    return lib().kanvit_config().decode() + f" py_ff={ps['ff'] or 'default'} py_no_ff_small={ps['no_ff_small']} py_no_lnff={ps['no_lnff']} py_no_ff_epi={ps['no_ff_epi']} py_no_dfreq_w={ps['no_dfreq_w']} py_no_patch_bw={ps['no_patch_bw']}" + alt + f" py_no_cls_tail={ps['no_cls_tail']}"
 
 
 def reload_config() -> str:
diff --git a/kan-vit_amd/kanvit/grouped.py b/kan-vit_amd/kanvit/grouped.py
--- a/kan-vit_amd/kanvit/grouped.py
+++ b/kan-vit_amd/kanvit/grouped.py
@@ -71,31 +71,43 @@
 
 
 def run_qkv(q_layers: Sequence, k_layers: Sequence, v_layers: Sequence, x2d: torch.Tensor) -> torch.Tensor:
-    H = len(q_layers)
-    layers = list(q_layers) + list(k_layers) + list(v_layers)
-    acts = {ops.base_activation_code(m.base_activation) for m in layers
-            if hasattr(m, "base_activation") and getattr(m, "use_base_update", True)}
-    if len(acts) > 1:
-        dh = x2d.shape[1] // H
-        return torch.cat([run_single(m, x2d[:, (g % H) * dh:(g % H + 1) * dh]) for g, m in enumerate(layers)], dim=1)
+    return run_projections([q_layers, k_layers, v_layers], x2d)
+
+
+def pack_projections(projections: Sequence[Sequence]):
+    H = len(projections[0])
+    assert all(len(p) == H for p in projections), "every projection has one layer per head"
+    layers = [m for p in projections for m in p]
     if isinstance(layers[0], torch.nn.Linear):
         cfg0 = linear_cfg(layers[0])
     elif hasattr(type(layers[0]), "kan_pack_grouped") and "layers" in layers[0].kan_cfg.__code__.co_varnames:
         cfg0 = layers[0].kan_cfg(layers)
     else:
         cfg0 = layers[0].kan_cfg()
-    cfg = replace(cfg0, groups=3 * H, x_group_mod=H)
+    cfg = replace(cfg0, groups=len(layers), x_group_mod=H)
     if isinstance(layers[0], torch.nn.Linear):
         w = stack_params([m.weight for m in layers], perm=(1, 0))
         bp = None
         bias = None if layers[0].bias is None else stack_params([m.bias for m in layers])
     else:
         w, bp, bias = type(layers[0]).kan_pack_grouped(layers)
+    return cfg, w, bp, bias
+
+
+def run_projections(projections: Sequence[Sequence], x2d: torch.Tensor, tag: str = None) -> torch.Tensor:
+    H = len(projections[0])
+    layers = [m for p in projections for m in p]
+    acts = {ops.base_activation_code(m.base_activation) for m in layers
+            if hasattr(m, "base_activation") and getattr(m, "use_base_update", True)}
+    if len(acts) > 1:
+        dh = x2d.shape[1] // H
+        return torch.cat([run_single(m, x2d[:, (g % H) * dh:(g % H + 1) * dh]) for g, m in enumerate(layers)], dim=1)
+    cfg, w, bp, bias = pack_projections(projections)
     if hasattr(layers[0], "kan_ln") and layers[0].kan_ln() is not None and ops.ln_fusable(cfg, x2d.shape[0]):
         gamma = stack_params([l.kan_ln().weight for l in layers])
         beta = stack_params([l.kan_ln().bias for l in layers])
-        return ops.kan_layer_ln(x2d, w, cfg, torch.cat([bp, gamma, beta], dim=1), bias, layers[0].kan_ln().eps)
+        return ops.kan_layer_ln(x2d, w, cfg, torch.cat([bp, gamma, beta], dim=1), bias, layers[0].kan_ln().eps, tag=tag)
     u = None
     if hasattr(layers[0], "kan_u_grouped"):
         u = type(layers[0]).kan_u_grouped(layers, x2d, H)
-    return ops.kan_layer(x2d, w, cfg, u=u, bparams=bp, bias=bias)
+    return ops.kan_layer(x2d, w, cfg, u=u, bparams=bp, bias=bias, tag=tag)
diff --git a/kan-vit_amd/kanvit/ops.py b/kan-vit_amd/kanvit/ops.py
--- a/kan-vit_amd/kanvit/ops.py
+++ b/kan-vit_amd/kanvit/ops.py
@@ -163,7 +163,7 @@
 
     @staticmethod
     @_fwd_f32
-    def forward(ctx, x, u, w, bparams, bias, cfg: LayerCfg):
+    def forward(ctx, x, u, w, bparams, bias, cfg: LayerCfg, tag: Optional[str] = None):
         for n, t in (("x", x), ("u", u), ("w", w), ("bparams", bparams), ("bias", bias)):
             _require_gpu_f32(n, t)
         x = x.contiguous()
@@ -180,7 +180,8 @@
             raise KanvitError(f"u shape {tuple(u.shape)} != {(M, cfg.groups * cfg.I)}")
         y = torch.empty(M, cfg.groups * cfg.O, device=x.device, dtype=torch.float32)
         d = _desc(cfg, M, ldx, cfg.groups * cfg.I, cfg.groups * cfg.O, 0 if bparams is None else bparams.shape[1])
-        tag = ("qkv" if cfg.groups > 1 else "layer") + "_fwd" + ("_bf16" if cfg.flags & _lib.FLAG_BF16_MFMA else "")
+        ctx.tag = tag
+        tag = _tag_prefix(cfg, tag) + "_fwd" + ("_bf16" if cfg.flags & _lib.FLAG_BF16_MFMA else "")
         with torch.cuda.device(x.device):
             nbytes = int(_lib.lib().kanvit_layer_fwd_workspace(C.byref(d)))
             ws = _workspace(nbytes, x.device) if nbytes else None
@@ -199,10 +200,14 @@
     def backward(ctx, dy):
         x, u, w, bparams = ctx.saved_tensors
         return _kan_backward(ctx.cfg, x, u if ctx.has_u else None, w, bparams, dy.float().contiguous(), ctx.needs_input_grad[:5],
-                             ctx.has_u, ctx.has_bias) + (None,)
-
-
-def _kan_backward(cfg: "LayerCfg", x, u, w, bparams, dy, needs, has_u, has_bias, patch=None):
+                             ctx.has_u, ctx.has_bias, tag=ctx.tag) + (None, None)
+
+
+def _tag_prefix(cfg: "LayerCfg", tag: Optional[str]) -> str:
+    return tag or ("qkv" if cfg.groups > 1 else "layer")
+
+
+def _kan_backward(cfg: "LayerCfg", x, u, w, bparams, dy, needs, has_u, has_bias, patch=None, tag=None):
     if patch is not None:
         pd, M = patch
         ldx = cfg.I
@@ -211,6 +216,7 @@
         pd = None
         M, ldx = x.shape
     need_x, need_u, need_w, need_bp, need_b = needs
+    stem = _tag_prefix(cfg, tag)
     d = _desc(cfg, M, ldx, cfg.groups * cfg.I, cfg.groups * cfg.O, 0 if bparams is None else bparams.shape[1])
     L = _lib.lib()
 
@@ -246,7 +252,7 @@
                 dpart = torch.empty(tiles, cfg.groups, cfg.G, device=x.device, dtype=torch.float32)
             nb_in = int(L.kanvit_layer_bwd_input_workspace(C.byref(d)))
             ws_in = _workspace(nb_in, x.device) if nb_in else None
-            with _timed(("qkv" if cfg.groups > 1 else "layer") + "_bwd_input" + ("_bf16" if nb_in else ""),
+            with _timed(stem + "_bwd_input" + ("_bf16" if nb_in else ""),
                         *_layer_cost(cfg, M, "bwd_input")):
                 check(L.kanvit_layer_bwd_input(C.byref(d), _ptr(x), _ptr(u), _ptr(w), _ptr(bparams), _ptr(dy),
                                                _ptr(dx), _ptr(du_buf), _ptr(dpart), _ptr(ws_in), C.c_size_t(nb_in),
@@ -262,12 +268,12 @@
                 dbp[:, :cfg.G] = dpart.sum(0)
         if need_w:
             dw = torch.empty_like(w)
-            weight_pass(d, dw, ("qkv" if cfg.groups > 1 else "layer") + "_bwd_weight" + ("_bf16" if cfg.flags & 1 else ""))
+            weight_pass(d, dw, stem + "_bwd_weight" + ("_bf16" if cfg.flags & 1 else ""))
         if freq_via_w:
             dq = LayerDesc(*[getattr(d, f) for f, _ in LayerDesc._fields_])
             dq.flags = cfg.flags | _lib.FLAG_SINE_DFREQ
             q = torch.empty_like(w)
-            weight_pass(dq, q, ("qkv" if cfg.groups > 1 else "layer") + "_bwd_freq" + ("_bf16" if cfg.flags & 1 else ""))
+            weight_pass(dq, q, stem + "_bwd_freq" + ("_bf16" if cfg.flags & 1 else ""))
             dbp = torch.zeros_like(bparams)
             dbp[:, :cfg.G] = q.mul_(w).view(cfg.groups, cfg.I, cfg.G, cfg.O).sum((1, 3))
         if need_b and has_bias:
@@ -291,7 +297,7 @@
 
     @staticmethod
     @_fwd_f32
-    def forward(ctx, x, w, bparams, bias, cfg: LayerCfg):
+    def forward(ctx, x, w, bparams, bias, cfg: LayerCfg, tag: Optional[str] = None):
         for n, t in (("x", x), ("w", w), ("bparams", bparams), ("bias", bias)):
             _require_gpu_f32(n, t)
         x, w, bparams = x.contiguous(), w.contiguous(), bparams.contiguous()
@@ -306,7 +312,8 @@
         y = torch.empty(M, cfg.groups * cfg.O, device=x.device, dtype=torch.float32)
         stats = torch.empty(M, cfg.x_group_mod, 2, device=x.device, dtype=torch.float32)
         d = _desc(cfg, M, ldx, cfg.groups * cfg.I, cfg.groups * cfg.O, bparams.shape[1])
-        tag = ("qkv" if cfg.groups > 1 else "layer") + "_fwd" + ("_bf16" if cfg.flags & _lib.FLAG_BF16_MFMA else "")
+        ctx.tag = tag
+        tag = _tag_prefix(cfg, tag) + "_fwd" + ("_bf16" if cfg.flags & _lib.FLAG_BF16_MFMA else "")
         with torch.cuda.device(x.device):
             nbytes = int(_lib.lib().kanvit_layer_fwd_workspace(C.byref(d)))
             ws = _workspace(nbytes, x.device) if nbytes else None
@@ -326,7 +333,7 @@
         need_x, need_w, need_bp, need_b = ctx.needs_input_grad[:4]
         need_ln = need_x or need_bp
         dx, du, dw, _, db = _kan_backward(cfg, x, stats, w, bparams, dy.float().contiguous(),
-                                          (need_ln, need_ln, need_w, False, need_b), True, ctx.has_bias)
+                                          (need_ln, need_ln, need_w, False, need_b), True, ctx.has_bias, tag=ctx.tag)
         dbp = None
         if need_ln:
             M, I, G = x.shape[0], cfg.I, cfg.G
@@ -341,14 +348,14 @@
                                                 _ptr(dgb[0]), _ptr(dgb[1]), _ptr(ws), C.c_size_t(nbytes), _stream()), "kanvit_layer_ln_bwd")
             if need_bp:
                 dbp = torch.cat([torch.zeros(cfg.groups, G, device=x.device, dtype=torch.float32), dgb[0], dgb[1]], dim=1)
-        return (dx if need_x else None), dw, dbp, db, None
+        return (dx if need_x else None), dw, dbp, db, None, None
 
 
 def kan_layer_ln(x: torch.Tensor, w: torch.Tensor, cfg: LayerCfg, bparams: torch.Tensor, bias: Optional[torch.Tensor],
-                 eps: float) -> torch.Tensor:
+                 eps: float, tag: Optional[str] = None) -> torch.Tensor:
     from dataclasses import replace
     f = cfg.flags | _lib.FLAG_FUSED_LN | (_lib.FLAG_BF16_MFMA if _autocast_flags() else 0)
-    return _KanLayerLnFn.apply(x, w, bparams, bias, replace(cfg, flags=f, ln_eps=float(eps)))
+    return _KanLayerLnFn.apply(x, w, bparams, bias, replace(cfg, flags=f, ln_eps=float(eps)), tag)
 
 
 def patchify(images: torch.Tensor, n_patches: int) -> torch.Tensor:
@@ -419,11 +426,11 @@
 
 
 def kan_layer(x: torch.Tensor, w: torch.Tensor, cfg: LayerCfg, u: Optional[torch.Tensor] = None,
-              bparams: Optional[torch.Tensor] = None, bias: Optional[torch.Tensor] = None) -> torch.Tensor:
+              bparams: Optional[torch.Tensor] = None, bias: Optional[torch.Tensor] = None, tag: Optional[str] = None) -> torch.Tensor:
     if torch.is_autocast_enabled("cuda") and torch.get_autocast_dtype("cuda") == torch.bfloat16 and not (cfg.flags & 1):
         from dataclasses import replace
         cfg = replace(cfg, flags=cfg.flags | _lib.FLAG_BF16_MFMA)
-    return _KanLayerFn.apply(x, u, w, bparams, bias, cfg)
+    return _KanLayerFn.apply(x, u, w, bparams, bias, cfg, tag)
 
 
 EDGE_L1_FAMILIES = (BSPLINE, CHEBY, RBF)
@@ -774,6 +781,54 @@
     return _AttnFn.apply(q, k, v, causal, q.shape[-1] ** -0.5 if scale is None else scale, _autocast_flags())
 
 
+class _AttnQ1Fn(torch.autograd.Function):
+
+    @staticmethod
+    @_fwd_f32
+    def forward(ctx, q0, kv, scale: float):
+        _require_gpu_f32("q0", q0)
+        _require_gpu_f32("kv", kv)
+        if kv.dim() != 5 or kv.shape[2] != 2 or q0.dim() != 3 or (q0.shape[0], q0.shape[1], q0.shape[2]) != (kv.shape[0], kv.shape[3], kv.shape[4]):
+            raise KanvitError(f"attention_q1: q0 {tuple(q0.shape)} and kv {tuple(kv.shape)} are not [B, H, D] and [B, N, 2, H, D]")
+        q0, kv = q0.contiguous(), kv.contiguous()
+        B, N, _, H, D = kv.shape
+        o = torch.empty(B, H, D, device=kv.device, dtype=torch.float32)
+        p = torch.empty(B, H, N, device=kv.device, dtype=torch.float32)
+        d, e = _attn_q1_desc(q0, kv, o, scale)
+        with torch.cuda.device(kv.device), _timed("attn_q1_fwd", 4 * B * H * N * D, 4 * B * H * (2 * N * D + N + 2 * D)):
+            check(_lib.lib().kanvit_attn_q1_fwd(C.byref(d), C.byref(e), _ptr(q0), _ptr(kv[:, :, 0]), _ptr(kv[:, :, 1]), _ptr(o), _ptr(p),
+                                                _stream()), "kanvit_attn_q1_fwd")
+        ctx.save_for_backward(q0, kv, o, p)
+        ctx.scale = scale
+        return o
+
+    @staticmethod
+    @_bwd
+    def backward(ctx, do):
+        q0, kv, o, p = ctx.saved_tensors
+        do = do.float().contiguous()
+        B, N, _, H, D = kv.shape
+        dq = torch.empty_like(q0)
+        dkv = torch.empty_like(kv)
+        d, e = _attn_q1_desc(q0, kv, o, ctx.scale)
+        with torch.cuda.device(kv.device), _timed("attn_q1_bwd", 8 * B * H * N * D, 4 * B * H * (4 * N * D + N + 4 * D)):
+            check(_lib.lib().kanvit_attn_q1_bwd(C.byref(d), C.byref(e), _ptr(q0), _ptr(kv[:, :, 0]), _ptr(kv[:, :, 1]), _ptr(o), _ptr(p),
+                                                _ptr(do), _ptr(dq), _ptr(dkv[:, :, 0]), _ptr(dkv[:, :, 1]), _stream()), "kanvit_attn_q1_bwd")
+        return dq, dkv, None
+
+
+def _attn_q1_desc(q0, kv, o, scale: float):
+    B, N, _, H, D = kv.shape
+    k = kv[:, :, 0]
+    d = AttnDesc(B, H, 1, D, 0, float(scale), 0, 0, q0.stride(0), q0.stride(1), 0, k.stride(0), k.stride(2), k.stride(1),
+                 k.stride(0), k.stride(2), k.stride(1), o.stride(0), o.stride(1), 0)
+    return d, _lib.AttnExt(N, 0, None, 0, 0, 0, 0)
+
+
+def attention_q1(q0: torch.Tensor, kv: torch.Tensor, scale: Optional[float] = None) -> torch.Tensor:
+    return _AttnQ1Fn.apply(q0, kv, kv.shape[-1] ** -0.5 if scale is None else float(scale))
+
+
 def expand_attention_mask(mask: Optional[torch.Tensor], q: torch.Tensor, k: torch.Tensor) -> Optional[torch.Tensor]:
     if mask is None:
         return None
diff --git a/kan-vit_amd/model.py b/kan-vit_amd/model.py
--- a/kan-vit_amd/model.py
+++ b/kan-vit_amd/model.py
@@ -2,7 +2,7 @@
 import torch.nn as nn
 
 from attention import MSA, FlashAttention
-from kanvit import ops
+from kanvit import _lib, ops
 from kanvit.dense import feed_forward, ff_mode, ff_small_supported, ln_feed_forward
 from kanvit.ops import add_layernorm
 from models.cheby import ChebyKANLayer
@@ -43,6 +43,26 @@
         x, h2 = add_layernorm(x, self.attn(h1), self.norm2, y_bf16=ybf)
         b, n, d = x.shape
         return x, feed_forward(h2.reshape(b * n, d), self.ff[0], self.ff[2]).view(b, n, d)
+
+
+    def run_cls(self, x, pending):
+        x, h1 = add_layernorm(x, pending, self.norm1)
+        ybf = (x.is_cuda and torch.is_autocast_enabled("cuda") and torch.get_autocast_dtype("cuda") == torch.bfloat16)
+        a0 = _FirstRow.apply(self.attn(h1)) if ybf else self.attn.forward_cls(h1)
+        s, h2 = add_layernorm(_FirstRow.apply(x), a0, self.norm2, y_bf16=ybf and ff_mode() != "bf16x3")
+        return s + feed_forward(h2, self.ff[0], self.ff[2])
+
+
+class _FirstRow(torch.autograd.Function):
+
+    @staticmethod
+    def forward(ctx, t):
+        ctx.n = t.shape[1]
+        return t[:, 0].contiguous()
+
+    @staticmethod
+    def backward(ctx, g):
+        return torch.nn.functional.pad(g.unsqueeze(1), (0, 0, 0, ctx.n - 1))
 
 
 class _ClsToken(torch.autograd.Function):
@@ -284,7 +304,13 @@
                 reg = self.linear_mapper.regularization_loss(rows, **reg_kw)
         out = self._embed(images, patches)
         pending = None
+        last = self.blocks[-1] if len(self.blocks) else None
+        cls_tail = (isinstance(last, TransformerBlock) and reg_kw is None and out.is_cuda and not _lib.py_switches()["no_cls_tail"]
+                    and not ff_small_supported(last.ff[0].in_features, last.ff[0].out_features))
         for blk in self.blocks:
+            if cls_tail and blk is last:
+                out = blk.run_cls(out, pending)
+                return self.mlp_head(out)
             if isinstance(blk, TransformerBlock) and reg_kw is not None:
                 out, pending, r = blk.run(out, pending, reg_kw)
                 reg = reg + r
diff --git a/kan-vit_amd/models/fastkan.py b/kan-vit_amd/models/fastkan.py
--- a/kan-vit_amd/models/fastkan.py
+++ b/kan-vit_amd/models/fastkan.py
@@ -109,9 +109,10 @@
         M = x2d.shape[0]
         dh = layers[0].input_dim
         xhat = F.layer_norm(x2d.view(M, n_heads, dh), (dh,), None, None, layers[0].layernorm.eps)
-        gamma = grouped.stack_params([l.layernorm.weight for l in layers]).view(1, 3, n_heads, dh)
-        beta = grouped.stack_params([l.layernorm.bias for l in layers]).view(1, 3, n_heads, dh)
-        return torch.addcmul(beta, xhat.unsqueeze(1), gamma).reshape(M, 3 * n_heads * dh)
+        P = len(layers) // n_heads
+        gamma = grouped.stack_params([l.layernorm.weight for l in layers]).view(1, P, n_heads, dh)
+        beta = grouped.stack_params([l.layernorm.bias for l in layers]).view(1, P, n_heads, dh)
+        return torch.addcmul(beta, xhat.unsqueeze(1), gamma).reshape(M, P * n_heads * dh)
 
     def edge_activation_l1(self, x, include_base=False):
         from dataclasses import replace
```

After: 1624, median of 6. +7.3%, better.
